# MaartenGr/PolyFuzz

Hardware: AMD Instinct MI355X
Metric: string-pairs/sec, TF-IDF cosine top-n 100k x 100k (config.timed_step says what a step is: by default the user-level .match() call of SURVEY section 8d's metric, `device_step` = the list resident in HBM; latency.top1_single_query_ms = top-1 match latency) (higher is better)
Workload: dtype f32

## Files before the change

### include/polyfuzz_hip.h

```cpp
#ifndef POLYFUZZ_HIP_H
#define POLYFUZZ_HIP_H

#include <stdint.h>

#ifdef __cplusplus
extern "C" {
#endif

#define PFZ_VERSION 100

typedef enum pfz_status {
    PFZ_OK = 0,
    PFZ_ERR_INVALID = -1,
    PFZ_ERR_NO_DEVICE = -2,
    PFZ_ERR_HIP = -3,
    PFZ_ERR_UNSUPPORTED = -4,
    PFZ_ERR_NOMEM = -5,
    PFZ_ERR_RCCL = -6
} pfz_status;

typedef struct pfz_ctx pfz_ctx;
typedef struct pfz_csr pfz_csr;
typedef struct pfz_index pfz_index;
typedef struct pfz_topn pfz_topn;
typedef struct pfz_strings pfz_strings;
typedef struct pfz_tfidf pfz_tfidf;
typedef struct pfz_comm pfz_comm;

int pfz_version(void);
const char *pfz_last_error(void);
int pfz_device_count(void);
int pfz_ctx_create(int device, pfz_ctx **out);
void pfz_ctx_destroy(pfz_ctx *ctx);
int pfz_ctx_sync(pfz_ctx *ctx);
int pfz_ctx_info(pfz_ctx *ctx, char *name256, int32_t *n_cu, int64_t *hbm_bytes);

int pfz_event_record(pfz_ctx *ctx, int32_t slot);
int pfz_event_elapsed_ms(pfz_ctx *ctx, int32_t slot_begin, int32_t slot_end, float *ms);
int pfz_stage_reserve(pfz_ctx *ctx, int64_t bytes, void **host);
int pfz_event_wait(pfz_ctx *ctx, int32_t slot);
int pfz_prof_enable(pfz_ctx *ctx, int32_t on);
int pfz_prof_reset(pfz_ctx *ctx);
int pfz_prof_get(pfz_ctx *ctx, const char *name, double *total_ms, int64_t *launches);

int pfz_csr_upload(pfz_ctx *ctx, int64_t n_rows, int64_t n_cols,
                   const int64_t *indptr, const int32_t *indices, const float *data,
                   pfz_csr **out);
int pfz_csr_shape(const pfz_csr *m, int64_t *n_rows, int64_t *n_cols, int64_t *nnz);
int pfz_csr_download(pfz_ctx *ctx, const pfz_csr *m, int64_t *indptr, int32_t *indices, float *data);
void pfz_csr_free(pfz_csr *m);

int pfz_index_build(pfz_ctx *ctx, const pfz_csr *to_matrix, pfz_index **out);
void pfz_index_free(pfz_index *ix);
int pfz_index_info(const pfz_index *ix, int64_t *n_rows, int64_t *n_cols, int64_t *nnz,
                   int64_t *block_cols, int64_t *n_blocks, int64_t *table_bytes);
int pfz_index_pieces(const pfz_index *ix, int64_t *n_pieces, int64_t *piece_postings);
int pfz_index_symmetric_launches(const pfz_index *ix, int64_t *launches, int64_t *rows);
int pfz_index_symmetric_census(const pfz_index *ix, int64_t *magnet_rows, int64_t *recomputed_rows);

int pfz_topn_alloc(pfz_ctx *ctx, int64_t n_rows, int32_t ntop, pfz_topn **out);
void pfz_topn_free(pfz_topn *t);
int pfz_topn_clear(pfz_ctx *ctx, pfz_topn *t);
int pfz_topn_download(pfz_ctx *ctx, const pfz_topn *t, int32_t *out_idx, float *out_val);
int pfz_topn_download_rows_after(pfz_ctx *ctx, const pfz_topn *t, int64_t row_begin, int64_t row_end,
                                 int32_t event_slot, int32_t *out_idx, float *out_val);
int pfz_topn_rows_begin(pfz_ctx *ctx, const pfz_topn *t, int64_t row_begin, int64_t row_end, int32_t event_slot, int32_t half);
int pfz_topn_rows_finish(pfz_ctx *ctx, int32_t half, const int32_t **idx, const float **val);
int pfz_topn_upload(pfz_ctx *ctx, pfz_topn *t, const int32_t *idx, const float *val);
int pfz_topn_device_ptrs(const pfz_topn *t, void **idx_dev, void **val_dev, int64_t *n_rows, int32_t *ntop);

int pfz_cossim_topn(pfz_ctx *ctx, const pfz_index *to_index, const pfz_csr *from_matrix,
                    int32_t ntop, float lower_bound, int32_t exclude_diag, int64_t diag_offset,
                    pfz_topn *out);

int pfz_cossim_topn_rows(pfz_ctx *ctx, const pfz_index *to_index, const pfz_csr *from_matrix,
                         int64_t row_begin, int64_t row_end, int32_t ntop, float lower_bound,
                         int32_t exclude_diag, int64_t diag_offset, pfz_topn *out);

int pfz_cossim_topn_ranges(pfz_ctx *ctx, const pfz_index *to_index, const pfz_csr *from_matrix, int32_t ntop, float lower_bound,
                           int32_t exclude_diag, int32_t n_ranges, const int64_t *range_ends, int32_t first_event, pfz_topn *out,
                           const int32_t **host_idx, const float **host_val);

int pfz_cossim_topn_host(pfz_ctx *ctx,
                         int64_t n_from, int64_t n_to, int64_t n_cols,
                         const int64_t *from_indptr, const int32_t *from_indices, const float *from_data,
                         const int64_t *to_indptr, const int32_t *to_indices, const float *to_data,
                         int32_t ntop, float lower_bound, int32_t exclude_diag,
                         int32_t *out_idx, float *out_val);

int pfz_strings_upload(pfz_ctx *ctx, const void *chars, const int64_t *offsets, int64_t n_strings,
                       int32_t char_width, pfz_strings **out);
void pfz_strings_free(pfz_strings *s);

typedef struct pfz_tfidf_params {
    int32_t ngram_lo, ngram_hi;
    int32_t clean;
    int32_t remove_space_ngrams;
} pfz_tfidf_params;

int pfz_tfidf_fit(pfz_ctx *ctx, const pfz_tfidf_params *params,
                  const pfz_strings *docs_a, const pfz_strings *docs_b, pfz_tfidf **out);
void pfz_tfidf_free(pfz_tfidf *v);
int pfz_tfidf_info(const pfz_tfidf *v, int64_t *vocab_size, int64_t *n_docs, int32_t *code_bits);
int pfz_tfidf_export(pfz_ctx *ctx, const pfz_tfidf *v, uint32_t *ngrams, double *idf, int64_t *df);
int pfz_tfidf_import(pfz_ctx *ctx, const pfz_tfidf_params *params, int64_t vocab_size, int64_t n_docs,
                     const uint32_t *ngrams, const double *idf, pfz_tfidf **out);
int pfz_tfidf_transform(pfz_ctx *ctx, const pfz_tfidf *v, const pfz_strings *docs, pfz_csr **out);

int pfz_indel_argmax(pfz_ctx *ctx, const pfz_strings *from_strings, const pfz_strings *to_strings,
                     const int32_t *skip_idx, int64_t from_begin, int64_t from_end,
                     int32_t *out_idx, double *out_score);
int pfz_indel_argmax_dev(pfz_ctx *ctx, const pfz_strings *from_strings, const pfz_strings *to_strings,
                         const int32_t *skip_idx, int64_t from_begin, int64_t from_end, pfz_topn *out);
int pfz_indel_matrix_host(pfz_ctx *ctx, const pfz_strings *from_strings, const pfz_strings *to_strings,
                          int64_t from_begin, int64_t from_end, double *out_matrix);
int pfz_indel_plan_info(pfz_ctx *ctx, const pfz_strings *to_strings, int64_t *n_symbols, int64_t *n_groups,
                        int64_t *char_steps);

int pfz_fuzz_extract_one(pfz_ctx *ctx, const pfz_strings *from_strings, const pfz_strings *to_strings, int32_t scorer,
                         const int32_t *skip_idx, int64_t from_begin, int64_t from_end, int32_t *out_idx, double *out_score);
int pfz_fuzz_extract_one_dev(pfz_ctx *ctx, const pfz_strings *from_strings, const pfz_strings *to_strings, int32_t scorer,
                             const int32_t *skip_idx, int64_t from_begin, int64_t from_end, pfz_topn *out,
                             uint64_t *work_counters);
int pfz_fuzz_plan_info(pfz_ctx *ctx, const pfz_strings *to_strings, int64_t *n_symbols, int64_t *n_groups, int64_t *n_tokens,
                       int64_t *n_general_strings);

int pfz_dense_cossim_topn_host(pfz_ctx *ctx, const float *from_vec, int64_t n_from,
                               const float *to_vec, int64_t n_to, int64_t dim,
                               int32_t ntop, float lower_bound, int32_t exclude_diag,
                               int32_t *out_idx, float *out_val);
int pfz_dense_dot_topn_host(pfz_ctx *ctx, const float *from_vec, int64_t n_from,
                            const float *to_vec, int64_t n_to, int64_t dim,
                            int32_t ntop, float lower_bound, int32_t exclude_diag,
                            int32_t *out_idx, float *out_val);

typedef struct pfz_dense pfz_dense;
int pfz_dense_upload(pfz_ctx *ctx, const float *vec, int64_t n, int64_t dim, int32_t normalize, pfz_dense **out);
int pfz_dense_shape(const pfz_dense *m, int64_t *n, int64_t *dim);
void pfz_dense_free(pfz_dense *m);
int pfz_dense_topn(pfz_ctx *ctx, const pfz_dense *from_vectors, const pfz_dense *to_vectors, int32_t ntop,
                   float lower_bound, int32_t exclude_diag, int64_t diag_offset, pfz_topn *out);

int pfz_pr_curve_host(pfz_ctx *ctx, const double *sim, int64_t n, const double *thresholds,
                      int32_t n_thresholds, int64_t *count_ge, double *sum_ge);
int pfz_linkage_top1(pfz_ctx *ctx, const pfz_topn *result, double min_similarity,
                     int32_t *out_cluster, int32_t *out_key, int32_t *out_info3);

int pfz_comm_unique_id(uint8_t id128[128]);
int pfz_comm_init(pfz_ctx *ctx, const uint8_t id128[128], int32_t rank, int32_t world, pfz_comm **out);
int pfz_rccl_versions(int32_t *header, int32_t *runtime);
void pfz_comm_destroy(pfz_comm *c);
typedef struct pfz_comm_group pfz_comm_group;
int pfz_comm_group_create(int32_t world, pfz_comm_group **out);
void pfz_comm_group_destroy(pfz_comm_group *g);
int pfz_comm_init_local(pfz_ctx *ctx, pfz_comm_group *g, int32_t rank, pfz_comm **out);
int pfz_comm_allgather_topn(pfz_comm *c, const pfz_topn *local, pfz_topn *global);
int pfz_comm_merge_to_shards(pfz_comm *c, const pfz_topn *local, int64_t to_offset, pfz_topn *out);
int pfz_comm_barrier(pfz_comm *c);
int pfz_comm_cossim_topn_symmetric(pfz_comm *c, const pfz_index *ix, const pfz_csr *A, int32_t ntop, float lower_bound,
                                   pfz_topn *out);
int pfz_index_symmetric_ok(const pfz_index *ix, const pfz_csr *A, int32_t ntop, int32_t n_parts, int32_t *yes);
int pfz_comm_symmetric_ok(pfz_comm *c, const pfz_index *ix, const pfz_csr *A, int32_t ntop, int32_t *yes);
int pfz_comm_info(const pfz_comm *c, int32_t *rank, int32_t *world);
int pfz_tfidf_fit_sharded(pfz_ctx *ctx, pfz_comm *comm, const pfz_tfidf_params *params,
                          const pfz_strings *replicated, const pfz_strings *local_shard, pfz_tfidf **out);

#ifdef __cplusplus
}
#endif
#endif
```

### polyfuzz_amd/_lib.py

```python
import ctypes
import os
import threading

import numpy as np

from . import _build

c_i32, c_i64, c_f32, c_f64 = ctypes.c_int32, ctypes.c_int64, ctypes.c_float, ctypes.c_double
c_vp = ctypes.c_void_p
P = ctypes.POINTER


class PfzError(RuntimeError):
    def __init__(self, code, msg):
        super().__init__(f"libpolyfuzz_hip error {code}: {msg}")
        self.code = code


class PfzUnsupported(PfzError, NotImplementedError):
    pass


class PfzNoDevice(PfzError):
    pass


class TfidfParams(ctypes.Structure):
    _fields_ = [("ngram_lo", c_i32), ("ngram_hi", c_i32), ("clean", c_i32), ("remove_space_ngrams", c_i32)]


SIGNATURES = {
    "pfz_version": (ctypes.c_int, []),
    "pfz_last_error": (ctypes.c_char_p, []),
    "pfz_device_count": (ctypes.c_int, []),
    "pfz_ctx_create": (ctypes.c_int, [ctypes.c_int, P(c_vp)]),
    "pfz_ctx_destroy": (None, [c_vp]),
    "pfz_ctx_sync": (ctypes.c_int, [c_vp]),
    "pfz_ctx_info": (ctypes.c_int, [c_vp, ctypes.c_char_p, P(c_i32), P(c_i64)]),
    "pfz_event_record": (ctypes.c_int, [c_vp, c_i32]),
    "pfz_event_elapsed_ms": (ctypes.c_int, [c_vp, c_i32, c_i32, P(c_f32)]),
    "pfz_prof_enable": (ctypes.c_int, [c_vp, c_i32]),
    "pfz_prof_reset": (ctypes.c_int, [c_vp]),
    "pfz_prof_get": (ctypes.c_int, [c_vp, ctypes.c_char_p, P(c_f64), P(c_i64)]),
    "pfz_csr_upload": (ctypes.c_int, [c_vp, c_i64, c_i64, c_vp, c_vp, c_vp, P(c_vp)]),
    "pfz_csr_shape": (ctypes.c_int, [c_vp, P(c_i64), P(c_i64), P(c_i64)]),
    "pfz_csr_download": (ctypes.c_int, [c_vp, c_vp, c_vp, c_vp, c_vp]),
    "pfz_csr_free": (None, [c_vp]),
    "pfz_index_build": (ctypes.c_int, [c_vp, c_vp, P(c_vp)]),
    "pfz_index_free": (None, [c_vp]),
    "pfz_index_info": (ctypes.c_int, [c_vp, P(c_i64), P(c_i64), P(c_i64), P(c_i64), P(c_i64), P(c_i64)]),
    "pfz_index_pieces": (ctypes.c_int, [c_vp, P(c_i64), P(c_i64)]),
    "pfz_index_symmetric_launches": (ctypes.c_int, [c_vp, P(c_i64), P(c_i64)]),
    "pfz_index_symmetric_census": (ctypes.c_int, [c_vp, P(c_i64), P(c_i64)]),
    "pfz_index_symmetric_ok": (ctypes.c_int, [c_vp, c_vp, c_i32, c_i32, P(c_i32)]),
    "pfz_comm_cossim_topn_symmetric": (ctypes.c_int, [c_vp, c_vp, c_vp, c_i32, ctypes.c_float, c_vp]),
    "pfz_comm_symmetric_ok": (ctypes.c_int, [c_vp, c_vp, c_vp, c_i32, P(c_i32)]),
    "pfz_rccl_versions": (ctypes.c_int, [P(c_i32), P(c_i32)]),
    "pfz_topn_alloc": (ctypes.c_int, [c_vp, c_i64, c_i32, P(c_vp)]),
    "pfz_topn_free": (None, [c_vp]),
    "pfz_topn_download": (ctypes.c_int, [c_vp, c_vp, c_vp, c_vp]),
    "pfz_topn_clear": (ctypes.c_int, [c_vp, c_vp]),
    "pfz_topn_download_rows_after": (ctypes.c_int, [c_vp, c_vp, c_i64, c_i64, c_i32, c_vp, c_vp]),
    "pfz_topn_rows_begin": (ctypes.c_int, [c_vp, c_vp, c_i64, c_i64, c_i32, c_i32]),
    "pfz_topn_rows_finish": (ctypes.c_int, [c_vp, c_i32, P(c_vp), P(c_vp)]),
    "pfz_cossim_topn_ranges": (ctypes.c_int, [c_vp, c_vp, c_vp, c_i32, ctypes.c_float, c_i32, c_i32, P(c_i64), c_i32, c_vp, P(c_vp), P(c_vp)]),
    "pfz_event_wait": (ctypes.c_int, [c_vp, c_i32]),
    "pfz_stage_reserve": (ctypes.c_int, [c_vp, c_i64, P(c_vp)]),
    "pfz_topn_upload": (ctypes.c_int, [c_vp, c_vp, c_vp, c_vp]),
    "pfz_topn_device_ptrs": (ctypes.c_int, [c_vp, P(c_vp), P(c_vp), P(c_i64), P(c_i32)]),
    "pfz_cossim_topn": (ctypes.c_int, [c_vp, c_vp, c_vp, c_i32, c_f32, c_i32, c_i64, c_vp]),
    "pfz_cossim_topn_rows": (ctypes.c_int, [c_vp, c_vp, c_vp, c_i64, c_i64, c_i32, c_f32, c_i32, c_i64, c_vp]),
    "pfz_cossim_topn_host": (ctypes.c_int, [c_vp, c_i64, c_i64, c_i64, c_vp, c_vp, c_vp, c_vp, c_vp, c_vp,
                                            c_i32, c_f32, c_i32, c_vp, c_vp]),
    "pfz_strings_upload": (ctypes.c_int, [c_vp, c_vp, c_vp, c_i64, c_i32, P(c_vp)]),
    "pfz_strings_free": (None, [c_vp]),
    "pfz_tfidf_fit": (ctypes.c_int, [c_vp, P(TfidfParams), c_vp, c_vp, P(c_vp)]),
    "pfz_tfidf_free": (None, [c_vp]),
    "pfz_tfidf_info": (ctypes.c_int, [c_vp, P(c_i64), P(c_i64), P(c_i32)]),
    "pfz_tfidf_export": (ctypes.c_int, [c_vp, c_vp, c_vp, c_vp, c_vp]),
    "pfz_tfidf_import": (ctypes.c_int, [c_vp, P(TfidfParams), c_i64, c_i64, c_vp, c_vp, P(c_vp)]),
    "pfz_tfidf_transform": (ctypes.c_int, [c_vp, c_vp, c_vp, P(c_vp)]),
    "pfz_indel_argmax": (ctypes.c_int, [c_vp, c_vp, c_vp, c_vp, c_i64, c_i64, c_vp, c_vp]),
    "pfz_indel_matrix_host": (ctypes.c_int, [c_vp, c_vp, c_vp, c_i64, c_i64, c_vp]),
    "pfz_indel_plan_info": (ctypes.c_int, [c_vp, c_vp, P(c_i64), P(c_i64), P(c_i64)]),
    "pfz_indel_argmax_dev": (ctypes.c_int, [c_vp, c_vp, c_vp, c_vp, c_i64, c_i64, c_vp]),
    "pfz_fuzz_extract_one": (ctypes.c_int, [c_vp, c_vp, c_vp, c_i32, c_vp, c_i64, c_i64, c_vp, c_vp]),
    "pfz_fuzz_extract_one_dev": (ctypes.c_int, [c_vp, c_vp, c_vp, c_i32, c_vp, c_i64, c_i64, c_vp, c_vp]),
    "pfz_fuzz_plan_info": (ctypes.c_int, [c_vp, c_vp, P(c_i64), P(c_i64), P(c_i64), P(c_i64)]),
    "pfz_dense_cossim_topn_host": (ctypes.c_int, [c_vp, c_vp, c_i64, c_vp, c_i64, c_i64, c_i32, c_f32, c_i32,
                                                  c_vp, c_vp]),
    "pfz_dense_dot_topn_host": (ctypes.c_int, [c_vp, c_vp, c_i64, c_vp, c_i64, c_i64, c_i32, c_f32, c_i32,
                                               c_vp, c_vp]),
    "pfz_dense_upload": (ctypes.c_int, [c_vp, c_vp, c_i64, c_i64, c_i32, P(c_vp)]),
    "pfz_dense_shape": (ctypes.c_int, [c_vp, P(c_i64), P(c_i64)]),
    "pfz_dense_free": (None, [c_vp]),
    "pfz_dense_topn": (ctypes.c_int, [c_vp, c_vp, c_vp, c_i32, c_f32, c_i32, c_i64, c_vp]),
    "pfz_pr_curve_host": (ctypes.c_int, [c_vp, c_vp, c_i64, c_vp, c_i32, c_vp, c_vp]),
    "pfz_linkage_top1": (ctypes.c_int, [c_vp, c_vp, c_f64, c_vp, c_vp, c_vp]),
    "pfz_comm_unique_id": (ctypes.c_int, [c_vp]),
    "pfz_comm_init": (ctypes.c_int, [c_vp, c_vp, c_i32, c_i32, P(c_vp)]),
    "pfz_comm_destroy": (None, [c_vp]),
    "pfz_comm_group_create": (ctypes.c_int, [c_i32, P(c_vp)]),
    "pfz_comm_group_destroy": (None, [c_vp]),
    "pfz_comm_init_local": (ctypes.c_int, [c_vp, c_vp, c_i32, P(c_vp)]),
    "pfz_comm_allgather_topn": (ctypes.c_int, [c_vp, c_vp, c_vp]),
    "pfz_comm_merge_to_shards": (ctypes.c_int, [c_vp, c_vp, c_i64, c_vp]),
    "pfz_comm_barrier": (ctypes.c_int, [c_vp]),
    "pfz_comm_info": (ctypes.c_int, [c_vp, P(c_i32), P(c_i32)]),
    "pfz_tfidf_fit_sharded": (ctypes.c_int, [c_vp, c_vp, P(TfidfParams), c_vp, c_vp, P(c_vp)]),
}

_lib = None
_lock = threading.Lock()


def lib_path():
    return os.environ.get("POLYFUZZ_HIP_LIB") or _build.LIB_PATH


def load():
    global _lib
    if _lib is not None:
        return _lib
    with _lock:
        if _lib is not None:
            return _lib
        path = lib_path()
        if not os.path.exists(path):
            raise ImportError(
                f"{path} is missing: build it with `python -c 'import __graft_entry__ as g; g.build()'` "
                "(hipcc, gfx950).  polyfuzz_amd has no CPU fallback.")
        lib = ctypes.CDLL(path)
        for name, (res, args) in SIGNATURES.items():
            fn = getattr(lib, name)
            fn.restype = res
            fn.argtypes = args
        _lib = lib
        return lib


def check(rc):
    if rc == 0:
        return
    msg = load().pfz_last_error().decode("utf-8", "replace")
    if rc == -4:
        raise PfzUnsupported(rc, msg)
    if rc == -2:
        raise PfzNoDevice(rc, msg)
    raise PfzError(rc, msg)


def _ptr(a):
    return None if a is None else a.ctypes.data_as(c_vp)


def device_count():
    return int(load().pfz_device_count())


class Context:
    _default = None

    def __init__(self, device=None):
        if device is None:
            device = int(os.environ.get("POLYFUZZ_HIP_DEVICE", os.environ.get("LOCAL_RANK", "0")))
        self.lib = load()
        h = c_vp()
        check(self.lib.pfz_ctx_create(int(device), ctypes.byref(h)))
        self.h = h
        self.device = int(device)

    @classmethod
    def default(cls):
        if cls._default is None:
            cls._default = cls()
        return cls._default

    def close(self):
        if getattr(self, "h", None):
            self.lib.pfz_ctx_destroy(self.h)
            self.h = None

    def __del__(self):
        try:
            self.close()
        except Exception:
            pass

    def sync(self):
        check(self.lib.pfz_ctx_sync(self.h))

    def info(self):
        name = ctypes.create_string_buffer(256)
        ncu, mem = c_i32(), c_i64()
        check(self.lib.pfz_ctx_info(self.h, name, ctypes.byref(ncu), ctypes.byref(mem)))
        return {"name": name.value.decode(), "n_cu": ncu.value, "hbm_bytes": mem.value}

    def event_record(self, slot):
        check(self.lib.pfz_event_record(self.h, slot))

    def event_wait(self, slot):
        check(self.lib.pfz_event_wait(self.h, slot))

    def event_wait_fn(self):
        return ctypes.cast(self.lib.pfz_event_wait, ctypes.c_void_p).value, self.h.value if hasattr(self.h, "value") else int(self.h)

    def event_elapsed_ms(self, a, b):
        ms = c_f32()
        check(self.lib.pfz_event_elapsed_ms(self.h, a, b, ctypes.byref(ms)))
        return float(ms.value)

    def prof_enable(self, on=True):
        check(self.lib.pfz_prof_enable(self.h, int(on)))

    def prof_reset(self):
        check(self.lib.pfz_prof_reset(self.h))

    def prof_get(self, name):
        ms, n = c_f64(), c_i64()
        check(self.lib.pfz_prof_get(self.h, name.encode(), ctypes.byref(ms), ctypes.byref(n)))
        return float(ms.value), int(n.value)


class _Handle:
    _free = None

    def __init__(self, ctx, h):
        self.ctx = ctx
        self.h = h

    def free(self):
        if getattr(self, "h", None) and self.ctx.h:
            getattr(self.ctx.lib, self._free)(self.h)
        self.h = None

    def __del__(self):
        try:
            self.free()
        except Exception:
            pass


class DeviceCSR(_Handle):
    _free = "pfz_csr_free"

    @classmethod
    def upload(cls, ctx, indptr, indices, data, n_cols):
        indptr = np.ascontiguousarray(indptr, np.int64)
        indices = np.ascontiguousarray(indices, np.int32)
        data = np.ascontiguousarray(data, np.float32)
        h = c_vp()
        check(ctx.lib.pfz_csr_upload(ctx.h, len(indptr) - 1, int(n_cols), _ptr(indptr), _ptr(indices), _ptr(data),
                                     ctypes.byref(h)))
        return cls(ctx, h)

    @classmethod
    def from_scipy(cls, ctx, m):
        m = m.tocsr()
        if not m.has_sorted_indices:
            m = m.sorted_indices()
        return cls.upload(ctx, m.indptr, m.indices, m.data, m.shape[1])

    @property
    def shape(self):
        r, c, z = c_i64(), c_i64(), c_i64()
        check(self.ctx.lib.pfz_csr_shape(self.h, ctypes.byref(r), ctypes.byref(c), ctypes.byref(z)))
        return r.value, c.value, z.value

    @property
    def n_rows(self):
        r = c_i64()
        check(self.ctx.lib.pfz_csr_shape(self.h, ctypes.byref(r), None, None))
        return r.value

    def download(self):
        n_rows, n_cols, nnz = self.shape
        indptr = np.empty(n_rows + 1, np.int64)
        indices = np.empty(nnz, np.int32)
        data = np.empty(nnz, np.float32)
        check(self.ctx.lib.pfz_csr_download(self.ctx.h, self.h, _ptr(indptr), _ptr(indices), _ptr(data)))
        return indptr, indices, data, n_cols


class DeviceIndex(_Handle):
    _free = "pfz_index_free"

    @classmethod
    def build(cls, ctx, to_csr):
        h = c_vp()
        check(ctx.lib.pfz_index_build(ctx.h, to_csr.h, ctypes.byref(h)))
        return cls(ctx, h)

    def info(self):
        v = [c_i64() for _ in range(6)]
        check(self.ctx.lib.pfz_index_info(self.h, *[ctypes.byref(x) for x in v]))
        keys = ("n_rows", "n_cols", "nnz", "block_cols", "n_blocks", "table_bytes")
        out = dict(zip(keys, (x.value for x in v)))
        npc, per = c_i64(), c_i64()
        check(self.ctx.lib.pfz_index_pieces(self.h, ctypes.byref(npc), ctypes.byref(per)))
        out.update(n_pieces=npc.value, piece_postings=per.value)
        return out

    def symmetric_launches(self):
        a, b = c_i64(), c_i64()
        check(self.ctx.lib.pfz_index_symmetric_launches(self.h, ctypes.byref(a), ctypes.byref(b)))
        return a.value, b.value

    def symmetric_ok(self, csr, ntop, n_parts=1):
        yes = c_i32()
        check(self.ctx.lib.pfz_index_symmetric_ok(self.h, csr.h, int(ntop), int(n_parts), ctypes.byref(yes)))
        return bool(yes.value)

    def symmetric_census(self):
        a, b = c_i64(), c_i64()
        check(self.ctx.lib.pfz_index_symmetric_census(self.h, ctypes.byref(a), ctypes.byref(b)))
        return a.value, b.value


class DeviceTopN(_Handle):
    _free = "pfz_topn_free"

    @classmethod
    def alloc(cls, ctx, n_rows, ntop):
        h = c_vp()
        check(ctx.lib.pfz_topn_alloc(ctx.h, int(n_rows), int(ntop), ctypes.byref(h)))
        t = cls(ctx, h)
        t.n_rows, t.ntop = int(n_rows), int(ntop)
        return t

    def download(self):
        idx = np.empty((self.n_rows, self.ntop), np.int32)
        val = np.empty((self.n_rows, self.ntop), np.float32)
        check(self.ctx.lib.pfz_topn_download(self.ctx.h, self.h, _ptr(idx), _ptr(val)))
        return idx, val

    def clear(self):
        check(self.ctx.lib.pfz_topn_clear(self.ctx.h, self.h))

    def download_rows_after(self, begin, end, event_slot):
        idx = np.empty((end - begin, self.ntop), np.int32)
        val = np.empty((end - begin, self.ntop), np.float32)
        check(self.ctx.lib.pfz_topn_download_rows_after(self.ctx.h, self.h, int(begin), int(end), int(event_slot), _ptr(idx),
                                                        _ptr(val)))
        return idx, val

    def rows_begin(self, begin, end, event_slot, half):
        check(self.ctx.lib.pfz_topn_rows_begin(self.ctx.h, self.h, int(begin), int(end), int(event_slot), int(half)))

    def rows_finish(self, half):
        a, b = c_vp(), c_vp()
        check(self.ctx.lib.pfz_topn_rows_finish(self.ctx.h, int(half), ctypes.byref(a), ctypes.byref(b)))
        return a.value, b.value

    @classmethod
    def from_host(cls, ctx, idx, val):
        idx = np.ascontiguousarray(idx, np.int32)
        val = np.ascontiguousarray(val, np.float32)
        if idx.ndim == 1:
            idx, val = idx[:, None], val[:, None]
        t = cls.alloc(ctx, idx.shape[0], idx.shape[1])
        check(ctx.lib.pfz_topn_upload(ctx.h, t.h, _ptr(idx), _ptr(val)))
        return t

    def upload(self, idx, val):
        idx = np.ascontiguousarray(idx, np.int32).reshape(self.n_rows, self.ntop)
        val = np.ascontiguousarray(val, np.float32).reshape(self.n_rows, self.ntop)
        check(self.ctx.lib.pfz_topn_upload(self.ctx.h, self.h, _ptr(idx), _ptr(val)))

    def device_ptrs(self):
        pi, pv = c_vp(), c_vp()
        check(self.ctx.lib.pfz_topn_device_ptrs(self.h, ctypes.byref(pi), ctypes.byref(pv), None, None))
        return pi.value, pv.value


def cossim_topn(ctx, index, from_csr, ntop, lower_bound, exclude_diag=False, diag_offset=0, out=None, rows=None):
    if out is None:
        out = DeviceTopN.alloc(ctx, from_csr.n_rows, ntop)
    if rows is None:
        check(ctx.lib.pfz_cossim_topn(ctx.h, index.h, from_csr.h, int(ntop), float(lower_bound),
                                      int(bool(exclude_diag)), int(diag_offset), out.h))
    else:
        check(ctx.lib.pfz_cossim_topn_rows(ctx.h, index.h, from_csr.h, int(rows[0]), int(rows[1]), int(ntop),
                                           float(lower_bound), int(bool(exclude_diag)), int(diag_offset), out.h))
    return out


def cossim_topn_ranges(ctx, index, from_csr, ntop, lower_bound, exclude_diag, range_ends, first_event, out=None, mirror=False):
    if out is None:
        out = DeviceTopN.alloc(ctx, from_csr.n_rows, ntop)
    ends = (c_i64 * len(range_ends))(*[int(e) for e in range_ends])
    hi, hv = c_vp(), c_vp()
    check(ctx.lib.pfz_cossim_topn_ranges(ctx.h, index.h, from_csr.h, int(ntop), float(lower_bound), int(bool(exclude_diag)),
                                         len(range_ends), ends, int(first_event), out.h,
                                         ctypes.byref(hi) if mirror else None, ctypes.byref(hv) if mirror else None))
    return (out, hi.value, hv.value) if mirror else out


def cossim_topn_host(ctx, from_csr3, to_csr3, n_cols, ntop, lower_bound, exclude_diag=False):
    fp, fi, fv = from_csr3
    tp, ti, tv = to_csr3
    fp = np.ascontiguousarray(fp, np.int64)
    fi = np.ascontiguousarray(fi, np.int32)
    fv = np.ascontiguousarray(fv, np.float32)
    tp = np.ascontiguousarray(tp, np.int64)
    ti = np.ascontiguousarray(ti, np.int32)
    tv = np.ascontiguousarray(tv, np.float32)
    n_from, n_to = len(fp) - 1, len(tp) - 1
    idx = np.empty((n_from, ntop), np.int32)
    val = np.empty((n_from, ntop), np.float32)
    check(ctx.lib.pfz_cossim_topn_host(ctx.h, n_from, n_to, int(n_cols), _ptr(fp), _ptr(fi), _ptr(fv),
                                       _ptr(tp), _ptr(ti), _ptr(tv), int(ntop), float(lower_bound),
                                       int(bool(exclude_diag)), _ptr(idx), _ptr(val)))
    return idx, val



try:
    from . import _pack
except ImportError:
    _pack = None


def usable_cpus():
    n = len(os.sched_getaffinity(0)) if hasattr(os, "sched_getaffinity") else (os.cpu_count() or 1)
    try:
        with open("/sys/fs/cgroup/cpu.max") as f:
            quota, period = f.read().split()[:2]
        if quota != "max":
            n = min(n, int(quota) // int(period))
    except (OSError, ValueError):
        pass
    return max(1, n)


def host_threads():
    env = os.environ.get("PFZ_HOST_THREADS")
    return max(1, min(16, int(env))) if env else max(1, min(8, usable_cpus() // 2))


_PACK_THREADS = _PACK_INTO_THREADS = host_threads()


def pack_strings(strings, objects=None):
    if _pack is not None and isinstance(strings, (list, tuple)):
        if objects is not None:
            raw, off, width = _pack.pack(strings, _PACK_THREADS, objects.ctypes.data)
        else:
            raw, off, width = _pack.pack(strings, _PACK_THREADS)
        return np.frombuffer(raw, np.uint8 if width == 1 else np.uint32), np.frombuffer(off, np.int64), width
    if objects is not None:
        objects[:] = strings
    return _pack_strings_py(strings)


def _pack_strings_py(strings):
    n = len(strings)
    lens = np.fromiter(map(len, strings), np.int64, n)
    off = np.zeros(n + 1, np.int64)
    np.cumsum(lens, out=off[1:])
    joined = "".join(strings)
    try:
        raw = joined.encode("latin-1")
        chars = np.frombuffer(raw, np.uint8)
        width = 1
    except UnicodeEncodeError:
        raw = joined.encode("utf-32-le", "surrogatepass")
        chars = np.frombuffer(raw, np.uint32)
        width = 4
    if len(chars) != off[-1]:
        raise ValueError("string packing length mismatch")
    return chars, off, width


class DeviceStrings(_Handle):
    _free = "pfz_strings_free"

    @classmethod
    def upload(cls, ctx, strings):
        if len(strings) >= 1024:
            direct = cls.upload_direct(ctx, strings)
            if direct is not None:
                return direct
        return cls.upload_packed(ctx, *pack_strings(strings))

    @classmethod
    def upload_direct(cls, ctx, strings, objects=None):
        if _pack is None or not hasattr(_pack, "pack_into") or not isinstance(strings, (list, tuple)):
            return None
        n = len(strings)
        off_bytes = (8 * (n + 1) + 255) & ~255
        cap = off_bytes + 48 * n + 65536
        host = c_vp()
        check(ctx.lib.pfz_stage_reserve(ctx.h, cap, ctypes.byref(host)))
        if not host.value:
            return None
        n_chars = _pack.pack_into(strings, objects.ctypes.data if objects is not None else 0, host.value, off_bytes, cap, _PACK_INTO_THREADS)
        if n_chars is None:
            return None
        h = c_vp()
        check(ctx.lib.pfz_strings_upload(ctx.h, c_vp(host.value + off_bytes), c_vp(host.value), n, 1, ctypes.byref(h)))
        s = cls(ctx, h)
        s.n = n
        s.char_width = 1
        return s

    @classmethod
    def upload_packed(cls, ctx, chars, off, width):
        n = len(off) - 1
        h = c_vp()
        check(ctx.lib.pfz_strings_upload(ctx.h, _ptr(chars) if len(chars) else None, _ptr(off), n, width,
                                         ctypes.byref(h)))
        s = cls(ctx, h)
        s.n = n
        s.char_width = width
        return s


class DeviceTfidf(_Handle):
    _free = "pfz_tfidf_free"

    @classmethod
    def fit(cls, ctx, params, docs_a, docs_b=None):
        h = c_vp()
        rc = ctx.lib.pfz_tfidf_fit(ctx.h, ctypes.byref(params), docs_a.h if docs_a is not None else None,
                                   docs_b.h if docs_b is not None else None, ctypes.byref(h))
        if rc == -1 and b"empty vocabulary" in ctx.lib.pfz_last_error():
            raise ValueError("empty vocabulary; perhaps the documents only contain stop words")
        check(rc)
        v = cls(ctx, h)
        v.params = params
        return v

    @classmethod
    def from_state(cls, ctx, params, ngrams, idf, n_docs):
        ngrams = np.ascontiguousarray(ngrams, np.uint32)
        idf = np.ascontiguousarray(idf, np.float64)
        h = c_vp()
        check(ctx.lib.pfz_tfidf_import(ctx.h, ctypes.byref(params), len(idf), int(n_docs), _ptr(ngrams), _ptr(idf),
                                       ctypes.byref(h)))
        v = cls(ctx, h)
        v.params = params
        return v

    def info(self):
        vs, nd, cb = c_i64(), c_i64(), c_i32()
        check(self.ctx.lib.pfz_tfidf_info(self.h, ctypes.byref(vs), ctypes.byref(nd), ctypes.byref(cb)))
        return {"vocab": vs.value, "n_docs": nd.value, "code_bits": cb.value}

# ... 265 lines not shown
```

### polyfuzz_amd/csrc/k3_core.h

```cpp
#pragma once
#include "pfz_internal.h"

#include <math.h>
#include <utility>

#ifndef PFZ_K3_EXP
#define PFZ_K3_EXP 0
#endif

namespace pfz {

constexpr int kSelectMinTop = 16;
constexpr int kWarmMaxTop = 8;
constexpr int kPiece = 16;
constexpr long long kPieceBoundMax = 1 << 20;

#ifndef PFZ_K3_SHFL_MAX
#define PFZ_K3_SHFL_MAX 0
#endif
__device__ inline uint64_t wave_max_u64(uint64_t v)
{
#if PFZ_K3_SHFL_MAX
#pragma unroll
    for (int d = 32; d >= 1; d >>= 1) {
// ... 184 lines not shown
    }
    return best - 1;
}

template <int N4, int kCap, bool kBounded = false>
__device__ inline void sweep_block(int4 *acc4, uint64_t *cand, TopState &st, int col0, int self_col, int ntop, int lane,
                                   int zero, uint64_t ub = ~0ull)
{
    static_assert(N4 % 128 == 0, "a wave sweeps whole 128-slot steps");
#pragma unroll 2
    for (int t = 0; t < N4 / 128; ++t) {
        const int i0 = t * 128 + lane, i1 = i0 + 64;
        const int4 v0 = acc4[i0], v1 = acc4[i1];
        acc4[i0] = make_int4(zero, zero, zero, zero);
        acc4[i1] = make_int4(zero, zero, zero, zero);
        const int mx = max3i(max3i(v0.x, v0.y, v0.z), max3i(v0.w, v1.x, v1.y), max3i(v1.z, v1.w, v1.w));
        if (__ballot(mx > st.thr)) {
            push4<kCap, kBounded>(cand, st, v0, col0 + i0 * 4, self_col, ntop, lane, ub);
            push4<kCap, kBounded>(cand, st, v1, col0 + i1 * 4, self_col, ntop, lane, ub);
        }
    }
}

template <int S> __device__ inline int row_bcast_i(int v)
{
    return __builtin_amdgcn_update_dpp(0, v, 0x150 + S, 0xf, 0xf, false);
}

template <int S>
__device__ inline int2 load_piece_entry(const char *__restrict__ post_bytes, int addr_t, int sub8)
{
    const uint32_t a = (uint32_t)(row_bcast_i<S>(addr_t) + sub8);
#if PFZ_K3_EXP == 2
    return make_int2((int)((a * 2654435761u) >> 19) & 8188, 0x3c000000);
#else
    return *(const int2 *)(post_bytes + a);
#endif
}

template <int S> __device__ inline void apply_entry(int *acc, const int2 &pe, float as_t)
{
    const int v = (int)(__int_as_float(row_bcast_i<S>(__float_as_int(as_t))) * __int_as_float(pe.y));
#if PFZ_K3_EXP == 1
    if (v == 0x7fffffff) atomicAdd((int *)((char *)acc + pe.x), v);
#elif PFZ_K3_EXP == 3
    atomicAdd((int *)((char *)acc + ((pe.x & 0x1f00) | (threadIdx.x * 4))), v);
#else
    atomicAdd((int *)((char *)acc + pe.x), v);
#endif
}

template <int... S>
__device__ inline void run_steps_seq(int *acc, const char *__restrict__ post_bytes, int addr_t, float as_t, int sub8,
                                     std::integer_sequence<int, S...>)
{
    const int2 pe[sizeof...(S)] = {load_piece_entry<S>(post_bytes, addr_t, sub8)...};
    (apply_entry<S>(acc, pe[S], as_t), ...);
}

template <int NS>
__device__ inline void run_steps(int *acc, const char *__restrict__ post_bytes, int addr_t, float as_t, int sub8)
{
    run_steps_seq(acc, post_bytes, addr_t, as_t, sub8, std::make_integer_sequence<int, NS>{});
}

__device__ inline int dpp_add_scan(int v)
{
    asm("s_nop 1\n\tv_add_u32_dpp %0, %0, %0 row_shr:1 row_mask:0xf bank_mask:0xf bound_ctrl:1" : "+v"(v));
    asm("s_nop 1\n\tv_add_u32_dpp %0, %0, %0 row_shr:2 row_mask:0xf bank_mask:0xf bound_ctrl:1" : "+v"(v));
    asm("s_nop 1\n\tv_add_u32_dpp %0, %0, %0 row_shr:4 row_mask:0xf bank_mask:0xf bound_ctrl:1" : "+v"(v));
    asm("s_nop 1\n\tv_add_u32_dpp %0, %0, %0 row_shr:8 row_mask:0xf bank_mask:0xf bound_ctrl:1" : "+v"(v));
    asm("s_nop 1\n\tv_add_u32_dpp %0, %0, %0 row_bcast:15 row_mask:0xa bank_mask:0xf" : "+v"(v));
    asm("s_nop 1\n\tv_add_u32_dpp %0, %0, %0 row_bcast:31 row_mask:0xc bank_mask:0xf" : "+v"(v));
    return v;
}

__device__ inline void scatter_pieces(int *acc, const char *__restrict__ post_bytes, int *mark, int np, int st, float as,
                                      int lane, int src4, int sub8, int dummy_addr)
{
    const int pin = dpp_add_scan(np);
    const int total = __builtin_amdgcn_readlane(pin, 63);
    const int excl = pin - np;
    const int base = st - excl;
    const int pt = 4 * (lane & 15) + (lane >> 4);
    for (int r0 = 0; r0 < total; r0 += 64) {
#if PFZ_K3_EXP == 4
        const int addr_t = np > 0 ? (int)((uint32_t)(st + ((r0 + pt) % np)) << 7) : dummy_addr;
        const float as_t = as;
#else
        const int rel = excl - r0;
        mark[lane] = 0;
        if (np > 0 && rel < 64 && rel + np > 0) mark[rel > 0 ? rel : 0] = lane + 1;
        wave_sync();
        const int owner1 = dpp_max_scan(mark[lane]);
        const int o4 = __builtin_amdgcn_ds_bpermute(src4, owner1) * 4 - 4;
        const int b_o = __builtin_amdgcn_ds_bpermute(o4, base);
        const float as_t = __int_as_float(__builtin_amdgcn_ds_bpermute(o4, __float_as_int(as)));
        const int P = r0 + pt;
        const int addr_t = P < total ? (int)((uint32_t)(b_o + P) << 7) : dummy_addr;
        wave_sync();
#endif
        const int left = total - r0;
        const int ng = left >= 64 ? 8 : (left + 7) >> 3;
#if PFZ_K3_EXP == 6
        if (ng <= 4) {
            if (ng <= 2) run_steps<4>(acc, post_bytes, addr_t, as_t, sub8);
            else run_steps<8>(acc, post_bytes, addr_t, as_t, sub8);
        } else {
            if (ng <= 6) run_steps<12>(acc, post_bytes, addr_t, as_t, sub8);
            else run_steps<16>(acc, post_bytes, addr_t, as_t, sub8);
        }
#else
        if (ng <= 4) {
            if (ng <= 2) {
                if (ng == 1) run_steps<2>(acc, post_bytes, addr_t, as_t, sub8);
                else run_steps<4>(acc, post_bytes, addr_t, as_t, sub8);
            } else {
                if (ng == 3) run_steps<6>(acc, post_bytes, addr_t, as_t, sub8);
                else run_steps<8>(acc, post_bytes, addr_t, as_t, sub8);
            }
        } else {
            if (ng <= 6) {
                if (ng == 5) run_steps<10>(acc, post_bytes, addr_t, as_t, sub8);
                else run_steps<12>(acc, post_bytes, addr_t, as_t, sub8);
            } else {
                if (ng == 7) run_steps<14>(acc, post_bytes, addr_t, as_t, sub8);
                else run_steps<16>(acc, post_bytes, addr_t, as_t, sub8);
            }
        }
#endif
    }
}

inline void k3_fixed_point(const pfz_csr *A, const pfz_index *ix, float lower_bound, float *scale, float *inv_scale, int32_t *thr0)
{
    if (lower_bound < 0.f) lower_bound = 0.f;
    const double bound = (double)A->max_norm * (double)ix->max_norm * 1.0001 + 1e-30;
    int k = 30;
    while (k > -60 && ldexp(bound, k) >= 2147483000.0) --k;
    while (k < 60 && ldexp(bound, k + 1) < 1073741824.0) ++k;
    *scale = (float)ldexp(1.0, k);
    *inv_scale = (float)ldexp(1.0, -k);
    const double thr_d = floor((double)lower_bound * (double)*scale);
    *thr0 = thr_d >= 2147483000.0 ? 2147483000 : (int32_t)thr_d;
}

bool k3_lockstep_wanted(const pfz_ctx *ctx, const pfz_index *ix, int64_t n_rows, int32_t ntop);
int k3_lockstep_launch(pfz_ctx *ctx, const pfz_index *ix, const pfz_csr *A, int64_t row_begin, int64_t n_rows, int32_t ntop,
                       int32_t thr0, float scale, float inv_scale, int32_t exclude_diag, int64_t diag_offset, pfz_topn *out);


int k3_sym_wanted(const pfz_ctx *ctx, const pfz_index *ix, const pfz_csr *A, int64_t row_begin, int64_t row_end, int32_t ntop,
                  int32_t thr0, float scale, int32_t exclude_diag, int64_t diag_offset, const pfz_topn *out);
int k3_sym_launch(pfz_ctx *ctx, const pfz_index *ix, const pfz_csr *A, int64_t row_begin, int64_t row_end, int32_t ntop,
                  int32_t thr0, float scale, float inv_scale, pfz_topn *out, bool start, bool *declined);
int k3_sym_launch_streamed(pfz_ctx *ctx, const pfz_index *ix, const pfz_csr *A, int32_t ntop, int32_t thr0, float scale, float inv_scale,
                           pfz_topn *out, int32_t n_ranges, const int64_t *ends, int32_t first_event, int32_t *host_idx, float *host_val,
                           bool *declined);
void k3_sym_free(pfz_index *ix);

}
```

### polyfuzz_amd/csrc/k3_cossim_topn.hip

```cpp
#include "k3_core.h"

#include <algorithm>
#include <math.h>
#include <stdlib.h>

namespace pfz {

constexpr int kMergeCap = 256;
constexpr int kMaxTop = 1024;

__global__ __launch_bounds__(256) void k_index_count(const int32_t *__restrict__ indptr,
                                                      const int32_t *__restrict__ indices, int32_t n_rows,
                                                      int32_t nb, int32_t block, int32_t *__restrict__ cnt)
{
    const int gid = (blockIdx.x * 256 + threadIdx.x) >> 4;
    const int sub = threadIdx.x & 15;
    if (gid >= n_rows) return;
    const int p0 = indptr[gid], p1 = indptr[gid + 1];
    const int b = gid / block;
    for (int p = p0 + sub; p < p1; p += 16) atomicAdd(&cnt[(int64_t)indices[p] * nb + b], 1);
}

__global__ __launch_bounds__(256) void k_index_fill(const int32_t *__restrict__ indptr,
                                                     const int32_t *__restrict__ indices,
// ... 245 lines not shown
                nxt0 = trow[b_next + 1];
            }
            for (int c0 = p0 + 64; c0 < p1; c0 += 64) {
                int s2 = 0, e2 = 0;
                float as2 = 0.f;
                if (c0 + lane < p1) {
                    const int k = a_idx[c0 + lane];
                    as2 = a_val[c0 + lane] * scale;
                    s2 = tab[(int64_t)k * nb + b];
                    e2 = tab[(int64_t)k * nb + b + 1];
                }
                if (__ballot(e2 > s2)) {
                    touched = true;
                    scatter_pieces(acc, post_bytes, mark, e2 - s2, s2, as2, lane, src4, sub8, dummy_addr);
                }
            }
            if (touched && ablate != 2) {
                wave_sync();
                if (!warmed) {
                    warmed = true;
                    if (ntop <= kWarmMaxTop) {
                        const int t = warm_threshold<N4>(acc4, 0, ntop + (self_col >= 0 ? 1 : 0), lane);
                        st.thr = t > st.thr ? t : st.thr;
                    }
                }
                sweep_block<N4, kCap, kBounded>(acc4, cand, st, b * C, self_col, ntop, lane, zero, ub_row);
                wave_sync();
            }
            b = b_next;
        }

        compact<kCap>(cand, st, ntop, lane);
        if (kBounded && lane == 0) ub[row] = st.cnt == ntop ? cand[ntop - 1] : 0ull;
        for (int r = lane; r < ntop; r += 64) {
            const uint64_t key = r < st.cnt ? cand[r] : 0ull;
            if (n_slices > 1) {
                part_keys[((int64_t)row * n_slices + slice) * ntop + r] = key;
            } else {
                out_idx[(int64_t)row * ntop + r] = key ? (int32_t)(~(uint32_t)key) : -1;
                out_val[(int64_t)row * ntop + r] = key ? (float)(int32_t)(uint32_t)(key >> 32) * inv_scale : 0.f;
            }
        }
        wave_sync();
    }
}

constexpr int kBankMin = 64, kBankCap = 1024;
__global__ __launch_bounds__(256) void k_index_bank_order(const int32_t *__restrict__ cnt, const int32_t *__restrict__ tab,
                                                           const int32_t *__restrict__ heavy, int32_t heavy_cap,
                                                           int2 *__restrict__ post)
{
    __shared__ int2 s_buf[4][kBankCap];
    __shared__ int s_cnt[4][32];
    const int lane = threadIdx.x & 63, wave = threadIdx.x >> 6;
    int2 *buf = s_buf[wave];
    int *bc = s_cnt[wave];
    const int n_heavy = min(heavy[0], heavy_cap);
    const int n_waves = (int)gridDim.x * 4;
    for (int h = (int)blockIdx.x * 4 + wave; h < n_heavy; h += n_waves) {
        {
            const int64_t slot = heavy[1 + h];
            const int c = min(cnt[slot], kBankCap);
            const int64_t base = (int64_t)tab[slot] * kPiece;
            if (lane < 32) bc[lane] = 0;
            __builtin_amdgcn_fence(__ATOMIC_ACQ_REL, "wavefront");
            __builtin_amdgcn_wave_barrier();
            for (int i = lane; i < c; i += 64) {
                int2 pe = post[base + i];
                const int b = (pe.x >> 2) & 31;
                const int j = atomicAdd(&bc[b], 1);
                buf[i] = make_int2(pe.x, pe.y);
                buf[i].x = pe.x | (j << 16);
            }
            __builtin_amdgcn_fence(__ATOMIC_ACQ_REL, "wavefront");
            __builtin_amdgcn_wave_barrier();
            const int my_cnt = lane < 32 ? bc[lane] : 0;
            for (int i = lane; i < c + 63 - (c + 63) % 64; i += 64) {
                const bool on = i < c;
                int2 pe = on ? buf[i] : make_int2(0, 0);
                const int j = (int)((uint32_t)pe.x >> 16), b = (pe.x >> 2) & 31;
                int pos = 0;
#pragma unroll
                for (int q = 0; q < 32; ++q) {
                    const int cq = __shfl(my_cnt, q, 64);
                    pos += min(cq, j) + ((q < b && cq > j) ? 1 : 0);
                }
                if (on) post[base + pos] = make_int2(pe.x & 0xffff, pe.y);
            }
            __builtin_amdgcn_fence(__ATOMIC_ACQ_REL, "wavefront");
            __builtin_amdgcn_wave_barrier();
        }
    }
}

__global__ __launch_bounds__(256) void k3_merge_slices(const uint64_t *__restrict__ part_keys, int32_t n_a,
                                                       int32_t n_slices, int32_t ntop, float inv_scale,
                                                       int32_t *__restrict__ out_idx, float *__restrict__ out_val)
{
    constexpr int kCap = kMergeCap;
    __shared__ __attribute__((aligned(16))) uint64_t cand_all[4][kCap];
    const int lane = threadIdx.x & 63, wave = threadIdx.x >> 6;
    const int row = blockIdx.x * 4 + wave;
    if (row >= n_a) return;
    uint64_t *cand = cand_all[wave];
    TopState st;
    st.cnt = 0;
    st.thr = 0;
    const uint64_t *src = part_keys + (int64_t)row * n_slices * ntop;
    const int total = n_slices * ntop;
    for (int e0 = 0; e0 < total; e0 += 64) {
        const uint64_t key = e0 + lane < total ? src[e0 + lane] : 0ull;
        const uint64_t mk = __ballot(key != 0ull);
        if (key) cand[st.cnt + __popcll(mk & ((1ull << lane) - 1ull))] = key;
        st.cnt += __popcll(mk);
        if (st.cnt > kCap - 64) compact<kCap>(cand, st, ntop, lane, false);
    }
    compact<kCap>(cand, st, ntop, lane);
    for (int r = lane; r < ntop; r += 64) {
        const uint64_t key = r < st.cnt ? cand[r] : 0ull;
        out_idx[(int64_t)row * ntop + r] = key ? (int32_t)(~(uint32_t)key) : -1;
        out_val[(int64_t)row * ntop + r] = key ? (float)(int32_t)(uint32_t)(key >> 32) * inv_scale : 0.f;
    }
}

__global__ __launch_bounds__(256) void k_topn_place(const int32_t *__restrict__ t_idx, const float *__restrict__ t_val, int64_t n_rows,
                                                    int32_t w, int32_t ntop, int32_t col0, int32_t *__restrict__ out_idx,
                                                    float *__restrict__ out_val)
{
    const int64_t i = (int64_t)blockIdx.x * 256 + threadIdx.x;
    if (i >= n_rows * w) return;
    const int64_t r = i / w;
    const int c = (int)(i - r * w);
    out_idx[r * ntop + col0 + c] = t_idx[i];
    out_val[r * ntop + col0 + c] = t_val[i];
}

static int env_int(const char *name, int dflt)
{
    const char *v = getenv(name);
    return v && *v ? atoi(v) : dflt;
}

int index_ready(const pfz_index *ix)
{
    int32_t v = 0;
    if (ix->pieces_lazy.pending) {
        PFZ_TRY(lazy_get(ix->ctx, &ix->pieces_lazy, &v));
        ix->n_pieces = v - 1;
    }
    if (ix->nnz_lazy.pending) {
        PFZ_TRY(lazy_get(ix->ctx, &ix->nnz_lazy, &v));
        ix->nnz = v;
    }
    return PFZ_OK;
}

}

using namespace pfz;

extern "C" {

int pfz_index_build(pfz_ctx *ctx, const pfz_csr *B, pfz_index **out)
{
    PFZ_REQUIRE(ctx && B && out, "pfz_index_build: NULL argument");
    PFZ_HIP(hipSetDevice(ctx->device));
    int block = env_int("PFZ_K3_BLOCK", 2048);
    if (block != 1024 && block != 1536 && block != 2048 && block != 4096) block = 2048;
    const int64_t nb = (B->n_rows + block - 1) / block;
    const int64_t slots = B->n_cols * nb;
    if (slots >= ((int64_t)1 << 31) - 2) {
        set_error("pfz_index_build: vocabulary %lld x %lld to-blocks exceeds the int32 offset table",
                  (long long)B->n_cols, (long long)nb);
        return PFZ_ERR_UNSUPPORTED;
    }
    Owner<pfz_index, pfz_index_free> ix(new pfz_index());
    ix->ctx = ctx;
    ix->n_rows = B->n_rows;
    ix->n_cols = B->n_cols;
    ix->block_cols = block;
    ix->n_blocks = (int32_t)nb;
    ix->max_norm = B->max_norm;
    ix->src_serial = B->serial;
    struct Tmp {
        int32_t *p = nullptr;
        ~Tmp() { if (p) pool_free(p); }
    } cnt, sub;
    const bool any = B->n_rows > 0;
    const bool lds_hist = B->n_cols <= 2 * (int64_t)kHistWords && !getenv("PFZ_NO_LDS_HIST");
    PFZ_TRY(pool_alloc(ctx, &ix->tab_base, (size_t)(slots + 3) * sizeof(int32_t)));
    ix->tab = ix->tab_base + 1;
    PFZ_TRY(pool_alloc(ctx, &cnt.p, (size_t)(slots + 2) * sizeof(int32_t)));
    if (lds_hist && any) {
        PFZ_TRY(pool_alloc(ctx, &sub.p, (size_t)(slots + 1) * kSub * sizeof(int32_t)));
        PFZ_HIP(hipMemsetAsync(sub.p, 0, (size_t)slots * kSub * sizeof(int32_t), ctx->stream));
    } else {
        PFZ_HIP(hipMemsetAsync(cnt.p, 0, (size_t)(slots + 2) * sizeof(int32_t), ctx->stream));
    }
    const char *bo_env = getenv("PFZ_K3_BANK_ORDER");
    const bool bank_order = any && lds_hist && !getenv("PFZ_K3_NO_BANK_ORDER") &&
                            ((bo_env && atoi(bo_env) > 0) || (!bo_env && B->n_rows >= 32768));
    const int32_t bank_min = kBankMin;
    const int32_t heavy_cap = (int32_t)std::min<int64_t>(slots, (int64_t)1 << 22);
    Tmp heavy;
    if (bank_order) {
        PFZ_TRY(pool_alloc(ctx, &heavy.p, (size_t)(heavy_cap + 1) * sizeof(int32_t)));
        PFZ_HIP(hipMemsetAsync(heavy.p, 0, sizeof(int32_t), ctx->stream));
    }
    const int32_t words = (int32_t)((B->n_cols + 1) / 2);
    const unsigned row_grid = (unsigned)((B->n_rows * 16 + 255) / 256);
    const unsigned slot_grid = (unsigned)((slots + kPiece + 255) / 256);
    {
        ProfScope ps(ctx, "k_index_count");
        if (any && lds_hist)
            hipLaunchKernelGGL(k_index_count_lds, dim3((unsigned)nb * kSub), dim3(1024), 0, ctx->stream, B->indptr, B->indices,
                               (int32_t)B->n_rows, (int32_t)nb, block, words, sub.p);
        else if (any)
            hipLaunchKernelGGL(k_index_count, dim3(row_grid), dim3(256), 0, ctx->stream, B->indptr, B->indices,
                               (int32_t)B->n_rows, (int32_t)nb, block, cnt.p);
        hipLaunchKernelGGL(k_index_pieces, dim3(slot_grid), dim3(256), 0, ctx->stream, cnt.p, lds_hist && any ? sub.p : nullptr, slots,
                           ix->tab, heavy.p, heavy_cap, bank_min);
    }
    PFZ_TRY(exclusive_scan_i32(ctx, ix->tab_base, slots + 1, &ix->pieces_lazy));
    const int64_t nnz_bound = B->nnz_lazy.pending ? B->nnz_cap : B->nnz;
    int64_t piece_cap = nnz_bound / kPiece + std::min<int64_t>(slots, nnz_bound) + 1;
    if (piece_cap > kPieceBoundMax) {
        int32_t total = 0;
        PFZ_TRY(lazy_get(ctx, &ix->pieces_lazy, &total));
        ix->n_pieces = total - 1;
        if (total - 1 >= (1 << 25) - 1) {
            set_error("pfz_index_build: %d index pieces (%lld postings padded to 16 per list and block) exceed the 4 GiB "
                      "the kernel addresses with 32-bit byte offsets", total - 1, (long long)csr_nnz(B));
            return PFZ_ERR_UNSUPPORTED;
        }
        piece_cap = total;
    }
    ix->piece_cap = piece_cap;
    PFZ_TRY(lazy_acquire(ctx, &ix->nnz_lazy));
    PFZ_TRY(pool_alloc(ctx, &ix->post, (size_t)piece_cap * kPiece * sizeof(int2)));
    if (block == 2048 && nb >= 2 && nb < 65536)
        PFZ_TRY(pool_alloc(ctx, &ix->pblk, (size_t)piece_cap * sizeof(uint16_t)));
    {
        ProfScope ps(ctx, "k_index_fill");
        hipLaunchKernelGGL(k_index_pad, dim3(slot_grid), dim3(256), 0, ctx->stream, cnt.p, ix->tab, slots, ix->post, ix->pblk, (int32_t)nb,
                           B->indptr + B->n_rows, ix->nnz_lazy.slot);
        PFZ_TRY(lazy_mark(ctx, &ix->nnz_lazy));
        if (any && lds_hist)
            hipLaunchKernelGGL(k_index_fill_lds, dim3((unsigned)nb * kSub), dim3(1024), 0, ctx->stream, B->indptr, B->indices,
                               B->data, (int32_t)B->n_rows, (int32_t)nb, block, words, ix->tab, sub.p, ix->post);
        else if (any)
            hipLaunchKernelGGL(k_index_fill, dim3(row_grid), dim3(256), 0, ctx->stream, B->indptr, B->indices, B->data,
                               (int32_t)B->n_rows, (int32_t)nb, block, cnt.p, ix->tab, ix->post);
    }
    if (bank_order) {
        ProfScope ps(ctx, "k_index_bank_order");
        hipLaunchKernelGGL(k_index_bank_order, dim3((unsigned)ctx->prop.multiProcessorCount * 4), dim3(256), 0, ctx->stream, cnt.p,
                           ix->tab, heavy.p, heavy_cap, ix->post);
    }
    PFZ_HIP(hipGetLastError());
    *out = ix.release();
    return PFZ_OK;
}

void pfz_index_free(pfz_index *ix)
{
    if (!ix) return;
    if (ix->ctx) (void)hipSetDevice(ix->ctx->device);
    k3_sym_free(ix);
    for (LazyI32 *z : {&ix->pieces_lazy, &ix->nnz_lazy})
        if (z->pending || z->slot) {
            if (z->ev) (void)hipEventSynchronize(z->ev);
            lazy_release(ix->ctx, z);
        }
    if (ix->tab_base) pool_free(ix->tab_base);
    if (ix->post) pool_free(ix->post);
    if (ix->pblk) pool_free(ix->pblk);
    delete ix;
}

int pfz_index_info(const pfz_index *ix, int64_t *n_rows, int64_t *n_cols, int64_t *nnz, int64_t *block_cols,
                   int64_t *n_blocks, int64_t *table_bytes)
{
    PFZ_REQUIRE(ix, "pfz_index_info: NULL index");
    PFZ_TRY(index_ready(ix));
    if (n_rows) *n_rows = ix->n_rows;
    if (n_cols) *n_cols = ix->n_cols;
    if (nnz) *nnz = ix->nnz;
    if (block_cols) *block_cols = ix->block_cols;
    if (n_blocks) *n_blocks = ix->n_blocks;
    if (table_bytes) *table_bytes = (ix->n_cols * ix->n_blocks + 2) * (int64_t)sizeof(int32_t);
    return PFZ_OK;
}

int pfz_index_pieces(const pfz_index *ix, int64_t *n_pieces, int64_t *piece_postings)
{
    PFZ_REQUIRE(ix, "pfz_index_pieces: NULL index");
    PFZ_TRY(index_ready(ix));
    if (n_pieces) *n_pieces = ix->n_pieces;
    if (piece_postings) *piece_postings = kPiece;
    return PFZ_OK;
}

int pfz_cossim_topn(pfz_ctx *ctx, const pfz_index *ix, const pfz_csr *A, int32_t ntop, float lower_bound,
                    int32_t exclude_diag, int64_t diag_offset, pfz_topn *out)
{
    PFZ_REQUIRE(A, "pfz_cossim_topn: NULL argument");
// ... 6 lines not shown
    PFZ_REQUIRE(ctx && ix && A && out, "pfz_cossim_topn: NULL argument");
    PFZ_REQUIRE(row_begin >= 0 && row_begin <= row_end && row_end <= A->n_rows,
                "pfz_cossim_topn_rows: rows [%lld, %lld) outside [0, %lld)", (long long)row_begin, (long long)row_end,
                (long long)A->n_rows);
    PFZ_REQUIRE(ntop >= 1, "pfz_cossim_topn: ntop must be >= 1 (got %d)", ntop);
    PFZ_REQUIRE(A->n_cols == ix->n_cols, "pfz_cossim_topn: from-matrix has %lld columns, index has %lld",
                (long long)A->n_cols, (long long)ix->n_cols);
    PFZ_REQUIRE(out->n_rows >= A->n_rows && out->ntop == ntop, "pfz_cossim_topn: result buffer is %lldx%d, need %lldx%d",
                (long long)out->n_rows, out->ntop, (long long)A->n_rows, ntop);
    PFZ_REQUIRE(lower_bound == lower_bound, "pfz_cossim_topn: lower_bound is NaN");
    const int64_t n_rows = row_end - row_begin;
    if (n_rows == 0) return PFZ_OK;
    PFZ_HIP(hipSetDevice(ctx->device));
    float scale, inv_scale;
    int32_t thr0;
    k3_fixed_point(A, ix, lower_bound, &scale, &inv_scale, &thr0);
    if (ntop > kMaxTop) {
        struct Tmp {
            void *p = nullptr;
            ~Tmp() { if (p) pool_free(p); }
        } t_idx, t_val, ub;
        PFZ_TRY(pool_alloc(ctx, &t_idx.p, (size_t)n_rows * kMaxTop * sizeof(int32_t)));
        PFZ_TRY(pool_alloc(ctx, &t_val.p, (size_t)n_rows * kMaxTop * sizeof(float)));
        PFZ_TRY(pool_alloc(ctx, &ub.p, (size_t)n_rows * sizeof(uint64_t)));
        PFZ_HIP(hipMemsetAsync(ub.p, 0xff, (size_t)n_rows * sizeof(uint64_t), ctx->stream));
        const int64_t max_grid = (int64_t)ctx->prop.multiProcessorCount * 16 * 64 * 8;
        const unsigned grid = (unsigned)(n_rows < max_grid ? n_rows : max_grid);
        ProfScope ps(ctx, "k3_cossim_topn");
        for (int32_t col0 = 0; col0 < ntop; col0 += kMaxTop) {
            const int32_t w = ntop - col0 < kMaxTop ? ntop - col0 : kMaxTop;
#define PFZ_K3_DEEP(CC)                                                                                                   \
    hipLaunchKernelGGL((k3_cossim_topn_kernel<CC, 1152, true>), dim3(grid), dim3(64), 0, ctx->stream, A->indptr + row_begin,     \
                       A->indices, A->data, (int32_t)n_rows, ix->tab, ix->post, ix->n_blocks, 0, w, thr0, scale,      \
                       inv_scale, exclude_diag, diag_offset + row_begin, (int32_t *)t_idx.p, (float *)t_val.p, 0, 1,              \
                       (uint64_t *)nullptr, (uint64_t *)ub.p)
            switch (ix->block_cols) {
            case 1024: PFZ_K3_DEEP(1024); break;
            case 1536: PFZ_K3_DEEP(1536); break;
            case 2048: PFZ_K3_DEEP(2048); break;
            case 4096: PFZ_K3_DEEP(4096); break;
            default:
                set_error("pfz_cossim_topn: no kernel for block size %d", ix->block_cols);
                return PFZ_ERR_INVALID;
            }
#undef PFZ_K3_DEEP
            hipLaunchKernelGGL(k_topn_place, dim3((unsigned)((n_rows * w + 255) / 256)), dim3(256), 0, ctx->stream,
                               (const int32_t *)t_idx.p, (const float *)t_val.p, n_rows, w, ntop, col0, out->idx + row_begin * ntop,
                               out->val + row_begin * ntop);
        }
        PFZ_HIP(hipGetLastError());
        return PFZ_OK;
    }
    if (const int sym = k3_sym_wanted(ctx, ix, A, row_begin, row_end, ntop, thr0, scale, exclude_diag, diag_offset, out)) {
        ProfScope ps(ctx, "k3_cossim_topn");
        bool declined = false;
        const int rc = k3_sym_launch(ctx, ix, A, row_begin, row_end, ntop, thr0, scale, inv_scale, out, sym == 1, &declined);
        if (!declined) return rc;
    }
    if (k3_lockstep_wanted(ctx, ix, n_rows, ntop)) {
        ProfScope ps(ctx, "k3_cossim_topn");
        return k3_lockstep_launch(ctx, ix, A, row_begin, n_rows, ntop, thr0, scale, inv_scale, exclude_diag, diag_offset, out);
    }
    int n_slices = env_int("PFZ_K3_SLICES", 0);
    if (n_slices <= 0) {
        const int64_t want = (int64_t)ctx->prop.multiProcessorCount * 24;
        n_slices = n_rows >= want ? 1 : (int)((want + n_rows - 1) / n_rows);
    }
    if (ntop > 128) n_slices = 1;
    n_slices = n_slices < 1 ? 1 : (n_slices > ix->n_blocks ? (ix->n_blocks > 0 ? ix->n_blocks : 1) : n_slices);
    if (ix->n_blocks > 0) {
        const int per_slice = (ix->n_blocks + n_slices - 1) / n_slices;
        n_slices = (ix->n_blocks + per_slice - 1) / per_slice;
    }
    uint64_t *part = nullptr;
    if (n_slices > 1) {
        PFZ_TRY(ensure_scratch(ctx, (size_t)n_rows * (size_t)n_slices * (size_t)ntop * sizeof(uint64_t)));
        part = (uint64_t *)ctx->scratch;
    }
    const int64_t items = n_rows * n_slices;
    const int64_t max_grid = (int64_t)ctx->prop.multiProcessorCount * 16 * 64 * 8;
    const unsigned grid = (unsigned)(items < max_grid ? items : max_grid / n_slices * n_slices);
    const int cap = ntop <= 32 ? 96 : (ntop <= 64 ? 128 : (ntop <= 128 ? 256 : 1152));
#ifdef PFZ_EXPERIMENTS
    const int ablate = env_int("PFZ_K3_ABLATE", 0);
#else
    const int ablate = 0;
#endif
    {
        ProfScope ps(ctx, "k3_cossim_topn");
#define PFZ_K3_LAUNCH(CC, CAP)                                                                                  \
    hipLaunchKernelGGL((k3_cossim_topn_kernel<CC, CAP>), dim3(grid), dim3(64), 0, ctx->stream,                  \
                       A->indptr + row_begin, A->indices, A->data, (int32_t)n_rows, ix->tab, ix->post,          \
                       ix->n_blocks, 0, ntop, thr0, scale, inv_scale, exclude_diag,                  \
                       diag_offset + row_begin, out->idx + row_begin * ntop, out->val + row_begin * ntop,       \
                       ablate, n_slices, part)
#define PFZ_K3_CASE(CC)                              \
    case CC:                                         \
        if (cap == 96) PFZ_K3_LAUNCH(CC, 96);        \
        else if (cap == 128) PFZ_K3_LAUNCH(CC, 128); \
        else if (cap == 256) PFZ_K3_LAUNCH(CC, 256); \
        else PFZ_K3_LAUNCH(CC, 1152);                \
        break;
        switch (ix->block_cols) {
            PFZ_K3_CASE(1024)
            PFZ_K3_CASE(1536)
            PFZ_K3_CASE(2048)
            PFZ_K3_CASE(4096)
        default:
            set_error("pfz_cossim_topn: no kernel for block size %d", ix->block_cols);
            return PFZ_ERR_INVALID;
        }
#undef PFZ_K3_CASE
#undef PFZ_K3_LAUNCH
    }
    if (n_slices > 1) {
        ProfScope ps(ctx, "k3_merge_slices");
        hipLaunchKernelGGL(k3_merge_slices, dim3((unsigned)((n_rows + 3) / 4)), dim3(256), 0, ctx->stream, part,
                           (int32_t)n_rows, n_slices, ntop, inv_scale, out->idx + row_begin * ntop, out->val + row_begin * ntop);
    }
    PFZ_HIP(hipGetLastError());
    return PFZ_OK;
}

int pfz_cossim_topn_ranges(pfz_ctx *ctx, const pfz_index *ix, const pfz_csr *A, int32_t ntop, float lower_bound, int32_t exclude_diag,
                           int32_t n_ranges, const int64_t *range_ends, int32_t first_event, pfz_topn *out, const int32_t **host_idx,
                           const float **host_val)
{
    if (host_idx) *host_idx = nullptr;
    if (host_val) *host_val = nullptr;
    PFZ_REQUIRE(ctx && ix && A && out && range_ends, "pfz_cossim_topn_ranges: NULL argument");
    PFZ_REQUIRE(n_ranges >= 1 && first_event >= 0 && first_event + n_ranges <= kEventSlots,
                "pfz_cossim_topn_ranges: %d ranges from event slot %d do not fit the %d slots", n_ranges, first_event, kEventSlots);
    int64_t prev = 0;
    bool on_blocks = true;
    for (int32_t i = 0; i < n_ranges; ++i) {
        PFZ_REQUIRE(range_ends[i] > prev && range_ends[i] <= A->n_rows, "pfz_cossim_topn_ranges: range ends must ascend inside (0, %lld]",
                    (long long)A->n_rows);
        on_blocks = on_blocks && (i == n_ranges - 1 || range_ends[i] % 2048 == 0);
        prev = range_ends[i];
    }
    PFZ_REQUIRE(prev == A->n_rows, "pfz_cossim_topn_ranges: the last range must end at the matrix' last row");
    PFZ_REQUIRE(ntop >= 1 && lower_bound == lower_bound && A->n_cols == ix->n_cols && out->n_rows >= A->n_rows && out->ntop == ntop,
                "pfz_cossim_topn_ranges: arguments as for pfz_cossim_topn");
    PFZ_HIP(hipSetDevice(ctx->device));
    if (on_blocks && ntop <= kMaxTop && !getenv("PFZ_K3_NO_STREAMED")) {
        float scale, inv_scale;
        int32_t thr0;
        k3_fixed_point(A, ix, lower_bound, &scale, &inv_scale, &thr0);
        if (k3_sym_wanted(ctx, ix, A, 0, A->n_rows, ntop, thr0, scale, exclude_diag, 0, out) == 1) {
            int32_t *h_idx = nullptr;
            float *h_val = nullptr;
            if (host_idx && host_val) {
                const size_t cells = (size_t)A->n_rows * (size_t)ntop;
                const size_t bytes = cells * (sizeof(int32_t) + sizeof(float));
                if (bytes > ctx->mirror_bytes) {
                    PFZ_HIP(hipStreamSynchronize(ctx->stream));
                    if (ctx->stream3) PFZ_HIP(hipStreamSynchronize(ctx->stream3));
                    for (int q = 0; q < 3; ++q)
                        if (ctx->stream3x[q]) PFZ_HIP(hipStreamSynchronize(ctx->stream3x[q]));
                    if (ctx->mirror) PFZ_HIP(hipHostFree(ctx->mirror));
                    ctx->mirror = nullptr;
                    ctx->mirror_bytes = 0;
                    PFZ_HIP(hipHostMalloc((void **)&ctx->mirror, bytes + bytes / 8, hipHostMallocDefault));
                    ctx->mirror_bytes = bytes + bytes / 8;
                }
                h_idx = (int32_t *)ctx->mirror;
                h_val = (float *)(ctx->mirror + cells * sizeof(int32_t));
            }
            ProfScope ps(ctx, "k3_cossim_topn");
            bool declined = false;
            const int rc = k3_sym_launch_streamed(ctx, ix, A, ntop, thr0, scale, inv_scale, out, n_ranges, range_ends, first_event, h_idx, h_val,
                                                  &declined);
            if (!declined) {
                if (rc == PFZ_OK && h_idx) {
                    *host_idx = h_idx;
                    *host_val = h_val;
                }
                return rc;
            }
        }
    }
    prev = 0;
    for (int32_t i = 0; i < n_ranges; ++i) {
        PFZ_TRY(pfz_cossim_topn_rows(ctx, ix, A, prev, range_ends[i], ntop, lower_bound, exclude_diag, 0, out));
        PFZ_HIP(hipEventRecord(ctx->events[first_event + i], ctx->stream));
        ctx->evt_want[first_event + i] = 0;
        prev = range_ends[i];
    }
    return PFZ_OK;
}

int pfz_cossim_topn_host(pfz_ctx *ctx, int64_t n_from, int64_t n_to, int64_t n_cols, const int64_t *from_indptr,
                         const int32_t *from_indices, const float *from_data, const int64_t *to_indptr,
                         const int32_t *to_indices, const float *to_data, int32_t ntop, float lower_bound,
                         int32_t exclude_diag, int32_t *out_idx, float *out_val)
{
    PFZ_REQUIRE(ctx && out_idx && out_val, "pfz_cossim_topn_host: NULL argument");
    pfz_csr *A = nullptr, *B = nullptr;
    pfz_index *ix = nullptr;
    pfz_topn *res = nullptr;
    int rc = pfz_csr_upload(ctx, n_from, n_cols, from_indptr, from_indices, from_data, &A);
    if (rc == PFZ_OK) rc = pfz_csr_upload(ctx, n_to, n_cols, to_indptr, to_indices, to_data, &B);
    if (rc == PFZ_OK) rc = pfz_index_build(ctx, B, &ix);
    if (rc == PFZ_OK) rc = pfz_topn_alloc(ctx, n_from, ntop, &res);
    if (rc == PFZ_OK) rc = pfz_cossim_topn(ctx, ix, A, ntop, lower_bound, exclude_diag, 0, res);
    if (rc == PFZ_OK) rc = pfz_topn_download(ctx, res, out_idx, out_val);
    pfz_topn_free(res);
    pfz_index_free(ix);
    pfz_csr_free(B);
    pfz_csr_free(A);
    return rc;
}

}
```

### polyfuzz_amd/csrc/k3_symmetric.hip

```cpp
#include "k3_core.h"

#include <stdio.h>
#include <stdlib.h>

namespace pfz {

constexpr int kSymC = 2048;
constexpr int kSymCap = 96;
constexpr int kSymKeep = 32;
#ifndef PFZ_K3_SYM_F
#define PFZ_K3_SYM_F 128
#endif
#ifndef PFZ_K3_SYM_PUSH
#define PFZ_K3_SYM_PUSH 512
#endif
constexpr int kSymF = PFZ_K3_SYM_F;
constexpr int kSymPush = PFZ_K3_SYM_PUSH;
constexpr int kSymMergeCap = kSymPush + 64;
#ifndef PFZ_K3_SYM_SIDE_STREAMS
#define PFZ_K3_SYM_SIDE_STREAMS 2
#endif
constexpr int kSymSides = PFZ_K3_SYM_SIDE_STREAMS;
static_assert(kSymSides >= 1 && kSymSides <= 4, "one to four side streams");
constexpr int kSymSlices = 8;
constexpr int kSymSlicedRows = 4096;
#ifndef PFZ_K3_SYM_EXP
#define PFZ_K3_SYM_EXP 0
#endif
constexpr int kSymMag = 1;
constexpr int kSymMagBlocks = 8;
constexpr int kSymP0PerCu = 128;
constexpr int kSymDoneStride = 32;
constexpr int kNoThr = 0x7fffffff;

struct K3SymArgs {
    const int32_t *a_indptr;
    const int32_t *a_idx;
    const float *a_val;
    int32_t n;
    const int32_t *tab;
    const int2 *post;
    const int2 *post_sym;
    const uint16_t *pblk;
    const int32_t *n_pieces1;
    int32_t nb, ntop, thr0;
    float scale, inv_scale;
    int32_t row_begin, row_end;
    int32_t n_parts, my_part, per;
    int32_t thr_by_part;
    uint64_t *keys_out;
    int32_t *thrv;
    uint16_t *slot4;
    uint32_t *gmin;
    int32_t *thr_slot;
    uint16_t *row_slot;
    int32_t *mag;
    int32_t n_mag_items, mag_b0, mag_row_end;
    uint64_t *keys;
    int32_t *push_cnt;
    uint64_t *push_buf;
    int32_t *ovf;
    uint64_t *part;
    int32_t ovf_base, ovf_max, n_sl;
    int32_t *out_idx;
    float *out_val;
    int32_t *host_idx;
    float *host_val;
    uint32_t *done;
    int32_t blk_lo, blk_hi;
};

__device__ inline int thr_pos(const K3SymArgs &a, int row)
{
    return a.thr_by_part ? (row % a.n_parts) * a.per + row / a.n_parts : row;
}
__device__ inline bool row_is_mine(const K3SymArgs &a, int row) { return a.n_parts == 1 || row % a.n_parts == a.my_part; }


__host__ __device__ inline int sym_slot(int rho, int i, int *t, int *l, int *e)
{
    const int p = i >> 1, half = i & 1, c = rho & 3;
    *t = p >> 3;
    *l = (rho >> 2) + 8 * (p & 7);
    *e = half * 4 + c;
    return 512 * *t + 256 * half + 4 * *l + c;
}

__global__ __launch_bounds__(1024) void k3_sym_order(const K3SymArgs a)
{
    __shared__ int s_gmin[256];
    const int b = blockIdx.x, lane = threadIdx.x & 63, wave = threadIdx.x >> 6;
    if (threadIdx.x < 256) s_gmin[threadIdx.x] = kNoThr;
    if (threadIdx.x == 0 && a.done) a.done[b * kSymDoneStride] = 0u;
    __syncthreads();
    for (int rho = wave * 2; rho < wave * 2 + 2; ++rho) {
        const int r = rho + 32 * lane;
        const int row = b * kSymC + r;
        if (row < a.n) a.push_cnt[row] = 0;
        const int thr = row < a.n ? a.thrv[thr_pos(a, row)] : kNoThr;
        const uint64_t key = ((uint64_t)(uint32_t)thr << 6) | (uint32_t)lane;
        int rank = 0;
#pragma unroll 16
        for (int m = 0; m < 64; ++m) {
            const uint32_t lo = (uint32_t)__builtin_amdgcn_readlane((int)(uint32_t)key, m);
            const uint32_t hi = (uint32_t)__builtin_amdgcn_readlane((int)(uint32_t)(key >> 32), m);
            rank += ((((uint64_t)hi << 32) | lo) < key) ? 1 : 0;
        }
        int t, l, e;
        const int slot = sym_slot(rho, rank, &t, &l, &e);
        const bool magnet = rank < kSymMag && row < a.n && b > 0;
        if (rank < kSymMag) a.mag[(int64_t)b * (32 * kSymMag) + rho * kSymMag + rank] = magnet ? row : -1;
        a.slot4[(int64_t)b * kSymC + r] = (uint16_t)(slot * 4);
        a.thr_slot[(int64_t)b * kSymC + slot] = magnet ? kNoThr : thr;
        a.row_slot[(int64_t)b * kSymC + slot] = (uint16_t)r;
        if (!magnet) atomicMin(&s_gmin[t * 64 + l], thr);
    }
    __syncthreads();
    if (threadIdx.x < 64) {
        uint32_t w = 0;
        for (int t = 0; t < 4; ++t) {
            const int g = s_gmin[t * 64 + threadIdx.x];
            w |= (g == kNoThr ? 0xffu : (uint32_t)g >> 24) << (8 * t);
        }
        a.gmin[(int64_t)b * 64 + threadIdx.x] = w;
    }
}

__global__ __launch_bounds__(256) void k3_sym_repost(const K3SymArgs a)
{
    const int64_t i = (int64_t)blockIdx.x * 256 + threadIdx.x;
    if (i >= (int64_t)*a.n_pieces1 * (kPiece / 2)) return;
    const int piece = (int)(i >> 3);
    const int b = a.pblk[piece];
    int4 e = ((const int4 *)a.post)[i];
    const uint16_t *s4 = a.slot4 + (int64_t)b * kSymC;
    if (piece > 0) {
        e.x = s4[e.x >> 2];
        e.z = s4[e.z >> 2];
    }
    ((int4 *)a.post_sym)[i] = e;
}


constexpr uint32_t kStageOwn = 1u << 30;
constexpr uint32_t kStageFgn = 1u << 31;

#ifndef PFZ_K3_SYM_PLAIN_STORES
#define PFZ_K3_SYM_PLAIN_STORES 0
#endif
__device__ inline void store_coherent(uint64_t *p, uint64_t v)
{
#if PFZ_K3_SYM_PLAIN_STORES
    *p = v;
#else
    __hip_atomic_store(p, v, __ATOMIC_RELAXED, __HIP_MEMORY_SCOPE_AGENT);
#endif
}

__device__ inline void sym_item_done(const K3SymArgs &a, int blk, int lane)
{
    if (!a.done) return;
    asm volatile("s_waitcnt vmcnt(0)" ::: "memory");
    if (lane == 0) __hip_atomic_fetch_add(&a.done[blk * kSymDoneStride], 1u, __ATOMIC_RELAXED, __HIP_MEMORY_SCOPE_AGENT);
}

__device__ inline uint32_t sym_items_of_block(const K3SymArgs &a, int b)
{
    const int rows = b < a.nb - 1 ? (a.n - b * kSymC < kSymC ? a.n - b * kSymC : kSymC) : 0;
    return (uint32_t)(rows + 32 * kSymMag * ((a.nb - 1 + kSymMagBlocks - 1) / kSymMagBlocks));
}

__global__ __launch_bounds__(64) void k3_sym_wait(const K3SymArgs a, int32_t *flag, int32_t flag_value)
{
    const int lane = threadIdx.x;
    if (lane == 0) {
        if (flag) __hip_atomic_store(flag, flag_value, __ATOMIC_RELAXED, __HIP_MEMORY_SCOPE_SYSTEM);
        if (a.blk_lo < a.blk_hi) a.ovf[0] = 0;
    }
    const uint64_t t0 = wall_clock64();
    for (int b0 = a.blk_lo; b0 < a.blk_hi; b0 += 64) {
        const int b = b0 + lane;
        const bool on = b < a.blk_hi;
        const uint32_t want = on ? sym_items_of_block(a, b) : 0u;
        for (;;) {
            const uint32_t got = on ? __hip_atomic_load(&a.done[b * kSymDoneStride], __ATOMIC_RELAXED, __HIP_MEMORY_SCOPE_AGENT) : 0u;
            if (!__ballot(got < want)) break;
            if (wall_clock64() - t0 > 1000000000ull) __builtin_trap();
            __builtin_amdgcn_s_sleep(32);
        }
    }
}

template <int kCap>
__device__ inline void drain_stage(uint64_t *cand, TopState &st, uint64_t *fbuf, int &fcnt, int ntop, int lane,
                                   const K3SymArgs &a, uint32_t inv_row)
{
    wave_sync();
    for (int e0 = 0; e0 < fcnt; e0 += 64) {
        const bool on = e0 + lane < fcnt;
        const uint64_t en = on ? fbuf[e0 + lane] : 0ull;
        const uint32_t lo = (uint32_t)en;
        const int cell = (int)(lo & 0x3fffffffu);
        const int x = (int)(uint32_t)(en >> 32);
        int rowl = 0, thr = kNoThr;
        if (on) {
            rowl = a.row_slot[cell];
            thr = a.thr_slot[cell];
        }
        const int row = (cell & ~(kSymC - 1)) + rowl;
#if PFZ_K3_SYM_EXP == 5
        if (false) {
#else
        if ((lo & kStageFgn) && x > thr) {
#endif
            const int pos = atomicAdd(&a.push_cnt[row], 1);
            if (pos < kSymPush) store_coherent(&a.push_buf[(int64_t)row * kSymPush + pos], (en & 0xffffffff00000000ull) | inv_row);
        }
        const bool own = (lo & kStageOwn) && x > st.thr;
        const uint64_t mo = __ballot(own);
        if (mo) {
            const int pos = st.cnt + __popcll(mo & ((1ull << lane) - 1ull));
            if (own) cand[pos] = (en & 0xffffffff00000000ull) | (uint32_t)(~row);
            st.cnt += __popcll(mo);
            st.pushed = 1;
            if (st.cnt > kCap - 64) compact<kCap>(cand, st, ntop, lane, false);
        }
    }
    wave_sync();
    fcnt = 0;
}

template <int kCap>
__device__ inline void stage1(uint64_t *cand, TopState &st, uint64_t *fbuf, int &fcnt, int x, uint32_t tgu, int cell, int ntop,
                              int lane, const K3SymArgs &a, uint32_t inv_row)
{
    const bool own = x > st.thr, fgn = (uint32_t)x >= tgu;
    const uint64_t mk = __ballot(own || fgn);
    if (mk) {
        const int pos = fcnt + __popcll(mk & ((1ull << lane) - 1ull));
        if (own || fgn)
            fbuf[pos] = ((uint64_t)(uint32_t)x << 32) | (own ? kStageOwn : 0u) | (fgn ? kStageFgn : 0u) | (uint32_t)cell;
        fcnt += __popcll(mk);
        if (fcnt > kSymF - 64) drain_stage<kCap>(cand, st, fbuf, fcnt, ntop, lane, a, inv_row);
    }
}

template <int kCap>
__device__ inline void stage8(uint64_t *cand, TopState &st, uint64_t *fbuf, int &fcnt, const int4 &v0, const int4 &v1, int pa,
                              int pb, int pc, uint32_t tgu, int cell0, int cell1, int ntop, int lane, const K3SymArgs &a,
                              uint32_t inv_row)
{
    if (__ballot(pa > st.thr || (uint32_t)pa >= tgu)) {
        stage1<kCap>(cand, st, fbuf, fcnt, v0.x, tgu, cell0, ntop, lane, a, inv_row);
        stage1<kCap>(cand, st, fbuf, fcnt, v0.y, tgu, cell0 + 1, ntop, lane, a, inv_row);
        stage1<kCap>(cand, st, fbuf, fcnt, v0.z, tgu, cell0 + 2, ntop, lane, a, inv_row);
    }
    if (__ballot(pb > st.thr || (uint32_t)pb >= tgu)) {
        stage1<kCap>(cand, st, fbuf, fcnt, v0.w, tgu, cell0 + 3, ntop, lane, a, inv_row);
        stage1<kCap>(cand, st, fbuf, fcnt, v1.x, tgu, cell1, ntop, lane, a, inv_row);
        stage1<kCap>(cand, st, fbuf, fcnt, v1.y, tgu, cell1 + 1, ntop, lane, a, inv_row);
    }
    if (__ballot(pc > st.thr || (uint32_t)pc >= tgu)) {
        stage1<kCap>(cand, st, fbuf, fcnt, v1.z, tgu, cell1 + 2, ntop, lane, a, inv_row);
        stage1<kCap>(cand, st, fbuf, fcnt, v1.w, tgu, cell1 + 3, ntop, lane, a, inv_row);
    }
}

template <int B> __device__ inline uint64_t top_byte_reaches(int mx, uint32_t q)
{
    uint64_t m;
    if (B == 0) asm("v_cmp_ge_u32_sdwa %0, %1, %2 src0_sel:BYTE_3 src1_sel:BYTE_0" : "=s"(m) : "v"(mx), "v"(q));
    else asm("v_cmp_ge_u32_sdwa %0, %1, %2 src0_sel:BYTE_3 src1_sel:BYTE_1" : "=s"(m) : "v"(mx), "v"(q));
    return m;
}

template <int N4, int kCap>
__device__ inline void sweep_block_handover(int4 *acc4, uint64_t *cand, TopState &st, int b, int ntop, int lane, int zero,
                                            uint32_t tq, uint64_t *fbuf, int &fcnt, const K3SymArgs &a, uint32_t inv_row)
{
    static_assert(N4 / 128 == 4, "four sweep steps per block");
#pragma unroll 1
    for (int h = 0; h < 2; ++h) {
#pragma unroll
        for (int u = 0; u < 2; ++u) {
            const int t = 2 * h + u;
            const int i0 = t * 128 + lane, i1 = i0 + 64;
            const int4 v0 = acc4[i0], v1 = acc4[i1];
            acc4[i0] = make_int4(zero, zero, zero, zero);
            acc4[i1] = make_int4(zero, zero, zero, zero);
            const int pa = max3i(v0.x, v0.y, v0.z), pb = max3i(v0.w, v1.x, v1.y), pc = max(v1.z, v1.w);
            const int mx = max3i(pa, pb, pc);
            const uint64_t hit = __ballot(mx > st.thr) | (u == 0 ? top_byte_reaches<0>(mx, tq) : top_byte_reaches<1>(mx, tq));
            if (hit)
                stage8<kCap>(cand, st, fbuf, fcnt, v0, v1, pa, pb, pc, (u == 0 ? tq << 24 : tq << 16) & 0xff000000u, b * kSymC + i0 * 4,
                             b * kSymC + i1 * 4, ntop, lane, a, inv_row);
        }
        tq >>= 16;
    }
}

__device__ inline void store_result(const K3SymArgs &a, int row, int r, uint64_t key)
{
    if (a.keys_out) {
        a.keys_out[(int64_t)row * a.ntop + r] = key;
    } else {
        const int32_t j = key ? (int32_t)(~(uint32_t)key) : -1;
        const float v = key ? (float)(int32_t)(uint32_t)(key >> 32) * a.inv_scale : 0.f;
        a.out_idx[(int64_t)row * a.ntop + r] = j;
        a.out_val[(int64_t)row * a.ntop + r] = v;
        if (a.host_idx) {
            a.host_idx[(int64_t)row * a.ntop + r] = j;
            a.host_val[(int64_t)row * a.ntop + r] = v;
        }
    }
}

template <int C, int MODE>
__global__ __launch_bounds__(64) void k3_sym_kernel(const K3SymArgs a)
{
    static_assert(C == kSymC, "sym_slot() is written for 2048-row blocks");
    __shared__ __attribute__((aligned(16))) struct {
        int acc[C];
        uint64_t cand[kSymCap];
        uint64_t fbuf[MODE == 1 ? kSymF : 1];
    } sm;
    int *const acc = sm.acc;
    uint64_t *const cand = sm.cand;
    uint64_t *const fbuf = sm.fbuf;
    int *const mark = (int *)(sm.cand + kSymCap) - 64;
// ... 333 lines not shown
    delete s;
    ix->sym = nullptr;
}

static int sym_env_int(const char *name, int dflt)
{
    const char *v = getenv(name);
    return v && *v ? atoi(v) : dflt;
}

int k3_sym_wanted(const pfz_ctx *ctx, const pfz_index *ix, const pfz_csr *A, int64_t row_begin, int64_t row_end, int32_t ntop,
                  int32_t thr0, float scale, int32_t exclude_diag, int64_t diag_offset, const pfz_topn *out)
{
    (void)ctx;
    const int force = sym_env_int("PFZ_K3_SYM", -1);
    if (force == 0) return 0;
    if (!exclude_diag || diag_offset != 0 || A->serial != ix->src_serial || A->n_rows != ix->n_rows) return 0;
    if (ix->block_cols != kSymC || !ix->pblk || ntop > kSymKeep || ix->n_blocks < 2 || ix->n_rows >= ((int64_t)1 << 30)) return 0;
    const K3SymState *s = ix->sym;
    if (s && s->n < 0) return 0;
    if (row_begin > 0) {
        const bool cont = s && s->next_row == row_begin && s->a_serial == A->serial && s->out == out && s->ntop == ntop &&
                          s->thr0 == thr0 && s->scale == scale;
        return cont ? 2 : 0;
    }
    if (force == 1) return 1;
    if (ix->n_rows < sym_env_int("PFZ_K3_SYM_MIN", 20480) || ix->n_rows > 250000) return 0;
    return (row_end - row_begin) * 5 >= ix->n_rows ? 1 : 0;
}

static int sym_state_alloc(pfz_ctx *ctx, const pfz_index *ix, K3SymState *s)
{
    const int64_t n = ix->n_rows;
    const size_t cells = (size_t)ix->n_blocks * kSymC;
    PFZ_TRY(pool_alloc(ctx, &s->thrv, (size_t)(n + 64) * sizeof(int32_t)));
    PFZ_TRY(pool_alloc(ctx, &s->slot4, cells * sizeof(uint16_t)));
    PFZ_TRY(pool_alloc(ctx, &s->gmin, cells / 32 * sizeof(uint32_t)));
    PFZ_TRY(pool_alloc(ctx, &s->thr_slot, cells * sizeof(int32_t)));
    PFZ_TRY(pool_alloc(ctx, &s->row_slot, cells * sizeof(uint16_t)));
    PFZ_TRY(pool_alloc(ctx, &s->mag, (size_t)ix->n_blocks * 32 * kSymMag * sizeof(int32_t)));
    PFZ_TRY(pool_alloc(ctx, &s->post_sym, (size_t)ix->piece_cap * kPiece * sizeof(int2)));
    PFZ_TRY(pool_alloc(ctx, &s->keys, (size_t)n * kSymKeep * sizeof(uint64_t)));
    PFZ_TRY(pool_alloc(ctx, &s->push_cnt, (size_t)n * sizeof(int32_t)));
    PFZ_TRY(pool_alloc(ctx, &s->push_buf, (size_t)n * kSymPush * sizeof(uint64_t)));
    PFZ_TRY(pool_alloc(ctx, &s->ovf, (size_t)(n + 1) * sizeof(int32_t)));
    PFZ_TRY(pool_alloc(ctx, &s->part, (size_t)kSymSlicedRows * kSymSlices * kSymKeep * sizeof(uint64_t)));
    for (int q = 0; q + 1 < kSymSides; ++q) {
        PFZ_TRY(pool_alloc(ctx, &s->ovfx[q], (size_t)(n + 1) * sizeof(int32_t)));
        PFZ_TRY(pool_alloc(ctx, &s->partx[q], (size_t)kSymSlicedRows * kSymSlices * kSymKeep * sizeof(uint64_t)));
    }
    PFZ_TRY(pool_alloc(ctx, &s->done, (size_t)(ix->n_blocks + 64) * kSymDoneStride * sizeof(uint32_t)));
    return PFZ_OK;
}

static K3SymState *sym_state_of(pfz_ctx *ctx, const pfz_index *ix)
{
    K3SymState *s = ix->sym;
    if (s) return s->n < 0 ? nullptr : s;
    s = new K3SymState();
    s->ctx = ctx;
    s->n = ix->n_rows;
    ix->sym = s;
    if (getenv("PFZ_K3_SYM_FAIL_ALLOC") || sym_state_alloc(ctx, ix, s) != PFZ_OK) {
        void *const bufs[] = {s->thrv, s->slot4, s->gmin, s->thr_slot, s->row_slot, s->mag, s->post_sym, s->keys, s->push_cnt, s->push_buf, s->ovf, s->part, s->ovfx[0], s->partx[0], s->ovfx[1], s->partx[1], s->ovfx[2], s->partx[2], s->done};
        for (void *p : bufs)
            if (p) pool_free(p);
        *s = K3SymState();
        s->ctx = ctx;
        s->n = -1;
        (void)hipGetLastError();
        return nullptr;
    }
    return s;
}

static int64_t sym_repost_pairs(const pfz_index *ix)
{
    if (ix->pieces_lazy.pending && hipEventQuery(ix->pieces_lazy.ev) == hipSuccess) (void)index_ready(ix);
    (void)hipGetLastError();
    return (ix->pieces_lazy.pending ? ix->piece_cap : (int64_t)ix->n_pieces + 1) * (kPiece / 2);
}

static void sym_fill_args(K3SymArgs &a, const pfz_index *ix, const pfz_csr *A, K3SymState *s, int32_t ntop, int32_t thr0, float scale,
                          float inv_scale)
{
    a.a_indptr = A->indptr;
    a.a_idx = A->indices;
    a.a_val = A->data;
    a.n = (int32_t)ix->n_rows;
    a.tab = ix->tab;
    a.post = ix->post;
    a.post_sym = s->post_sym;
    a.pblk = ix->pblk;
    a.nb = ix->n_blocks;
    a.n_pieces1 = ix->tab + ix->n_cols * ix->n_blocks;
    a.ntop = ntop;
    a.thr0 = thr0;
    a.scale = scale;
    a.inv_scale = inv_scale;
    a.row_begin = 0;
    a.row_end = (int32_t)ix->n_rows;
    a.n_parts = 1;
    a.my_part = 0;
    a.per = (int32_t)ix->n_rows;
    a.thr_by_part = 0;
    a.keys_out = nullptr;
    a.thrv = s->thrv;
    a.slot4 = s->slot4;
    a.gmin = s->gmin;
    a.thr_slot = s->thr_slot;
    a.row_slot = s->row_slot;
    a.mag = s->mag;
    a.n_mag_items = 0;
    a.mag_b0 = 0;
    a.mag_row_end = 0;
    a.keys = s->keys;
    a.push_cnt = s->push_cnt;
    a.push_buf = s->push_buf;
    a.ovf = s->ovf;
    a.part = s->part;
    a.ovf_base = 0;
    a.ovf_max = 0;
    a.n_sl = 1;
    a.out_idx = nullptr;
    a.out_val = nullptr;
    a.done = nullptr;
    a.blk_lo = a.blk_hi = 0;
    a.host_idx = nullptr;
    a.host_val = nullptr;
}

static void sym_launch_pass2(pfz_ctx *ctx, K3SymArgs a, hipStream_t stream = nullptr, int per_cu = 16)
{
    if (!stream) stream = ctx->stream;
    const int nb = a.nb;
    const unsigned grid2 = (unsigned)ctx->prop.multiProcessorCount * (unsigned)per_cu;
    const int per = (nb + kSymSlices - 1) / kSymSlices;
    a.n_mag_items = 0;
    a.n_parts = 1;
    a.n_sl = (nb + per - 1) / per;
    a.ovf_base = 0;
    a.ovf_max = kSymSlicedRows;
    if (a.n_sl > 1) {
        hipLaunchKernelGGL((k3_sym_kernel<kSymC, 2>), dim3(grid2), dim3(64), 0, stream, a);
        hipLaunchKernelGGL(k3_sym_merge_slices, dim3(256), dim3(256), 0, stream, a);
        a.ovf_base = kSymSlicedRows;
    }
    a.n_sl = 1;
    a.ovf_max = a.n;
    hipLaunchKernelGGL((k3_sym_kernel<kSymC, 2>), dim3(grid2), dim3(64), 0, stream, a);
}

int k3_sym_launch(pfz_ctx *ctx, const pfz_index *ix, const pfz_csr *A, int64_t row_begin, int64_t row_end, int32_t ntop,
                  int32_t thr0, float scale, float inv_scale, pfz_topn *out, bool start, bool *declined)
{
    const int64_t n = ix->n_rows;
    const int nb = ix->n_blocks;
    *declined = false;
    K3SymState *s = sym_state_of(ctx, ix);
    if (!s) {
        *declined = true;
        return PFZ_OK;
    }
    s->next_row = -1;
    K3SymArgs a;
    sym_fill_args(a, ix, A, s, ntop, thr0, scale, inv_scale);
    a.out_idx = out->idx;
    a.out_val = out->val;
    if (start) {
        a.row_begin = 0;
        a.row_end = (int32_t)n;
        const unsigned grid0 = (unsigned)std::min<int64_t>(n, (int64_t)ctx->prop.multiProcessorCount * kSymP0PerCu);
        hipLaunchKernelGGL((k3_sym_kernel<kSymC, 0>), dim3(grid0), dim3(64), 0, ctx->stream, a);
        hipLaunchKernelGGL(k3_sym_order, dim3((unsigned)nb), dim3(1024), 0, ctx->stream, a);
        const int64_t pairs = sym_repost_pairs(ix);
        hipLaunchKernelGGL(k3_sym_repost, dim3((unsigned)((pairs + 255) / 256)), dim3(256), 0, ctx->stream, a);
    }
    PFZ_HIP(hipMemsetAsync(s->ovf, 0, sizeof(int32_t), ctx->stream));
    const int64_t last_block_row = (int64_t)(nb - 1) * kSymC;
    a.row_begin = (int32_t)row_begin;
    a.row_end = (int32_t)(row_end < last_block_row ? row_end : last_block_row);
    if (a.row_end < a.row_begin) a.row_end = a.row_begin;
    a.mag_b0 = (int32_t)(row_begin / kSymC);
    a.mag_row_end = (int32_t)row_end;
    a.n_mag_items = (int32_t)(((row_end - 1) / kSymC - a.mag_b0 + 1) * 32 * kSymMag * ((nb - 1 + kSymMagBlocks - 1) / kSymMagBlocks));
#ifdef PFZ_EXPERIMENTS
    if (const char *solo = getenv("PFZ_K3_SYM_SOLO")) {
        int p = 0, np_ = 1;
        if (sscanf(solo, "%d/%d", &p, &np_) == 2 && np_ > 1 && p >= 0 && p < np_ && row_begin == 0) {
            a.n_parts = np_;
            a.my_part = p;
            a.row_begin = p;
        }
    }
    const int rows1 = a.row_end > a.row_begin ? (a.row_end - a.row_begin + a.n_parts - 1) / a.n_parts : 0;
    if (rows1 + a.n_mag_items > 0)
        hipLaunchKernelGGL((k3_sym_kernel<kSymC, 1>), dim3((unsigned)(rows1 + a.n_mag_items)), dim3(64), 0, ctx->stream, a);
    a.n_parts = 1;
    a.my_part = 0;
    if (false)
#endif
    if (a.row_end - a.row_begin + a.n_mag_items > 0)
        hipLaunchKernelGGL((k3_sym_kernel<kSymC, 1>), dim3((unsigned)(a.row_end - a.row_begin + a.n_mag_items)), dim3(64), 0, ctx->stream, a);
    a.n_mag_items = 0;
    a.row_begin = (int32_t)row_begin;
    a.row_end = (int32_t)row_end;
    hipLaunchKernelGGL(k3_sym_merge<4>, dim3((unsigned)((row_end - row_begin + 3) / 4)), dim3(256), 0, ctx->stream, a);
    sym_launch_pass2(ctx, a);
    PFZ_HIP(hipGetLastError());
    s->next_row = row_end;
    s->launches += 1;
    s->rows += row_end - row_begin;
    s->a_serial = A->serial;
    s->out = out;
    s->ntop = ntop;
    s->thr0 = thr0;
    s->scale = scale;
    return PFZ_OK;
}

int k3_sym_launch_streamed(pfz_ctx *ctx, const pfz_index *ix, const pfz_csr *A, int32_t ntop, int32_t thr0, float scale, float inv_scale,
                           pfz_topn *out, int32_t n_ranges, const int64_t *ends, int32_t first_event, int32_t *host_idx, float *host_val,
                           bool *declined)
{
    const int64_t n = ix->n_rows;
    const int nb = ix->n_blocks;
    *declined = false;
    K3SymState *s = sym_state_of(ctx, ix);
    if (!s) {
        *declined = true;
        return PFZ_OK;
    }
    if (!ctx->stream3) {
        int pr_lo = 0, pr_hi = 0;
        PFZ_HIP(hipDeviceGetStreamPriorityRange(&pr_lo, &pr_hi));
        PFZ_HIP(hipStreamCreateWithPriority(&ctx->stream3, hipStreamNonBlocking, pr_hi));
        PFZ_HIP(hipEventCreateWithFlags(&ctx->ev3, hipEventDisableTiming));
        for (int q = 0; q + 1 < kSymSides; ++q) {
            PFZ_HIP(hipStreamCreateWithPriority(&ctx->stream3x[q], hipStreamNonBlocking, pr_hi));
            PFZ_HIP(hipEventCreateWithFlags(&ctx->ev3x[q], hipEventDisableTiming));
        }
    }
    s->next_row = -1;
    K3SymArgs a;
    sym_fill_args(a, ix, A, s, ntop, thr0, scale, inv_scale);
    a.out_idx = out->idx;
    a.out_val = out->val;
    a.host_idx = host_idx;
    a.host_val = host_val;
    a.done = s->done;
    const unsigned grid0 = (unsigned)std::min<int64_t>(n, (int64_t)ctx->prop.multiProcessorCount * kSymP0PerCu);
    hipLaunchKernelGGL((k3_sym_kernel<kSymC, 0>), dim3(grid0), dim3(64), 0, ctx->stream, a);
    hipLaunchKernelGGL(k3_sym_order, dim3((unsigned)nb), dim3(1024), 0, ctx->stream, a);
    const int64_t pairs = sym_repost_pairs(ix);
    hipLaunchKernelGGL(k3_sym_repost, dim3((unsigned)((pairs + 255) / 256)), dim3(256), 0, ctx->stream, a);
    PFZ_HIP(hipEventRecord(ctx->ev3, ctx->stream));
    const int64_t last_block_row = (int64_t)(nb - 1) * kSymC;
    a.row_begin = 0;
    a.row_end = (int32_t)last_block_row;
    a.mag_b0 = 0;
    a.mag_row_end = (int32_t)n;
    a.n_mag_items = (int32_t)((int64_t)nb * 32 * kSymMag * ((nb - 1 + kSymMagBlocks - 1) / kSymMagBlocks));
    a.done = s->done;
    hipLaunchKernelGGL((k3_sym_kernel<kSymC, 1>), dim3((unsigned)(a.row_end + a.n_mag_items)), dim3(64), 0, ctx->stream, a);
    PFZ_HIP(hipGetLastError());
    a.n_mag_items = 0;
    hipStream_t sides[4] = {ctx->stream3, ctx->stream3x[0], ctx->stream3x[1], ctx->stream3x[2]};
    hipEvent_t side_ev[4] = {ctx->ev3, ctx->ev3x[0], ctx->ev3x[1], ctx->ev3x[2]};
    const int n_sides = n_ranges < kSymSides ? n_ranges : kSymSides;
    for (int q = 0; q < n_sides; ++q) PFZ_HIP(hipStreamWaitEvent(sides[q], ctx->ev3, 0));
    int64_t row0 = 0;
    int64_t covered[4] = {0, 0, 0, 0};
    int32_t *flag[4] = {nullptr, nullptr, nullptr, nullptr};
    int32_t flag_value[4] = {0, 0, 0, 0};
    for (int32_t i = 0; i < n_ranges; ++i) {
        const int q = i % n_sides;
        hipStream_t side = sides[q];
        const int64_t row1 = ends[i];
        a.ovf = q ? s->ovfx[q - 1] : s->ovf;
        a.part = q ? s->partx[q - 1] : s->part;
        a.blk_lo = (int32_t)(covered[q] / kSymC);
        a.blk_hi = (int32_t)((row1 + kSymC - 1) / kSymC);
        covered[q] = row1;
        hipLaunchKernelGGL(k3_sym_wait, dim3(1), dim3(64), 0, side, a, flag[q], flag_value[q]);
        a.row_begin = (int32_t)row0;
        a.row_end = (int32_t)row1;
        hipLaunchKernelGGL(k3_sym_merge<PFZ_K3_SYM_MERGE_W>, dim3((unsigned)((row1 - row0 + PFZ_K3_SYM_MERGE_W - 1) / PFZ_K3_SYM_MERGE_W)),
                           dim3(64 * PFZ_K3_SYM_MERGE_W), 0, side, a);
        sym_launch_pass2(ctx, a, side, 2);
        PFZ_HIP(hipGetLastError());
        PFZ_HIP(hipEventRecord(ctx->events[first_event + i], side));
        PFZ_TRY(event_flag_next(ctx, first_event + i, &flag[q], &flag_value[q]));
        row0 = row1;
    }
    a.blk_lo = a.blk_hi = 0;
    a.ovf = s->ovf;
    a.part = s->part;
    for (int q = 0; q < n_sides; ++q) {
        hipLaunchKernelGGL(k3_sym_wait, dim3(1), dim3(64), 0, sides[q], a, flag[q], flag_value[q]);
        PFZ_HIP(hipGetLastError());
        PFZ_HIP(hipEventRecord(side_ev[q], sides[q]));
    }
    for (int q = 0; q < n_sides; ++q) PFZ_HIP(hipStreamWaitEvent(ctx->stream, side_ev[q], 0));
    s->next_row = n;
    s->launches += 1;
    s->rows += n;
    s->a_serial = A->serial;
    s->out = out;
    s->ntop = ntop;
    s->thr0 = thr0;
    s->scale = scale;
    return PFZ_OK;
}

__global__ __launch_bounds__(256) void k3_sym_merge_parts(const uint64_t *__restrict__ keys_all, int32_t n_parts, int32_t n,
                                                           int32_t ntop, float inv_scale, int32_t *__restrict__ out_idx,
                                                           float *__restrict__ out_val)
{
    __shared__ __attribute__((aligned(16))) uint64_t cand_all[4][256];
    const int lane = threadIdx.x & 63, wave = threadIdx.x >> 6;
    const int row = blockIdx.x * 4 + wave;
    if (row >= n) return;
    uint64_t *cand = cand_all[wave];
    TopState st;
    st.cnt = 0;
    st.thr = 0;
    st.pushed = 0;
    const int total = n_parts * ntop;
    for (int e0 = 0; e0 < total; e0 += 64) {
        const int e = e0 + lane;
        const uint64_t k = e < total ? keys_all[((int64_t)(e / ntop) * n + row) * ntop + e % ntop] : 0ull;
        const uint64_t mk = __ballot(k != 0ull);
        if (k) cand[st.cnt + __popcll(mk & ((1ull << lane) - 1ull))] = k;
        st.cnt += __popcll(mk);
    }
    compact<256>(cand, st, ntop, lane);
    for (int q = lane; q < ntop; q += 64) {
        const uint64_t key = q < st.cnt ? cand[q] : 0ull;
        out_idx[(int64_t)row * ntop + q] = key ? (int32_t)(~(uint32_t)key) : -1;
        out_val[(int64_t)row * ntop + q] = key ? (float)(int32_t)(uint32_t)(key >> 32) * inv_scale : 0.f;
    }
}

bool k3_sym_sharded_ok(const pfz_index *ix, const pfz_csr *A, int32_t ntop, int32_t n_parts)
{
    if (A->serial != ix->src_serial || A->n_rows != ix->n_rows) return false;
    if (ix->block_cols != kSymC || !ix->pblk || ntop > kSymKeep || ix->n_blocks < 2 || ix->n_rows >= ((int64_t)1 << 30)) return false;
    if (n_parts < 1 || (int64_t)n_parts * ntop > 256 || n_parts > 64) return false;
    if (ix->sym && ix->sym->n < 0) return false;
    const int force = sym_env_int("PFZ_K3_SYM", -1);
    if (force >= 0) return force != 0;
    return ix->n_rows >= sym_env_int("PFZ_K3_SYM_MIN", 20480) && ix->n_rows <= 250000;
}

static int k3_sym_sharded_body(pfz_ctx *ctx, pfz_comm *comm, const pfz_index *ix, const pfz_csr *A, int32_t ntop, float lower_bound,
                               pfz_topn *out);

int k3_sym_sharded(pfz_ctx *ctx, pfz_comm *comm, const pfz_index *ix, const pfz_csr *A, int32_t ntop, float lower_bound, pfz_topn *out)
{
    const int rc = k3_sym_sharded_body(ctx, comm, ix, A, ntop, lower_bound, out);
    if (rc != PFZ_OK && comm_world(comm) > 1) comm_abort(comm);
    return rc;
}

static int k3_sym_sharded_body(pfz_ctx *ctx, pfz_comm *comm, const pfz_index *ix, const pfz_csr *A, int32_t ntop, float lower_bound,
                               pfz_topn *out)
{
    const int64_t n = ix->n_rows;
    const int nb = ix->n_blocks;
    const int n_parts = comm_world(comm), part = comm_rank(comm);
    K3SymState *s = sym_state_of(ctx, ix);
    if (!s) {
        set_error("pfz_comm_cossim_topn_symmetric: the session buffers of this index could not be allocated");
        return PFZ_ERR_NOMEM;
    }
    float scale, inv_scale;
    int32_t thr0;
    k3_fixed_point(A, ix, lower_bound, &scale, &inv_scale, &thr0);
    s->next_row = -1;
    struct Tmp {
        uint64_t *p = nullptr;
        ~Tmp() { if (p) pool_free(p); }
    } mine, all;
    const size_t list_bytes = (size_t)n * ntop * sizeof(uint64_t);
    PFZ_TRY(pool_alloc(ctx, &mine.p, list_bytes));
    PFZ_TRY(pool_alloc(ctx, &all.p, list_bytes * n_parts));
    K3SymArgs a;
    sym_fill_args(a, ix, A, s, ntop, thr0, scale, inv_scale);
    a.n_parts = n_parts;
    a.my_part = part;
    a.per = (int32_t)((n + n_parts - 1) / n_parts);
    a.thr_by_part = 1;
    a.keys_out = mine.p;
    PFZ_HIP(hipMemsetAsync(s->ovf, 0, sizeof(int32_t), ctx->stream));
    a.row_begin = part;
    a.row_end = (int32_t)n;
    const unsigned mine0 = (unsigned)((n - part + n_parts - 1) / n_parts);
    const unsigned grid0 = std::min<unsigned>(mine0, (unsigned)ctx->prop.multiProcessorCount * (unsigned)kSymP0PerCu);
    if (mine0) hipLaunchKernelGGL((k3_sym_kernel<kSymC, 0>), dim3(grid0), dim3(64), 0, ctx->stream, a);
    PFZ_HIP(hipGetLastError());
    if (n_parts > 1) PFZ_TRY(comm_allgather_bytes(comm, s->thrv + (size_t)part * a.per, s->thrv, (size_t)a.per * sizeof(int32_t)));
    hipLaunchKernelGGL(k3_sym_order, dim3((unsigned)nb), dim3(1024), 0, ctx->stream, a);
    const int64_t pairs = sym_repost_pairs(ix);
    hipLaunchKernelGGL(k3_sym_repost, dim3((unsigned)((pairs + 255) / 256)), dim3(256), 0, ctx->stream, a);
    const int64_t last_block_row = (int64_t)(nb - 1) * kSymC;
    a.row_end = (int32_t)(n < last_block_row ? n : last_block_row);
    const int rows1 = a.row_end > part ? (a.row_end - part + n_parts - 1) / n_parts : 0;
    if (a.row_end < a.row_begin) a.row_end = a.row_begin;
    a.mag_b0 = 0;
    a.mag_row_end = (int32_t)n;
    a.n_mag_items = (int32_t)(nb * 32 * kSymMag * ((nb - 1 + kSymMagBlocks - 1) / kSymMagBlocks));
    hipLaunchKernelGGL((k3_sym_kernel<kSymC, 1>), dim3((unsigned)(rows1 + a.n_mag_items)), dim3(64), 0, ctx->stream, a);
    a.n_mag_items = 0;
    a.row_begin = 0;
    a.row_end = (int32_t)n;
    hipLaunchKernelGGL(k3_sym_merge<4>, dim3((unsigned)((n + 3) / 4)), dim3(256), 0, ctx->stream, a);
    sym_launch_pass2(ctx, a);
    PFZ_HIP(hipGetLastError());
    const uint64_t *lists = mine.p;
    if (n_parts > 1) {
        PFZ_TRY(comm_allgather_bytes(comm, mine.p, all.p, list_bytes));
        lists = all.p;
    }
    hipLaunchKernelGGL(k3_sym_merge_parts, dim3((unsigned)((n + 3) / 4)), dim3(256), 0, ctx->stream, lists, n_parts, (int32_t)n, ntop,
                       inv_scale, out->idx, out->val);
    PFZ_HIP(hipGetLastError());
    s->launches += 1;
    s->rows += n;
    return PFZ_OK;
}

}

extern "C" int pfz_index_symmetric_launches(const pfz_index *ix, int64_t *launches, int64_t *rows)
{
    PFZ_REQUIRE(ix, "pfz_index_symmetric_launches: NULL index");
    if (launches) *launches = ix->sym ? ix->sym->launches : 0;
    if (rows) *rows = ix->sym ? ix->sym->rows : 0;
    return PFZ_OK;
}

extern "C" int pfz_index_symmetric_census(const pfz_index *ix, int64_t *magnet_rows, int64_t *recomputed_rows)
{
    PFZ_REQUIRE(ix, "pfz_index_symmetric_census: NULL index");
    int64_t mags = 0, rec = 0;
    const pfz::K3SymState *s = ix->sym;
    if (s && s->n > 0 && s->launches > 0) {
        PFZ_HIP(hipSetDevice(ix->ctx->device));
        std::vector<int32_t> mag((size_t)ix->n_blocks * 32 * pfz::kSymMag);
        int32_t n_ovf = 0;
        PFZ_TRY(pfz::copy_d2h(ix->ctx, mag.data(), s->mag, mag.size() * sizeof(int32_t)));
        PFZ_TRY(pfz::copy_d2h(ix->ctx, &n_ovf, s->ovf, sizeof(int32_t)));
        for (int32_t r : mag) mags += r >= 0;
        rec = n_ovf;
    }
    if (magnet_rows) *magnet_rows = mags;
    if (recomputed_rows) *recomputed_rows = rec;
    return PFZ_OK;
}
// ... 39 lines not shown
```

### polyfuzz_amd/csrc/pfz_internal.h

```cpp
#pragma once

#include <hip/hip_runtime.h>
#include <stdint.h>
#include <string>
#include <vector>
#include <map>
#include <atomic>

#include "polyfuzz_hip.h"

namespace pfz {

void set_error(const char *fmt, ...) __attribute__((format(printf, 1, 2)));
int hip_fail(hipError_t e, const char *what, const char *file, int line);

#define PFZ_HIP(call)                                                      \
    do {                                                                   \
        hipError_t _e = (call);                                            \
        if (_e != hipSuccess) return pfz::hip_fail(_e, #call, __FILE__, __LINE__); \
    } while (0)

#define PFZ_TRY(call)                 \
    do {                              \
        int _s = (call);              \
        if (_s != PFZ_OK) return _s;  \
    } while (0)

#define PFZ_REQUIRE(cond, ...)                    \
    do {                                          \
        if (!(cond)) {                            \
            pfz::set_error(__VA_ARGS__);          \
            return PFZ_ERR_INVALID;               \
        }                                         \
    } while (0)

constexpr int kWave = 64;
constexpr int kHistWords = 36864;
constexpr int kEventSlots = 64;

inline uint64_t next_serial()
{
    static std::atomic<uint64_t> s{1};
    return s.fetch_add(1);
}
struct K3SymState;

struct LazyI32 {
    hipEvent_t ev = nullptr;
    int32_t *slot = nullptr;
    bool pending = false;
    int32_t value = 0;
};

struct ProfEntry {
    std::vector<hipEvent_t> begin, end;
    double total_ms = 0.0;
    int64_t launches = 0;
};

}

struct pfz_ctx {
    int device = -1;
    hipStream_t stream = nullptr;
    hipStream_t stream2 = nullptr;
    hipEvent_t side_events[4] = {};
    hipStream_t stream3 = nullptr;
    hipEvent_t ev3 = nullptr;
    hipStream_t stream3x[3] = {nullptr, nullptr, nullptr};
    hipEvent_t ev3x[3] = {nullptr, nullptr, nullptr};
    hipDeviceProp_t prop;
    hipEvent_t events[pfz::kEventSlots] = {};
    bool prof = false;
    int prof_level = 0;
    std::map<std::string, pfz::ProfEntry> prof_entries;
    std::vector<hipEvent_t> event_pool;
    void *scratch = nullptr;
    size_t scratch_bytes = 0;
    char *stage = nullptr;
    size_t stage_bytes = 0, stage_off = 0;
    char *stage2 = nullptr;
    size_t stage2_bytes = 0;
    int32_t *evt_flag = nullptr;
    int32_t evt_want[pfz::kEventSlots] = {};
    int32_t evt_serial = 0;
    struct RowsJob { const pfz_topn *t = nullptr; int64_t row_begin = 0, row_end = 0; int32_t slot = -1; bool issued = false; } rows_job[2];
    char *mirror = nullptr;
    size_t mirror_bytes = 0;
    char *rows_stage[2] = {};
    size_t rows_bytes[2] = {}, rows_n[2] = {};
    hipEvent_t rows_ev[2] = {};
    uint64_t *scan_state = nullptr;
    size_t scan_tiles = 0;
    uint32_t scan_epoch = 0;
    std::vector<int32_t *> lazy_slots;
    std::vector<hipEvent_t> lazy_events;
    std::vector<int32_t *> lazy_chunks;
    std::map<size_t, std::vector<void *>> pool_free_lists;
    size_t pool_cached_bytes = 0, pool_live_bytes = 0;
};

struct pfz_csr {
    pfz_ctx *ctx = nullptr;
    int64_t n_rows = 0, n_cols = 0;
    mutable int64_t nnz = 0;
    mutable pfz::LazyI32 nnz_lazy;
    int64_t nnz_cap = 0;
    int32_t *indptr = nullptr;
    int32_t *indices = nullptr;
    float *data = nullptr;
    float max_norm = 1.f;
    uint64_t serial = pfz::next_serial();
};

struct pfz_index {
    pfz_ctx *ctx = nullptr;
    int64_t n_rows = 0, n_cols = 0;
    int32_t block_cols = 0, n_blocks = 0;
    mutable int32_t n_pieces = 0;
    mutable int64_t nnz = 0;
    mutable pfz::LazyI32 pieces_lazy, nnz_lazy;
    int64_t piece_cap = 0;
    int32_t *tab_base = nullptr;
    int32_t *tab = nullptr;
    int2 *post = nullptr;
    uint16_t *pblk = nullptr;
    float max_norm = 1.f;
    uint64_t src_serial = 0;
    mutable pfz::K3SymState *sym = nullptr;
};

struct pfz_topn {
    pfz_ctx *ctx = nullptr;
    int64_t n_rows = 0;
    int32_t ntop = 0;
    int32_t *idx = nullptr;
    float *val = nullptr;
};

struct pfz_strings {
    pfz_ctx *ctx = nullptr;
    int64_t n = 0, n_units = 0;
    int32_t char_width = 1;
    void *chars = nullptr;
    bool chars_in_offsets = false;
    int64_t *offsets = nullptr;
    int64_t max_len = 0;
    std::vector<int64_t> h_off;
    struct pfz_indel_plan *indel_plan = nullptr;
    struct pfz_fuzz_forms *fuzz_forms = nullptr;
    struct pfz_fuzz_plan *fuzz_plan = nullptr;
    uint64_t cache_gen = 0;
    uint64_t *slots = nullptr;
    size_t slots_cap = 0;
    int32_t *row_cnt = nullptr;
};

void pfz_indel_plan_free(struct pfz_indel_plan *p);
void pfz_fuzz_forms_free(struct pfz_fuzz_forms *f);
void pfz_fuzz_plan_free(struct pfz_fuzz_plan *p);

struct pfz_tfidf {
    pfz_ctx *ctx = nullptr;
    pfz_tfidf_params params;
    uint64_t gen = 0;
    int32_t bits_per_char = 0;
    int32_t code_bits = 0;
    uint32_t *alpha_map = nullptr;
    int64_t alpha_map_len = 0;
    std::vector<uint32_t> alphabet;
    uint32_t *bitmap = nullptr;
    int32_t *prefix = nullptr;
    int64_t n_groups = 0;
    int64_t vocab = 0, n_docs = 0;
    uint64_t *vcodes = nullptr;
    int32_t *df = nullptr;
    double *idf = nullptr;
};

namespace pfz {

inline int decode_skip_codes(std::vector<int32_t> &v)
{
    bool eq = false, le = false;
    for (int32_t x : v) {
        eq |= x >= 0;
        le |= x <= -2;
    }
    if (eq && le) return -1;
    if (!le) return 0;
    for (int32_t &x : v) x = x <= -2 ? -2 - x : -1;
    return 1;
}
__host__ __device__ inline bool choice_left_out(int orig, int s, int up_to) { return up_to ? orig <= s : orig == s; }

template <typename T, void (*Free)(T *)> struct Owner {
    T *p;
    explicit Owner(T *q) : p(q) {}
    ~Owner() { if (p) Free(p); }
    Owner(const Owner &) = delete;
    Owner &operator=(const Owner &) = delete;
    T *operator->() const { return p; }
    T *release() { T *q = p; p = nullptr; return q; }
};

int ensure_scratch(pfz_ctx *ctx, size_t bytes);
int lazy_begin(pfz_ctx *ctx, LazyI32 *z, const int32_t *dev);
int lazy_acquire(pfz_ctx *ctx, LazyI32 *z);
int lazy_mark(pfz_ctx *ctx, LazyI32 *z);
int lazy_get(pfz_ctx *ctx, LazyI32 *z, int32_t *out);
void lazy_release(pfz_ctx *ctx, LazyI32 *z);
int64_t csr_nnz(const pfz_csr *m);
int index_ready(const pfz_index *ix);
int ensure_side_stream(pfz_ctx *ctx);
int event_flag_next(pfz_ctx *ctx, int32_t slot, int32_t **flag, int32_t *value);
int copy_h2d(pfz_ctx *ctx, void *dst_dev, const void *src_host, size_t bytes);
int copy_d2h(pfz_ctx *ctx, void *dst_host, const void *src_dev, size_t bytes);
struct ProfScope {
    pfz_ctx *ctx;
    const char *name;
    hipStream_t st;
    hipEvent_t b = nullptr, e = nullptr;
    ProfScope(pfz_ctx *c, const char *n, hipStream_t on = nullptr);
    ~ProfScope();
};
void prof_count(pfz_ctx *ctx, const char *name);

int pool_alloc_raw(pfz_ctx *ctx, void **p, size_t bytes);
template <typename T> inline int pool_alloc(pfz_ctx *ctx, T **p, size_t bytes)
{
    return pool_alloc_raw(ctx, (void **)p, bytes);
}
void pool_free(void *p);
int pool_release(pfz_ctx *ctx);

int comm_rank(const pfz_comm *c);
int comm_world(const pfz_comm *c);
int comm_allgather_bytes(pfz_comm *c, const void *send, void *recv, size_t bytes_per_rank);
int comm_allreduce_sum_i32(pfz_comm *c, int32_t *buf, size_t n);
int comm_allreduce_sum_i64(pfz_comm *c, int64_t *buf, size_t n);
int comm_agree(pfz_comm *c, bool mine, bool *all);
void comm_abort(pfz_comm *c);

int exclusive_scan_i32(pfz_ctx *ctx, int32_t *data, int64_t n, LazyI32 *total = nullptr);

int best_to_topn(pfz_ctx *ctx, const int32_t *d_idx, const double *d_score, int64_t n, pfz_topn *out);

int64_t sort_codes_capacity(int64_t n);
int sort_codes_u64(pfz_ctx *ctx, const uint64_t *in, uint64_t *out, int64_t n);

}
```

### polyfuzz_amd/models/_tfidf.py

```python
import os
import re
import time
from typing import List, Tuple

import numpy as np
import pandas as pd
from scipy.sparse import csr_matrix

from .. import _lib
from ._base import BaseMatcher
from ._utils import topn_to_frame, object_column, clip_top_n, FrameBuilder, _METHODS

_SPLIT_MIN_ROWS = 20000
_SPLIT_EVENT = 48
_SPLIT_BLOCK = 2048
_SYMMETRIC_ROWS = (20480, 250000)


def _split_ends(n, self_match=False):
    env = os.environ.get("PFZ_MATCH_SHARES")
    shares = None
    if env:
        sh = tuple(float(x) for x in env.split(","))
        if 1 <= len(sh) <= 16 and all(x > 0 for x in sh):
            shares = tuple(x / sum(sh) for x in sh)
    if shares is None:
        if self_match and _SYMMETRIC_ROWS[0] <= n <= _SYMMETRIC_ROWS[1] and n >= 2 * _SPLIT_MIN_ROWS and os.environ.get("PFZ_K3_SYM") != "0":
            shares = (1.0 / 12,) * 12
        else:
            shares = (0.4, 0.3, 0.2, 0.1) if n >= 2 * _SPLIT_MIN_ROWS else (0.6, 0.4)
    ends, acc = [], 0.0
    for f in shares[:-1]:
        acc += f
        e = int(n * acc) // _SPLIT_BLOCK * _SPLIT_BLOCK
        if e > (ends[-1] if ends else 0) and e < n:
            ends.append(e)
    ends.append(n)
    return ends


def _clean_string(string: str) -> str:
    string = re.sub(r'[^A-Za-z0-9 ]+', '', string.lower())
    string = re.sub(r'\s+', ' ', string).strip()
    return string


_TRACE = bool(os.environ.get("PFZ_MATCH_TRACE"))
_DIRECT_PACK = os.environ.get("PFZ_DIRECT_PACK", "1") != "0"
_RANGE_FILL = os.environ.get("PFZ_RANGE_FILL", "1") != "0"
_FROM_IN_PACK = os.environ.get("PFZ_FROM_IN_PACK", "1") != "0"


class HipTfidfVectorizer:

    def __init__(self, owner, dev):
        self._owner = owner
        self._dev = dev
        self._state = None

    def _export(self):
        if self._state is None:
            ngrams, idf, df = self._dev.export()
            names = ["".join(chr(c) for c in row if c) for row in ngrams.tolist()]
            self._state = (ngrams, idf, df, names)
        return self._state

    @property
    def idf_(self):
        return self._export()[1]

    @property
    def vocabulary_(self):
        return {g: i for i, g in enumerate(self._export()[3])}

    def get_feature_names_out(self):
        return np.array(self._export()[3], dtype=object)

    def transform(self, raw_documents) -> csr_matrix:
        docs = self._owner._upload(list(raw_documents))
        return _download_csr(self._dev.transform(docs))


def _download_csr(dev_csr) -> csr_matrix:
    indptr, indices, data, n_cols = dev_csr.download()
    return csr_matrix((data.astype(np.float64), indices, indptr), shape=(len(indptr) - 1, n_cols))


class TFIDF(BaseMatcher):
    def __init__(self,
                 n_gram_range: Tuple[int, int] = (3, 3),
                 clean_string: bool = True,
                 min_similarity: float = 0.75,
                 top_n: int = 1,
                 cosine_method: str = "sparse",
                 model_id: str = None,
                 remove_space_ngrams=True):
        super().__init__(model_id)
        self.type = "TF-IDF"
        self.n_gram_range = n_gram_range
        self.clean_string = clean_string
        self.min_similarity = min_similarity
        self.cosine_method = cosine_method
        self.top_n = top_n
        self.remove_space_ngrams = remove_space_ngrams
        self._dev_vec = None
        self._dev_to = None
        self._dev_index = None
        self._vectorizer = None
        self._host_state = None
        self.last_timings = None

    @property
    def vectorizer(self):
        self._restore()
        return self._vectorizer

    @property
    def tf_idf_to(self):
        self._restore()
        return None if self._dev_to is None else _download_csr(self._dev_to)

    def match(self,
              from_list: List[str],
              to_list: List[str] = None,
              re_train: bool = True) -> pd.DataFrame:
        if self.cosine_method not in _METHODS:
            raise ValueError(f"cosine_method must be one of {_METHODS}")
        ctx = _lib.Context.default()
        t0 = time.perf_counter()
        ranged = _RANGE_FILL and _lib._PACK_INTO_THREADS > 1 and to_list is None and isinstance(from_list, list) and len(from_list) >= _SPLIT_MIN_ROWS and \
            _lib._pack is not None and hasattr(_lib._pack, "fill_ranges")
        col = [np.empty(len(from_list), dtype=object)] if isinstance(from_list, list) and len(from_list) >= 1024 and _FROM_IN_PACK and not ranged else None
        from_dev, to_dev = self._extract_tf_idf(from_list, to_list, re_train, col)
        top_n = clip_top_n(self.top_n, to_list)
        self_match = to_list is None
        lower = float(self.min_similarity) if self.cosine_method in ("sparse", "hip") else 0.0
        n = len(from_list)
        names = from_list if self_match else to_list
        split = n >= _SPLIT_MIN_ROWS and top_n >= 1 and _lib._pack is not None and isinstance(names, (list, tuple))
        if split:
            ends = _split_ends(n, self_match)
            res, h_idx, h_val = _lib.cossim_topn_ranges(ctx, self._dev_index, from_dev, top_n, lower, self_match, ends, _SPLIT_EVENT,
                                                        mirror=True)
            if not h_idx:
                res.rows_begin(0, ends[0], _SPLIT_EVENT, 0)
        else:
            res = _lib.cossim_topn(ctx, self._dev_index, from_dev, max(top_n, 1), lower, exclude_diag=self_match)
        t1 = time.perf_counter()
        pending = ranged and split and bool(h_idx)
        from_col = col[0] if col and col[0] is not None else None if pending else object_column(from_list)
        t2 = time.perf_counter()
        if split:
            fb = FrameBuilder(from_list, names, top_n, from_col, from_pending=pending)
            waited = framed = 0.0
            tp = t2
            row0 = 0
            trace = [("enqueued", t1 - t0), ("frame wrapped", time.perf_counter() - t0)] if _TRACE else None
            if h_idx and _RANGE_FILL and hasattr(_lib._pack, "fill_ranges"):
                wait_addr, ctx_addr = ctx.event_wait_fn()
                stamps = np.zeros(2 * len(ends)) if _TRACE else None
                fb.fill_ranges(h_idx, h_val, ends, wait_addr, ctx_addr, _SPLIT_EVENT, stamps)
                tb = time.perf_counter()
                if trace is not None:
                    off = time.perf_counter() - time.monotonic()
                    for i in range(len(ends)):
                        trace += [(f"range {i} [{ends[i - 1] if i else 0}, {ends[i]}) here", stamps[2 * i] + off - t0),
                                  (f"range {i} filled", stamps[2 * i + 1] + off - t0)]
                    trace.append(("fill returned", tb - t0))
                framed, tp = framed + (tb - tp), tb
                ends = ()
            for i, row1 in enumerate(ends):
                if h_idx:
                    ctx.event_wait(_SPLIT_EVENT + i)
                    idx_addr, val_addr = h_idx + 4 * top_n * row0, h_val + 4 * top_n * row0
                else:
                    idx_addr, val_addr = res.rows_finish(i & 1)
                    if i + 1 < len(ends):
                        res.rows_begin(row1, ends[i + 1], _SPLIT_EVENT + i + 1, (i + 1) & 1)
                ta = time.perf_counter()
                fb.fill_raw(idx_addr, val_addr, row1 - row0, row0)
                tb = time.perf_counter()
                if trace is not None:
                    trace += [(f"range {i} [{row0}, {row1}) here", ta - t0), (f"range {i} filled", tb - t0)]
                waited, framed, tp = waited + (ta - tp), framed + (tb - ta), tb
                row0 = row1
            self.last_trace = trace
            frame = fb.frame()
            t4 = time.perf_counter()
            framed += t4 - tp
        else:
            idx, val = res.download()
            t3 = time.perf_counter()
            frame = topn_to_frame(idx, val, from_list, names, top_n, from_col=from_col)
            t4 = time.perf_counter()
            waited, framed = t3 - t2, t4 - t3
        self.last_timings = {"upload_and_enqueue": (t1 - t0) * 1e3, "from_column": (t2 - t1) * 1e3,
                             "wait_and_download": waited * 1e3, "frame": framed * 1e3}
        return frame

    def match_device(self, from_list: List[str], to_list: List[str] = None, re_train: bool = True):
        if self.cosine_method not in _METHODS:
            raise ValueError(f"cosine_method must be one of {_METHODS}")
        ctx = _lib.Context.default()
        from_dev, _ = self._extract_tf_idf(from_list, to_list, re_train)
        top_n = clip_top_n(self.top_n, to_list)
        lower = float(self.min_similarity) if self.cosine_method in ("sparse", "hip") else 0.0
        return _lib.cossim_topn(ctx, self._dev_index, from_dev, max(top_n, 1), lower, exclude_diag=to_list is None)

    def _params(self):
        lo, hi = int(self.n_gram_range[0]), int(self.n_gram_range[1])
        return _lib.TfidfParams(lo, hi, int(bool(self.clean_string)), int(bool(self.remove_space_ngrams)))

    def _upload(self, strings, objects=None):
        ctx = _lib.Context.default()
        direct = _lib.DeviceStrings.upload_direct(ctx, strings, objects) if len(strings) >= 1024 and _DIRECT_PACK else None
        if direct is not None:
            return direct
        packed = _lib.pack_strings(strings, objects)
        if self.clean_string and packed[2] != 1:
            packed = _lib.pack_strings([_clean_string(s) for s in strings])
        return _lib.DeviceStrings.upload_packed(ctx, *packed)

    def _extract_tf_idf(self, from_list, to_list=None, re_train=True, from_objects=None):
        ctx = _lib.Context.default()
        self._restore()
        objs = from_objects[0] if from_objects else None
        if from_objects:
            from_objects[0] = None
        if to_list:
            from_s = self._upload(from_list, objs)
            if from_objects:
                from_objects[0] = objs
            if re_train:
                to_s = self._upload(to_list)
                self._fit(ctx, to_s, from_s)
                self._set_to_side(ctx, self._dev_vec.transform(to_s))
            self._require_fitted()
            return self._dev_vec.transform(from_s), self._dev_to
        if re_train:
            from_s = self._upload(from_list, objs)
            if from_objects:
                from_objects[0] = objs
            self._fit(ctx, from_s, None)
            self._set_to_side(ctx, self._dev_vec.transform(from_s))
        self._require_fitted()
        return self._dev_to, self._dev_to

    def _fit(self, ctx, docs_a, docs_b):
        self._dev_vec = _lib.DeviceTfidf.fit(ctx, self._params(), docs_a, docs_b)
        self._vectorizer = HipTfidfVectorizer(self, self._dev_vec)
        self._host_state = None

    def _set_to_side(self, ctx, dev_csr):
        self._dev_to = dev_csr
        self._dev_index = _lib.DeviceIndex.build(ctx, dev_csr)

    def _require_fitted(self):
        if self._dev_vec is None or self._dev_index is None:
            raise ValueError("This TFIDF instance is not fitted yet: call match(..., re_train=True) first")

    def __getstate__(self):
        state = {k: v for k, v in self.__dict__.items()
                 if k not in ("_dev_vec", "_dev_to", "_dev_index", "_vectorizer", "_host_state")}
        host = self._host_state
        if host is None and self._dev_vec is not None:
            ngrams, idf, _ = self._dev_vec.export()
            host = {"ngrams": ngrams, "idf": idf, "n_docs": self._dev_vec.info()["n_docs"],
                    "params": tuple(getattr(self._dev_vec.params, f) for f, _ in _lib.TfidfParams._fields_),
                    "to_csr": None if self._dev_to is None else self._dev_to.download()}
        state["_host_state"] = host
        return state

    def __setstate__(self, state):
        self.__dict__.update(state)
        self._dev_vec = self._dev_to = self._dev_index = self._vectorizer = None

    def _restore(self):
        if self._dev_vec is not None or self._host_state is None:
            return
        ctx = _lib.Context.default()
        h = self._host_state
        self._dev_vec = _lib.DeviceTfidf.from_state(ctx, _lib.TfidfParams(*h["params"]), h["ngrams"], h["idf"],
                                                    h["n_docs"])
        self._vectorizer = HipTfidfVectorizer(self, self._dev_vec)
        if h["to_csr"] is not None:
            indptr, indices, data, n_cols = h["to_csr"]
            self._set_to_side(ctx, _lib.DeviceCSR.upload(ctx, indptr, indices, data, n_cols))
```

### polyfuzz_amd/pipeline.py

```python
import numpy as np

from . import _lib

PROFILED_KERNELS = ("k1_extract", "k2_rows_short", "k2_rows_long", "k2_df_hist", "k2_finalize", "k_index_count",
                    "k_index_fill", "k_index_bank_order", "k3_cossim_topn")


def shard_bounds(n, world, rank):
    base, rem = divmod(n, world)
    begin = rank * base + min(rank, rem)
    return begin, begin + base + (1 if rank < rem else 0)


def balanced_bounds(strings, world):
    n = len(strings)
    if world <= 1 or n == 0:
        return [(0, n)] + [(n, n)] * (max(world, 1) - 1)
    cost = np.fromiter((len(s) + 1 for s in strings), np.int64, n)
    cs = np.cumsum(cost)
    edges = [0] + [int(np.searchsorted(cs, cs[-1] * r // world, side="left")) for r in range(1, world)] + [n]
    edges = [min(max(e, 0), n) for e in edges]
    for i in range(1, len(edges)):
        edges[i] = max(edges[i], edges[i - 1])
    return list(zip(edges[:-1], edges[1:]))


class HipEngine:

    def __init__(self, ctx):
        self.ctx = ctx

    def upload_strings(self, strings):
        return _lib.DeviceStrings.upload(self.ctx, strings)

    def fit(self, params, docs_a, docs_b):
        return _lib.DeviceTfidf.fit(self.ctx, params, docs_a, docs_b)

    def fit_sharded(self, comm, params, replicated, local_shard):
        return _lib.tfidf_fit_sharded(self.ctx, comm, params, replicated, local_shard)

    def transform(self, vec, docs):
        return vec.transform(docs)

    def build_index(self, to_csr):
        return _lib.DeviceIndex.build(self.ctx, to_csr)

    def alloc_topn(self, n_rows, ntop):
        return _lib.DeviceTopN.alloc(self.ctx, n_rows, ntop)

    def cossim_topn(self, index, from_csr, ntop, lower_bound, exclude_diag, diag_offset, out):
        return _lib.cossim_topn(self.ctx, index, from_csr, ntop, lower_bound, exclude_diag=exclude_diag,
                                diag_offset=diag_offset, out=out)

    def allgather_topn(self, comm, local, out):
        return comm.allgather_topn(local, out)

    def symmetric_ok(self, comm, index, csr, ntop):
        return comm.symmetric_ok(index, csr, ntop)

    def cossim_topn_symmetric(self, comm, index, csr, ntop, lower_bound, out):
        return comm.cossim_topn_symmetric(index, csr, ntop, lower_bound, out)


class TfidfMatchJob:
    def __init__(self, ctx, from_shard, to_list, top_n=1, min_similarity=0.0, n_gram_range=(3, 3),
                 clean_string=True, remove_space_ngrams=True, comm=None, self_match=False, shard_offset=0,
                 rows_per_rank=None, engine=None):
        self.ctx = ctx
        self.eng = engine if engine is not None else HipEngine(ctx)
        self.comm = comm
        self.top_n = int(top_n)
        self.min_similarity = float(min_similarity)
        self.self_match = bool(self_match)
        self.shard_offset = int(shard_offset)
        self.params = _lib.TfidfParams(int(n_gram_range[0]), int(n_gram_range[1]), int(bool(clean_string)),
                                       int(bool(remove_space_ngrams)))
        self.n_from = len(from_shard)
        self.from_dev = self.eng.upload_strings(from_shard)
        if to_list is None:
            if not self.self_match or self.shard_offset != 0:
                raise ValueError("to_list=None means a whole-list self-match (self_match=True, shard_offset=0)")
            self.n_to, self.to_dev = self.n_from, self.from_dev
        elif to_list is from_shard and self.self_match and self.shard_offset == 0:
            self.n_to, self.to_dev = self.n_from, self.from_dev
        else:
            self.n_to = len(to_list)
            self.to_dev = self.eng.upload_strings(to_list)
        self.rows_per_rank = self.n_from if rows_per_rank is None else int(rows_per_rank)
        if self.rows_per_rank < self.n_from:
            raise ValueError("rows_per_rank is smaller than this rank's shard")
        self.local = self.eng.alloc_topn(self.rows_per_rank, self.top_n)
        self.local.clear()
        self.gathered = None
        if comm is not None and comm.world > 1:
            self.gathered = self.eng.alloc_topn(self.rows_per_rank * comm.world, self.top_n)
        self.vec = self.from_csr = self.to_csr = self.index = None
        self.full = None
        self.result_is_full = False
        self._symmetric = None

    def step(self):
        eng = self.eng
        sharded = self.comm is not None and self.comm.world > 1
        if self.self_match:
            self.vec = eng.fit(self.params, self.to_dev, None)
        elif sharded:
            self.vec = eng.fit_sharded(self.comm, self.params, self.to_dev, self.from_dev)
        else:
            self.vec = eng.fit(self.params, self.to_dev, self.from_dev)
        self.to_csr = eng.transform(self.vec, self.to_dev)
        self.index = eng.build_index(self.to_csr)
        if self.self_match and sharded and self.to_dev is not self.from_dev and self._symmetric is None:
            self._symmetric = bool(eng.symmetric_ok(self.comm, self.index, self.to_csr, self.top_n))
        if self._symmetric:
            if self.full is None:
                self.full = eng.alloc_topn(self.n_to, self.top_n)
            self.from_csr = self.to_csr
            eng.cossim_topn_symmetric(self.comm, self.index, self.to_csr, self.top_n, self.min_similarity, self.full)
            self.result_is_full = True
            return self.full
        self.result_is_full = False
        if self.self_match and self.shard_offset == 0 and (self.to_dev is self.from_dev or (not sharded and self.n_from == self.n_to)):
            self.from_csr = self.to_csr
        else:
            self.from_csr = eng.transform(self.vec, self.from_dev)
        eng.cossim_topn(self.index, self.from_csr, self.top_n, self.min_similarity, self.self_match, self.shard_offset,
                        self.local)
        if self.gathered is not None:
            eng.allgather_topn(self.comm, self.local, self.gathered)
        return self.gathered if self.gathered is not None else self.local

    def whole_result(self, idx, val, shard_sizes):
        if self.result_is_full:
            return idx, val
        return self.unpad(idx, val, shard_sizes, self.rows_per_rank)

    @staticmethod
    def unpad(idx, val, shard_sizes, rows_per_rank):
        keep = np.concatenate([np.arange(r * rows_per_rank, r * rows_per_rank + n) for r, n in enumerate(shard_sizes)])
        return idx[keep], val[keep]

    def step_description(self):
        what = ("fit vocabulary+idf on the list (K1/K2), vectorise it, build the inverted index, fused cosine top-n "
                "with the diagonal excluded (K3)" if self.self_match else
                "fit vocabulary+idf on to+from (K1/K2), vectorise both lists, build the to-side inverted index, "
                "fused cosine top-n (K3)")
        if self.result_is_full:
            return what + ("; the self-match cut over the ranks in K3's symmetric form (every unordered pair once over all ranks): all-gather "
                           "of the ranks' pass-0 thresholds and of their per-row candidate lists, merged on every rank")
        return what + ("; all-gather of the per-shard results" if self.gathered else "")

    def host_matrices(self):
        fp, fi, fv, n_cols = self.from_csr.download()
        tp, ti, tv, _ = self.to_csr.download()
        return (fp, fi, fv.astype(np.float64)), (tp, ti, tv.astype(np.float64)), n_cols

    def stats(self):
        (fp, fi, _), (tp, ti, _), n_cols = self.host_matrices()
        df_from = np.bincount(fi, minlength=n_cols).astype(np.float64)
        df_to = np.bincount(ti, minlength=n_cols).astype(np.float64)
        out = {"vocab": int(n_cols), "nnz_from": int(fp[-1]), "nnz_to": int(tp[-1]),
               "madds": float((df_from * df_to).sum())}
        if self.from_csr is self.to_csr and self.index is not None:
            info = self.index.info()
            c, nb = info["block_cols"], info["n_blocks"]
            row_of = np.repeat(np.arange(len(tp) - 1, dtype=np.int64), np.diff(tp))
            per_list = np.bincount(ti.astype(np.int64) * nb + row_of // c, minlength=n_cols * nb).astype(np.float64)
            madds_diag = float((per_list * per_list).sum())
            out["madds_symmetric"] = 0.5 * (out["madds"] + madds_diag)
            out["cells_symmetric"] = float(((nb - np.arange(len(tp) - 1, dtype=np.int64) // c) * c).sum())
        return out


def sharded_self_match(ctx, comm, names, top_n=1, min_similarity=0.0, n_gram_range=(3, 3), clean_string=True,
                       remove_space_ngrams=True, engine=None):
    from .models._utils import topn_to_frame
    names = names if isinstance(names, list) else list(names)
    bounds = balanced_bounds(names, comm.world) if len(names) > 250_000 else [shard_bounds(len(names), comm.world, r) for r in range(comm.world)]
    b, e = bounds[comm.rank]
    sizes = [y - x for x, y in bounds]
    job = TfidfMatchJob(ctx, names[b:e], names, top_n=top_n, min_similarity=min_similarity, n_gram_range=n_gram_range,
                        clean_string=clean_string, remove_space_ngrams=remove_space_ngrams, comm=comm, self_match=True,
                        shard_offset=b, rows_per_rank=max(sizes), engine=engine)
    idx, val = job.step().download()
    idx, val = job.whole_result(idx, val, sizes)
    return topn_to_frame(np.ascontiguousarray(idx, np.int32), np.ascontiguousarray(val, np.float32), names, names, top_n)


class ToShardedMatchJob:

    def __init__(self, ctx, from_list, to_shard, to_offset, comm, top_n=1, min_similarity=0.0, n_gram_range=(3, 3),
                 clean_string=True, remove_space_ngrams=True, self_match=False):
        self.ctx, self.comm = ctx, comm
        self.top_n, self.min_similarity, self.self_match = int(top_n), float(min_similarity), bool(self_match)
        self.to_offset = int(to_offset)
        self.params = _lib.TfidfParams(int(n_gram_range[0]), int(n_gram_range[1]), int(bool(clean_string)),
                                       int(bool(remove_space_ngrams)))
        self.from_dev = _lib.DeviceStrings.upload(ctx, from_list)
        self.to_dev = _lib.DeviceStrings.upload(ctx, to_shard)
        self.n_from = len(from_list)
        self.local = _lib.DeviceTopN.alloc(ctx, self.n_from, self.top_n)
        self.merged = _lib.DeviceTopN.alloc(ctx, self.n_from, self.top_n)

    def step(self):
        ctx = self.ctx
        self.vec = _lib.tfidf_fit_sharded(ctx, self.comm, self.params, None if self.self_match else self.from_dev, self.to_dev)
        self.to_csr = self.vec.transform(self.to_dev)
        self.index = _lib.DeviceIndex.build(ctx, self.to_csr)
        self.from_csr = self.vec.transform(self.from_dev)
        _lib.cossim_topn(ctx, self.index, self.from_csr, self.top_n, self.min_similarity, exclude_diag=self.self_match,
                         diag_offset=-self.to_offset, out=self.local)
        return self.comm.merge_to_shards(self.local, self.to_offset, self.merged)


class DenseMatchJob:

    def __init__(self, ctx, from_shard, to_vectors, top_n=1, min_similarity=0.0, normalize=True, comm=None,
                 self_match=False, shard_offset=0, rows_per_rank=None):
        self.ctx, self.comm = ctx, comm
        self.top_n, self.min_similarity = int(top_n), float(min_similarity)
        self.self_match, self.shard_offset = bool(self_match), int(shard_offset)
        self.from_dev = _lib.DeviceDense.upload(ctx, from_shard, normalize)
        self.to_dev = self.from_dev if to_vectors is None else _lib.DeviceDense.upload(ctx, to_vectors, normalize)
        if to_vectors is None and (not self.self_match or self.shard_offset != 0):
            raise ValueError("to_vectors=None means a whole-matrix self-match (self_match=True, shard_offset=0)")
        self.n_from, self.n_to = self.from_dev.n, self.to_dev.n
        self.rows_per_rank = self.n_from if rows_per_rank is None else int(rows_per_rank)
        if self.rows_per_rank < self.n_from:
            raise ValueError("rows_per_rank is smaller than this rank's shard")
        self.local = _lib.DeviceTopN.alloc(ctx, self.rows_per_rank, self.top_n)
        self.local.clear()
        self.gathered = None
        if comm is not None and comm.world > 1:
            self.gathered = _lib.DeviceTopN.alloc(ctx, self.rows_per_rank * comm.world, self.top_n)

    def step(self):
        _lib.dense_topn(self.ctx, self.from_dev, self.to_dev, self.top_n, self.min_similarity,
                        exclude_diag=self.self_match, diag_offset=self.shard_offset, out=self.local)
        if self.gathered is not None:
            self.comm.allgather_topn(self.local, self.gathered)
        return self.gathered if self.gathered is not None else self.local


class BestChoiceJob:

    def __init__(self, ctx, from_shard, to_list, scorer="ratio", comm=None, skip=None, rows_per_rank=None):
        from .models._rapidfuzz import _DEVICE_SCORERS, _K4_SCORERS, upload_for
        if scorer not in _DEVICE_SCORERS:
            raise NotImplementedError(f"scorer {scorer!r} has no kernel")
        self.ctx, self.comm, self.scorer = ctx, comm, scorer
        self.from_shard, self.to_list, self.skip = list(from_shard), to_list, skip
        self.n_from = len(self.from_shard)
        self.rows_per_rank = self.n_from if rows_per_rank is None else int(rows_per_rank)
        if self.rows_per_rank < self.n_from:
            raise ValueError("rows_per_rank is smaller than this rank's shard")
        self.k4 = scorer in _K4_SCORERS
        self._qfix = None
        self.f_dev = upload_for(ctx, scorer, self.from_shard)
        self.t_dev = upload_for(ctx, scorer, to_list)
        self.local = _lib.DeviceTopN.alloc(ctx, max(self.rows_per_rank, 1), 2)
        self.local.clear()
        self.gathered = None
        if comm is not None and comm.world > 1:
            self.gathered = _lib.DeviceTopN.alloc(ctx, max(self.rows_per_rank, 1) * comm.world, 2)

    def plan_info(self):
        return _lib.indel_plan_info(self.ctx, self.t_dev) if self.k4 else _lib.fuzz_plan_info(self.ctx, self.t_dev)

    def _qratio_rows(self):
        if self._qfix is None:
            self._qfix = []
            if self.scorer == "QRatio":
                for i, s in enumerate(self.from_shard):
                    if len(s) == 0:
                        first = next((j for j in range(len(self.to_list))
                                      if not (self.skip is not None and (j == self.skip[i] or j <= -2 - int(self.skip[i])))), -1)
                        self._qfix.append((i, first))
        return self._qfix

    def step(self):
        if self.n_from and len(self.to_list):
            if self.k4:
                _lib.indel_argmax_dev(self.ctx, self.f_dev, self.t_dev, self.local, self.skip)
            else:
                _lib.fuzz_extract_one_dev(self.ctx, self.f_dev, self.t_dev, self.scorer, self.local, self.skip)
            fix = self._qratio_rows()
            if fix:
                idx, val = self.local.download()
                for i, first in fix:
                    idx[i, 0], val[i, :] = first, 0.0
                self.local.upload(idx, val)
        if self.gathered is not None:
            self.comm.allgather_topn(self.local, self.gathered)
        return self.gathered if self.gathered is not None else self.local

    def result_host(self, result):
        idx, score = _lib.best_from_topn(*result.download())
        if self.gathered is None:
            idx, score = idx[:self.n_from], score[:self.n_from]
        return idx, score

    def roofline(self, step_s, peak_tops):
        if self.k4:
            return None
        w = _lib.fuzz_extract_one_dev(self.ctx, self.f_dev, self.t_dev, self.scorer, self.local, self.skip, counters=True) \
            if self.n_from and len(self.to_list) else None
        w = w or {"pairs_bounded": 0, "pairs_scored": 0, "word_steps_scored": 0}
        pairs = self.n_from * float(len(self.to_list))
        ops = 40.0 * w["pairs_bounded"] + 10.0 * w["word_steps_scored"]
        return {"kernel": "k7_fuzz", "bound": "int32 VALU issue (+ LDS look-ups)", "achieved": ops / step_s / 1e12 if step_s > 0 else None,
                "peak": peak_tops, "unit": "Tera int-op/s", "frac": ops / step_s / 1e12 / peak_tops if step_s > 0 else None, "traffic": None,
                "pairs_per_s_kernel": pairs / step_s if step_s > 0 else None, "pairs_bounded": w["pairs_bounded"],
                "pairs_scored": w["pairs_scored"], "scored_fraction": w["pairs_scored"] / max(pairs, 1.0),
                "word_steps_scored_estimate": w["word_steps_scored"],
                "what": "40 int-ops per bounded pair (two sweeps) + 10 per 64-bit word-step of the scored pairs, over the summed "
                        "k7 kernel time, against 256 CU x 4 SIMD x 32 lanes x 2.4 GHz; extractOne keeps only the maximum, so the "
                        "kernel scores only the pairs whose upper bound reaches the best score found so far"}

    @staticmethod
    def unpad(idx, score, sizes, rows_per_rank):
        keep = np.concatenate([np.arange(r * rows_per_rank, r * rows_per_rank + m) for r, m in enumerate(sizes)])
        return idx[keep], score[keep]
# ... 23 lines not shown
```

Baseline: 3632 billion.

## Deduplicate identical TF-IDF rows before self-match top-n and expand results per group

Adds a GPU pass that hashes each CSR row, groups rows with identical sparse vectors, and builds a compact CSR of distinct rows. The symmetric top-n kernel runs over the distinct rows only, and a new expand kernel maps results back to every original row, adjusting for duplicate groups. It removes redundant similarity work when the input list contains duplicate strings. In exchange it adds hashing, compaction and expansion kernels, so correctness depends on the tie and self-exclusion handling inside each group.

```diff
diff --git a/include/polyfuzz_hip.h b/include/polyfuzz_hip.h
--- a/include/polyfuzz_hip.h
+++ b/include/polyfuzz_hip.h
@@ -80,6 +80,18 @@
 int pfz_cossim_topn_ranges(pfz_ctx *ctx, const pfz_index *to_index, const pfz_csr *from_matrix, int32_t ntop, float lower_bound,
                            int32_t exclude_diag, int32_t n_ranges, const int64_t *range_ends, int32_t first_event, pfz_topn *out,
                            const int32_t **host_idx, const float **host_val);
+
+typedef struct pfz_distinct pfz_distinct;
+int pfz_csr_distinct(pfz_ctx *ctx, const pfz_csr *matrix, pfz_distinct **out);
+void pfz_distinct_free(pfz_distinct *d);
+int pfz_distinct_info(const pfz_distinct *d, int64_t *n_rows, int64_t *n_distinct);
+int pfz_distinct_csr(const pfz_distinct *d, const pfz_csr **csr);
+int pfz_distinct_download(pfz_ctx *ctx, const pfz_distinct *d, int32_t *rep, int32_t *first, int32_t *grp_ptr, int32_t *grp_rows);
+int pfz_cossim_topn_distinct(pfz_ctx *ctx, const pfz_index *distinct_index, pfz_distinct *d, int32_t ntop, float lower_bound,
+                             pfz_topn *out);
+int pfz_cossim_topn_ranges_distinct(pfz_ctx *ctx, const pfz_index *distinct_index, pfz_distinct *d, int32_t ntop, float lower_bound,
+                                    int32_t n_ranges, const int64_t *range_ends, int32_t first_event, pfz_topn *out,
+                                    const int32_t **host_idx, const float **host_val);
 
 int pfz_cossim_topn_host(pfz_ctx *ctx,
                          int64_t n_from, int64_t n_to, int64_t n_cols,
diff --git a/polyfuzz_amd/_lib.py b/polyfuzz_amd/_lib.py
--- a/polyfuzz_amd/_lib.py
+++ b/polyfuzz_amd/_lib.py
@@ -64,6 +64,13 @@
     "pfz_topn_rows_begin": (ctypes.c_int, [c_vp, c_vp, c_i64, c_i64, c_i32, c_i32]),
     "pfz_topn_rows_finish": (ctypes.c_int, [c_vp, c_i32, P(c_vp), P(c_vp)]),
     "pfz_cossim_topn_ranges": (ctypes.c_int, [c_vp, c_vp, c_vp, c_i32, ctypes.c_float, c_i32, c_i32, P(c_i64), c_i32, c_vp, P(c_vp), P(c_vp)]),
+    "pfz_csr_distinct": (ctypes.c_int, [c_vp, c_vp, P(c_vp)]),
+    "pfz_distinct_free": (None, [c_vp]),
+    "pfz_distinct_info": (ctypes.c_int, [c_vp, P(c_i64), P(c_i64)]),
+    "pfz_distinct_csr": (ctypes.c_int, [c_vp, P(c_vp)]),
+    "pfz_distinct_download": (ctypes.c_int, [c_vp, c_vp, c_vp, c_vp, c_vp, c_vp]),
+    "pfz_cossim_topn_distinct": (ctypes.c_int, [c_vp, c_vp, c_vp, c_i32, c_f32, c_vp]),
+    "pfz_cossim_topn_ranges_distinct": (ctypes.c_int, [c_vp, c_vp, c_vp, c_i32, c_f32, c_i32, P(c_i64), c_i32, c_vp, P(c_vp), P(c_vp)]),
     "pfz_event_wait": (ctypes.c_int, [c_vp, c_i32]),
     "pfz_stage_reserve": (ctypes.c_int, [c_vp, c_i64, P(c_vp)]),
     "pfz_topn_upload": (ctypes.c_int, [c_vp, c_vp, c_vp, c_vp]),
@@ -282,6 +289,42 @@
         return indptr, indices, data, n_cols
 
 
+class _BorrowedCSR(DeviceCSR):
+
+    def free(self):
+        self.h = None
+
+
+class DeviceDistinct(_Handle):
+    _free = "pfz_distinct_free"
+
+    @classmethod
+    def build(cls, ctx, csr):
+        h = c_vp()
+        check(ctx.lib.pfz_csr_distinct(ctx.h, csr.h, ctypes.byref(h)))
+        d = cls(ctx, h)
+        a, b = c_i64(), c_i64()
+        check(ctx.lib.pfz_distinct_info(h, ctypes.byref(a), ctypes.byref(b)))
+        d.n_rows, d.n_distinct = a.value, b.value
+        m = c_vp()
+        check(ctx.lib.pfz_distinct_csr(h, ctypes.byref(m)))
+        d.csr = _BorrowedCSR(ctx, m)
+        return d
+
+    def free(self):
+        if getattr(self, "csr", None) is not None:
+            self.csr.h = None
+        super().free()
+
+    def download(self):
+        rep = np.empty(self.n_rows, np.int32)
+        first = np.empty(self.n_distinct, np.int32)
+        grp_ptr = np.empty(self.n_distinct + 1, np.int32)
+        grp_rows = np.empty(self.n_rows, np.int32)
+        check(self.ctx.lib.pfz_distinct_download(self.ctx.h, self.h, _ptr(rep), _ptr(first), _ptr(grp_ptr), _ptr(grp_rows)))
+        return rep, first, grp_ptr, grp_rows
+
+
 class DeviceIndex(_Handle):
     _free = "pfz_index_free"
 
@@ -394,6 +437,23 @@
                                          len(range_ends), ends, int(first_event), out.h,
                                          ctypes.byref(hi) if mirror else None, ctypes.byref(hv) if mirror else None))
     return (out, hi.value, hv.value) if mirror else out
+
+
+def cossim_topn_distinct(ctx, distinct_index, distinct, ntop, lower_bound, out=None):
+    if out is None:
+        out = DeviceTopN.alloc(ctx, distinct.n_rows, ntop)
+    check(ctx.lib.pfz_cossim_topn_distinct(ctx.h, distinct_index.h, distinct.h, int(ntop), float(lower_bound), out.h))
+    return out
+
+
+def cossim_topn_ranges_distinct(ctx, distinct_index, distinct, ntop, lower_bound, range_ends, first_event, out=None):
+    if out is None:
+        out = DeviceTopN.alloc(ctx, distinct.n_rows, ntop)
+    ends = (c_i64 * len(range_ends))(*[int(e) for e in range_ends])
+    hi, hv = c_vp(), c_vp()
+    check(ctx.lib.pfz_cossim_topn_ranges_distinct(ctx.h, distinct_index.h, distinct.h, int(ntop), float(lower_bound), len(range_ends), ends,
+                                                  int(first_event), out.h, ctypes.byref(hi), ctypes.byref(hv)))
+    return out, hi.value, hv.value
 
 
 def cossim_topn_host(ctx, from_csr3, to_csr3, n_cols, ntop, lower_bound, exclude_diag=False):
diff --git a/polyfuzz_amd/csrc/k3_core.h b/polyfuzz_amd/csrc/k3_core.h
--- a/polyfuzz_amd/csrc/k3_core.h
+++ b/polyfuzz_amd/csrc/k3_core.h
@@ -360,11 +360,28 @@
 
 int k3_sym_wanted(const pfz_ctx *ctx, const pfz_index *ix, const pfz_csr *A, int64_t row_begin, int64_t row_end, int32_t ntop,
                   int32_t thr0, float scale, int32_t exclude_diag, int64_t diag_offset, const pfz_topn *out);
+struct K3Expand {
+    int32_t n, ntop;
+    const int32_t *rep;
+    const int32_t *grp_ptr;
+    const int32_t *grp_rows;
+    const int32_t *d_indptr;
+    const float *d_val;
+    uint64_t *keys;
+    float scale, inv_scale;
+    int32_t thr0;
+    int32_t *out_idx;
+    float *out_val;
+    int32_t *host_idx;
+    float *host_val;
+};
+void k3_expand_launch(hipStream_t stream, const K3Expand &x, int64_t row_begin, int64_t row_end);
 int k3_sym_launch(pfz_ctx *ctx, const pfz_index *ix, const pfz_csr *A, int64_t row_begin, int64_t row_end, int32_t ntop,
-                  int32_t thr0, float scale, float inv_scale, pfz_topn *out, bool start, bool *declined);
+                  int32_t thr0, float scale, float inv_scale, pfz_topn *out, bool start, bool *declined, const K3Expand *ex = nullptr);
 int k3_sym_launch_streamed(pfz_ctx *ctx, const pfz_index *ix, const pfz_csr *A, int32_t ntop, int32_t thr0, float scale, float inv_scale,
                            pfz_topn *out, int32_t n_ranges, const int64_t *ends, int32_t first_event, int32_t *host_idx, float *host_val,
-                           bool *declined);
+                           bool *declined, const K3Expand *ex = nullptr, const int64_t *d_ends = nullptr);
 void k3_sym_free(pfz_index *ix);
-
-}
+int ctx_mirror(pfz_ctx *ctx, size_t bytes);
+
+}
diff --git a/polyfuzz_amd/csrc/k3_cossim_topn.hip b/polyfuzz_amd/csrc/k3_cossim_topn.hip
--- a/polyfuzz_amd/csrc/k3_cossim_topn.hip
+++ b/polyfuzz_amd/csrc/k3_cossim_topn.hip
@@ -421,6 +421,21 @@
         PFZ_TRY(lazy_get(ix->ctx, &ix->nnz_lazy, &v));
         ix->nnz = v;
     }
+    return PFZ_OK;
+}
+
+int ctx_mirror(pfz_ctx *ctx, size_t bytes)
+{
+    if (bytes <= ctx->mirror_bytes) return PFZ_OK;
+    PFZ_HIP(hipStreamSynchronize(ctx->stream));
+    if (ctx->stream3) PFZ_HIP(hipStreamSynchronize(ctx->stream3));
+    for (int q = 0; q < 3; ++q)
+        if (ctx->stream3x[q]) PFZ_HIP(hipStreamSynchronize(ctx->stream3x[q]));
+    if (ctx->mirror) PFZ_HIP(hipHostFree(ctx->mirror));
+    ctx->mirror = nullptr;
+    ctx->mirror_bytes = 0;
+    PFZ_HIP(hipHostMalloc((void **)&ctx->mirror, bytes + bytes / 8, hipHostMallocDefault));
+    ctx->mirror_bytes = bytes + bytes / 8;
     return PFZ_OK;
 }
 
@@ -733,18 +748,7 @@
             float *h_val = nullptr;
             if (host_idx && host_val) {
                 const size_t cells = (size_t)A->n_rows * (size_t)ntop;
-                const size_t bytes = cells * (sizeof(int32_t) + sizeof(float));
-                if (bytes > ctx->mirror_bytes) {
-                    PFZ_HIP(hipStreamSynchronize(ctx->stream));
-                    if (ctx->stream3) PFZ_HIP(hipStreamSynchronize(ctx->stream3));
-                    for (int q = 0; q < 3; ++q)
-                        if (ctx->stream3x[q]) PFZ_HIP(hipStreamSynchronize(ctx->stream3x[q]));
-                    if (ctx->mirror) PFZ_HIP(hipHostFree(ctx->mirror));
-                    ctx->mirror = nullptr;
-                    ctx->mirror_bytes = 0;
-                    PFZ_HIP(hipHostMalloc((void **)&ctx->mirror, bytes + bytes / 8, hipHostMallocDefault));
-                    ctx->mirror_bytes = bytes + bytes / 8;
-                }
+                PFZ_TRY(ctx_mirror(ctx, cells * (sizeof(int32_t) + sizeof(float))));
                 h_idx = (int32_t *)ctx->mirror;
                 h_val = (float *)(ctx->mirror + cells * sizeof(int32_t));
             }
diff --git a/polyfuzz_amd/csrc/k3_distinct.hip b/polyfuzz_amd/csrc/k3_distinct.hip
--- /dev/null
+++ b/polyfuzz_amd/csrc/k3_distinct.hip
@@ -0,0 +1,436 @@
+#include "k3_core.h"
+
+namespace pfz {
+
+constexpr int kDistinctSub = 8;
+constexpr int kDistinctRows = 256 / kDistinctSub;
+constexpr int kProbe = 64;
+constexpr uint64_t kSlotEmpty = ~0ull;
+constexpr uint64_t kRowMask = (1ull << 30) - 1ull;
+
+__device__ inline uint64_t mix64(uint64_t x)
+{
+    x ^= x >> 30;
+    x *= 0xbf58476d1ce4e5b9ull;
+    x ^= x >> 27;
+    x *= 0x94d049bb133111ebull;
+    x ^= x >> 31;
+    return x;
+}
+
+__device__ inline uint64_t shfl_xor_u64(uint64_t v, int m)
+{
+    const uint32_t lo = (uint32_t)__shfl_xor((int)(uint32_t)v, m);
+    const uint32_t hi = (uint32_t)__shfl_xor((int)(uint32_t)(v >> 32), m);
+    return ((uint64_t)hi << 32) | lo;
+}
+
+__global__ __launch_bounds__(256) void k_distinct_insert(const int32_t *__restrict__ indptr, const int32_t *__restrict__ idx,
+                                                         const float *__restrict__ val, int32_t n, uint64_t *__restrict__ table,
+                                                         uint32_t mask, int32_t *__restrict__ slot_of)
+{
+    const int row = blockIdx.x * kDistinctRows + threadIdx.x / kDistinctSub, sub = threadIdx.x % kDistinctSub;
+    const int b = row < n ? indptr[row] : 0, e = row < n ? indptr[row + 1] : 0;
+    uint64_t h = 0;
+    for (int p = b + sub; p < e; p += kDistinctSub)
+        h += mix64(((uint64_t)(uint32_t)idx[p] << 32) | (uint32_t)__float_as_int(val[p]));
+    for (int m = 1; m < kDistinctSub; m <<= 1) h += shfl_xor_u64(h, m);
+    if (sub != 0 || row >= n) return;
+    h = mix64(h + (uint64_t)(uint32_t)(e - b) * 0x9e3779b97f4a7c15ull);
+    const uint64_t tag = h & ~kRowMask, entry = tag | (uint32_t)row;
+    uint32_t slot = (uint32_t)h & mask;
+    int found = -1;
+    for (int t = 0; t < kProbe; ++t) {
+        const uint64_t old = atomicCAS((unsigned long long *)&table[slot], (unsigned long long)kSlotEmpty, (unsigned long long)entry);
+        if (old == kSlotEmpty) {
+            found = (int)slot;
+            break;
+        }
+        if ((old & ~kRowMask) == tag) {
+            atomicMin((unsigned long long *)&table[slot], (unsigned long long)entry);
+            found = (int)slot;
+            break;
+        }
+        slot = (slot + 1u) & mask;
+    }
+    slot_of[row] = found;
+}
+
+__global__ __launch_bounds__(256) void k_distinct_resolve(const int32_t *__restrict__ indptr, const int32_t *__restrict__ idx,
+                                                          const float *__restrict__ val, int32_t n, const uint64_t *__restrict__ table,
+                                                          const int32_t *__restrict__ slot_of, int32_t *__restrict__ leader,
+                                                          int32_t *__restrict__ flag, int32_t *__restrict__ len, int32_t *__restrict__ cnt,
+                                                          int32_t *__restrict__ cursor)
+{
+    const int row = blockIdx.x * kDistinctRows + threadIdx.x / kDistinctSub, sub = threadIdx.x % kDistinctSub;
+    int cand = row;
+    if (row < n) {
+        const int s = slot_of[row];
+        if (s >= 0) cand = (int)(table[s] & kRowMask);
+    }
+    int same = 1;
+    if (cand != row) {
+        const int b = indptr[row], e = indptr[row + 1], cb = indptr[cand], ce = indptr[cand + 1];
+        same = (e - b) == (ce - cb);
+        if (same)
+            for (int p = sub; p < e - b; p += kDistinctSub)
+                same &= (idx[b + p] == idx[cb + p]) & (__float_as_int(val[b + p]) == __float_as_int(val[cb + p]));
+    }
+    for (int m = 1; m < kDistinctSub; m <<= 1) same &= __shfl_xor(same, m);
+    if (sub != 0 || row >= n) return;
+    if (!same) cand = row;
+    leader[row] = cand;
+    flag[row] = cand == row;
+    len[row] = 0;
+    cnt[row] = 0;
+    cursor[row] = 0;
+}
+
+__global__ __launch_bounds__(256) void k_distinct_number(const int32_t *__restrict__ indptr, int32_t n, const int32_t *__restrict__ leader,
+                                                         const int32_t *__restrict__ did, int32_t *__restrict__ rep,
+                                                         int32_t *__restrict__ first, int32_t *__restrict__ len, int32_t *__restrict__ cnt,
+                                                         int32_t *__restrict__ below)
+{
+    const int r = blockIdx.x * 256 + threadIdx.x;
+    if (r >= n) return;
+    const int l = leader[r], d = did[l];
+    rep[r] = d;
+    atomicAdd(&cnt[d], 1);
+    if (l == r) {
+        first[d] = r;
+        len[d] = indptr[r + 1] - indptr[r];
+    }
+    if (r % 2048 == 0) below[r / 2048] = did[r];
+}
+
+__global__ __launch_bounds__(256) void k_distinct_fill(const int32_t *__restrict__ indptr, const int32_t *__restrict__ idx,
+                                                       const float *__restrict__ val, int32_t n, const int32_t *__restrict__ leader,
+                                                       const int32_t *__restrict__ rep, const int32_t *__restrict__ d_indptr,
+                                                       int32_t *__restrict__ d_idx, float *__restrict__ d_val,
+                                                       const int32_t *__restrict__ grp_ptr, int32_t *__restrict__ cursor,
+                                                       int32_t *__restrict__ grp_rows, int32_t *__restrict__ unordered)
+{
+    const int row = blockIdx.x * kDistinctRows + threadIdx.x / kDistinctSub, sub = threadIdx.x % kDistinctSub;
+    if (row >= n) return;
+    const int d = rep[row];
+    if (leader[row] == row) {
+        const int b = indptr[row], e = indptr[row + 1], o = d_indptr[d];
+        for (int p = sub; p < e - b; p += kDistinctSub) {
+            d_idx[o + p] = idx[b + p];
+            d_val[o + p] = val[b + p];
+        }
+        if (sub == 0) grp_rows[grp_ptr[d]] = row;
+    } else if (sub == 0) {
+        unordered[grp_ptr[d] + 1 + atomicAdd(&cursor[d], 1)] = row;
+    }
+}
+
+__global__ __launch_bounds__(256) void k_distinct_place(int32_t n, const int32_t *__restrict__ leader, const int32_t *__restrict__ rep,
+                                                        const int32_t *__restrict__ grp_ptr, const int32_t *__restrict__ unordered,
+                                                        int32_t *__restrict__ grp_rows, const int32_t *__restrict__ did,
+                                                        const int32_t *__restrict__ d_indptr, int32_t *__restrict__ below, int32_t n_below)
+{
+    const int r = blockIdx.x * 256 + threadIdx.x;
+    if (r == 0) {
+        below[n_below] = did[n];
+        below[n_below + 1] = d_indptr[n];
+    }
+    if (r >= n || leader[r] == r) return;
+    const int d = rep[r], b = grp_ptr[d] + 1, e = grp_ptr[d + 1];
+    int rank = 0;
+    for (int p = b; p < e; ++p) rank += unordered[p] < r;
+    grp_rows[b + rank] = r;
+}
+
+__global__ __launch_bounds__(64) void k3_expand(const K3Expand x, int32_t row_begin, int32_t row_end)
+{
+    const int lane = threadIdx.x;
+    const int r = row_begin + blockIdx.x;
+    if (r >= row_end) return;
+    const int ntop = x.ntop;
+    const int d = x.rep[r];
+    uint64_t key = lane < ntop ? x.keys[(int64_t)d * ntop + lane] : 0ull;
+    int cur = 0, end = 0;
+    if (key) {
+        const int c = (int)(~(uint32_t)key);
+        cur = x.grp_ptr[c];
+        end = x.grp_ptr[c + 1];
+    }
+    const int sb = x.grp_ptr[d], se = x.grp_ptr[d + 1];
+    uint64_t mine = 0ull;
+    if (se - sb == 1 && !__ballot(end - cur > 1)) {
+        if (key) mine = (key & 0xffffffff00000000ull) | (uint32_t)(~x.grp_rows[cur]);
+    } else {
+        uint32_t sum = (uint32_t)(key >> 32);
+        if (se - sb > 1) {
+            int s = 0;
+            for (int p = x.d_indptr[d] + lane; p < x.d_indptr[d + 1]; p += 64) {
+                const float v = x.d_val[p];
+                const float as = v * x.scale;
+                s += (int)(as * v);
+            }
+            for (int m = 1; m < 64; m <<= 1) s += __shfl_xor(s, m);
+            if (lane == ntop && s > x.thr0) {
+                sum = (uint32_t)s;
+                cur = sb;
+                end = se;
+            }
+        }
+        int col = 0;
+        if (cur < end) {
+            col = x.grp_rows[cur];
+            if (col == r && ++cur < end) col = x.grp_rows[cur];
+        }
+        for (int o = 0; o < ntop; ++o) {
+            const uint64_t k = cur < end ? ((uint64_t)sum << 32) | (uint32_t)(~col) : 0ull;
+            uint64_t best = k;
+            for (int m = 1; m < 64; m <<= 1) {
+                const uint64_t other = shfl_xor_u64(best, m);
+                best = other > best ? other : best;
+            }
+            if (best == 0ull) break;
+            if (lane == o) mine = best;
+            if (k == best && ++cur < end) {
+                col = x.grp_rows[cur];
+                if (col == r && ++cur < end) col = x.grp_rows[cur];
+            }
+        }
+    }
+    if (lane < ntop) {
+        const int32_t j = mine ? (int32_t)(~(uint32_t)mine) : -1;
+        const float v = mine ? (float)(int32_t)(uint32_t)(mine >> 32) * x.inv_scale : 0.f;
+        x.out_idx[(int64_t)r * ntop + lane] = j;
+        x.out_val[(int64_t)r * ntop + lane] = v;
+        if (x.host_idx) {
+            x.host_idx[(int64_t)r * ntop + lane] = j;
+            x.host_val[(int64_t)r * ntop + lane] = v;
+            __threadfence_system();
+        }
+    }
+}
+
+void k3_expand_launch(hipStream_t stream, const K3Expand &x, int64_t row_begin, int64_t row_end)
+{
+    if (row_end <= row_begin) return;
+    hipLaunchKernelGGL(k3_expand, dim3((unsigned)(row_end - row_begin)), dim3(64), 0, stream, x, (int32_t)row_begin, (int32_t)row_end);
+}
+
+static int distinct_keys(pfz_ctx *ctx, pfz_distinct *d, int32_t ntop)
+{
+    const size_t want = (size_t)(d->nd > 0 ? d->nd : 1) * (size_t)ntop;
+    if (want <= d->keys_cap) return PFZ_OK;
+    if (d->keys) pool_free(d->keys);
+    d->keys = nullptr;
+    d->keys_cap = 0;
+    PFZ_TRY(pool_alloc(ctx, &d->keys, want * sizeof(uint64_t)));
+    d->keys_cap = want;
+    return PFZ_OK;
+}
+
+static void fill_expand(K3Expand &x, const pfz_distinct *d, int32_t ntop, float scale, float inv_scale, int32_t thr0, pfz_topn *out)
+{
+    x.n = (int32_t)d->n;
+    x.ntop = ntop;
+    x.rep = d->rep;
+    x.grp_ptr = d->grp_ptr;
+    x.grp_rows = d->grp_rows;
+    x.d_indptr = d->csr->indptr;
+    x.d_val = d->csr->data;
+    x.keys = d->keys;
+    x.scale = scale;
+    x.inv_scale = inv_scale;
+    x.thr0 = thr0;
+    x.out_idx = out->idx;
+    x.out_val = out->val;
+    x.host_idx = nullptr;
+    x.host_val = nullptr;
+}
+
+}
+
+using namespace pfz;
+
+extern "C" {
+
+void pfz_distinct_free(pfz_distinct *d)
+{
+    if (!d) return;
+    if (d->ctx) (void)hipSetDevice(d->ctx->device);
+    void *const bufs[] = {d->rep, d->first, d->grp_ptr, d->grp_rows, d->keys};
+    for (void *p : bufs)
+        if (p) pool_free(p);
+    pfz_csr_free(d->csr);
+    delete d;
+}
+
+int pfz_csr_distinct(pfz_ctx *ctx, const pfz_csr *m, pfz_distinct **out)
+{
+    PFZ_REQUIRE(ctx && m && out, "pfz_csr_distinct: NULL argument");
+    PFZ_REQUIRE(m->n_rows >= 1 && m->n_rows < ((int64_t)1 << 30), "pfz_csr_distinct: 1 to 2^30 - 1 rows (got %lld)", (long long)m->n_rows);
+    PFZ_HIP(hipSetDevice(ctx->device));
+    const int64_t n = m->n_rows;
+    Owner<pfz_distinct, pfz_distinct_free> d(new pfz_distinct());
+    d->ctx = ctx;
+    d->n = n;
+    d->csr = new pfz_csr();
+    d->csr->ctx = ctx;
+    d->csr->n_cols = m->n_cols;
+    d->csr->max_norm = m->max_norm;
+    const int64_t cap = m->nnz_lazy.pending ? m->nnz_cap : m->nnz;
+    d->csr->nnz_cap = cap;
+    PFZ_TRY(pool_alloc(ctx, &d->csr->indptr, (size_t)(n + 1) * sizeof(int32_t)));
+    PFZ_TRY(pool_alloc(ctx, &d->csr->indices, (size_t)(cap > 0 ? cap : 1) * sizeof(int32_t)));
+    PFZ_TRY(pool_alloc(ctx, &d->csr->data, (size_t)(cap > 0 ? cap : 1) * sizeof(float)));
+    PFZ_TRY(pool_alloc(ctx, &d->rep, (size_t)n * sizeof(int32_t)));
+    PFZ_TRY(pool_alloc(ctx, &d->first, (size_t)n * sizeof(int32_t)));
+    PFZ_TRY(pool_alloc(ctx, &d->grp_ptr, (size_t)(n + 1) * sizeof(int32_t)));
+    PFZ_TRY(pool_alloc(ctx, &d->grp_rows, (size_t)n * sizeof(int32_t)));
+    uint32_t slots = 1024;
+    while ((int64_t)slots < 2 * n) slots <<= 1;
+    const int32_t n_below = (int32_t)((n + 2047) / 2048);
+    struct Tmp {
+        void *p = nullptr;
+        ~Tmp() { if (p) pool_free(p); }
+    } table, work;
+    PFZ_TRY(pool_alloc(ctx, &table.p, (size_t)slots * sizeof(uint64_t)));
+    PFZ_TRY(pool_alloc(ctx, &work.p, ((size_t)n * 5 + 1 + (size_t)n_below + 2) * sizeof(int32_t)));
+    int32_t *slot_of = (int32_t *)work.p, *leader = slot_of + n, *did = leader + n, *cursor = did + n + 1, *unordered = cursor + n,
+            *below = unordered + n;
+    int32_t *len = d->csr->indptr, *cnt = d->grp_ptr;
+    const unsigned row_grid = (unsigned)((n + kDistinctRows - 1) / kDistinctRows), flat_grid = (unsigned)((n + 255) / 256);
+    {
+        ProfScope ps(ctx, "k_distinct");
+        PFZ_HIP(hipMemsetAsync(table.p, 0xff, (size_t)slots * sizeof(uint64_t), ctx->stream));
+        hipLaunchKernelGGL(k_distinct_insert, dim3(row_grid), dim3(256), 0, ctx->stream, m->indptr, m->indices, m->data, (int32_t)n,
+                           (uint64_t *)table.p, slots - 1u, slot_of);
+        hipLaunchKernelGGL(k_distinct_resolve, dim3(row_grid), dim3(256), 0, ctx->stream, m->indptr, m->indices, m->data, (int32_t)n,
+                           (const uint64_t *)table.p, slot_of, leader, did, len, cnt, cursor);
+        PFZ_TRY(exclusive_scan_i32(ctx, did, n));
+        hipLaunchKernelGGL(k_distinct_number, dim3(flat_grid), dim3(256), 0, ctx->stream, m->indptr, (int32_t)n, leader, did, d->rep,
+                           d->first, len, cnt, below);
+        PFZ_TRY(exclusive_scan_i32(ctx, len, n));
+        PFZ_TRY(exclusive_scan_i32(ctx, cnt, n));
+        hipLaunchKernelGGL(k_distinct_fill, dim3(row_grid), dim3(256), 0, ctx->stream, m->indptr, m->indices, m->data, (int32_t)n, leader,
+                           d->rep, d->csr->indptr, d->csr->indices, d->csr->data, d->grp_ptr, cursor, d->grp_rows, unordered);
+        hipLaunchKernelGGL(k_distinct_place, dim3(flat_grid), dim3(256), 0, ctx->stream, (int32_t)n, leader, d->rep, d->grp_ptr, unordered,
+                           d->grp_rows, did, d->csr->indptr, below, n_below);
+        PFZ_HIP(hipGetLastError());
+    }
+    std::vector<int32_t> h((size_t)n_below + 2);
+    PFZ_TRY(copy_d2h(ctx, h.data(), below, h.size() * sizeof(int32_t)));
+    d->nd = h[(size_t)n_below];
+    d->csr->n_rows = d->nd;
+    d->csr->nnz = h[(size_t)n_below + 1];
+    d->below.assign(h.begin(), h.begin() + n_below);
+    d->below.push_back((int32_t)d->nd);
+    *out = d.release();
+    return PFZ_OK;
+}
+
+int pfz_distinct_info(const pfz_distinct *d, int64_t *n_rows, int64_t *n_distinct)
+{
+    PFZ_REQUIRE(d, "pfz_distinct_info: NULL argument");
+    if (n_rows) *n_rows = d->n;
+    if (n_distinct) *n_distinct = d->nd;
+    return PFZ_OK;
+}
+
+int pfz_distinct_csr(const pfz_distinct *d, const pfz_csr **csr)
+{
+    PFZ_REQUIRE(d && csr, "pfz_distinct_csr: NULL argument");
+    *csr = d->csr;
+    return PFZ_OK;
+}
+
+int pfz_distinct_download(pfz_ctx *ctx, const pfz_distinct *d, int32_t *rep, int32_t *first, int32_t *grp_ptr, int32_t *grp_rows)
+{
+    PFZ_REQUIRE(ctx && d, "pfz_distinct_download: NULL argument");
+    PFZ_HIP(hipSetDevice(ctx->device));
+    PFZ_HIP(hipStreamSynchronize(ctx->stream));
+    if (rep) PFZ_TRY(copy_d2h(ctx, rep, d->rep, (size_t)d->n * sizeof(int32_t)));
+    if (first && d->nd > 0) PFZ_TRY(copy_d2h(ctx, first, d->first, (size_t)d->nd * sizeof(int32_t)));
+    if (grp_ptr) PFZ_TRY(copy_d2h(ctx, grp_ptr, d->grp_ptr, (size_t)(d->nd + 1) * sizeof(int32_t)));
+    if (grp_rows) PFZ_TRY(copy_d2h(ctx, grp_rows, d->grp_rows, (size_t)d->n * sizeof(int32_t)));
+    return PFZ_OK;
+}
+
+static int distinct_job(pfz_ctx *ctx, const pfz_index *ix, pfz_distinct *d, int32_t ntop, float lower_bound, pfz_topn *out,
+                        float *scale, float *inv_scale, int32_t *thr0, const char *who)
+{
+    PFZ_REQUIRE(ctx && ix && d && out, "%s: NULL argument", who);
+    PFZ_REQUIRE(ntop >= 1 && lower_bound == lower_bound, "%s: ntop >= 1 and a lower bound that is a number", who);
+    PFZ_REQUIRE(ix->src_serial == d->csr->serial, "%s: the index must be built from the distinct rows (pfz_distinct_csr)", who);
+    PFZ_REQUIRE(out->n_rows >= d->n && out->ntop == ntop, "%s: result buffer is %lldx%d, need %lldx%d", who, (long long)out->n_rows,
+                out->ntop, (long long)d->n, ntop);
+    PFZ_HIP(hipSetDevice(ctx->device));
+    k3_fixed_point(d->csr, ix, lower_bound, scale, inv_scale, thr0);
+    if (k3_sym_wanted(ctx, ix, d->csr, 0, d->nd, ntop, *thr0, *scale, 1, 0, out) != 1) {
+        set_error("%s: %lld distinct rows, top %d: not a self-match K3 takes in its symmetric form", who, (long long)d->nd, ntop);
+        return PFZ_ERR_UNSUPPORTED;
+    }
+    return distinct_keys(ctx, d, ntop);
+}
+
+int pfz_cossim_topn_distinct(pfz_ctx *ctx, const pfz_index *ix, pfz_distinct *d, int32_t ntop, float lower_bound, pfz_topn *out)
+{
+    float scale, inv_scale;
+    int32_t thr0;
+    PFZ_TRY(distinct_job(ctx, ix, d, ntop, lower_bound, out, &scale, &inv_scale, &thr0, "pfz_cossim_topn_distinct"));
+    K3Expand x;
+    fill_expand(x, d, ntop, scale, inv_scale, thr0, out);
+    ProfScope ps(ctx, "k3_cossim_topn");
+    bool declined = false;
+    PFZ_TRY(k3_sym_launch(ctx, ix, d->csr, 0, d->nd, ntop, thr0, scale, inv_scale, out, true, &declined, &x));
+    if (declined) {
+        set_error("pfz_cossim_topn_distinct: no memory for the symmetric session");
+        return PFZ_ERR_UNSUPPORTED;
+    }
+    return PFZ_OK;
+}
+
+int pfz_cossim_topn_ranges_distinct(pfz_ctx *ctx, const pfz_index *ix, pfz_distinct *d, int32_t ntop, float lower_bound, int32_t n_ranges,
+                                    const int64_t *range_ends, int32_t first_event, pfz_topn *out, const int32_t **host_idx,
+                                    const float **host_val)
+{
+    if (host_idx) *host_idx = nullptr;
+    if (host_val) *host_val = nullptr;
+    PFZ_REQUIRE(range_ends, "pfz_cossim_topn_ranges_distinct: NULL argument");
+    PFZ_REQUIRE(n_ranges >= 1 && first_event >= 0 && first_event + n_ranges <= kEventSlots,
+                "pfz_cossim_topn_ranges_distinct: %d ranges from event slot %d do not fit the %d slots", n_ranges, first_event, kEventSlots);
+    float scale, inv_scale;
+    int32_t thr0;
+    PFZ_TRY(distinct_job(ctx, ix, d, ntop, lower_bound, out, &scale, &inv_scale, &thr0, "pfz_cossim_topn_ranges_distinct"));
+    std::vector<int64_t> d_ends((size_t)n_ranges);
+    int64_t prev = 0;
+    for (int32_t i = 0; i < n_ranges; ++i) {
+        const int64_t e = range_ends[i];
+        PFZ_REQUIRE(e > prev && e <= d->n && (e % 2048 == 0 || e == d->n) && (i < n_ranges - 1 || e == d->n),
+                    "pfz_cossim_topn_ranges_distinct: range ends ascend in multiples of 2048 to the last row (%lld)", (long long)d->n);
+        const int64_t need = e == d->n ? d->nd : d->below[(size_t)(e / 2048)];
+        d_ends[(size_t)i] = std::min<int64_t>((need + 2047) / 2048 * 2048, d->nd);
+        prev = e;
+    }
+    K3Expand x;
+    fill_expand(x, d, ntop, scale, inv_scale, thr0, out);
+    if (host_idx && host_val) {
+        const size_t cells = (size_t)d->n * (size_t)ntop;
+        PFZ_TRY(ctx_mirror(ctx, cells * (sizeof(int32_t) + sizeof(float))));
+        x.host_idx = (int32_t *)ctx->mirror;
+        x.host_val = (float *)(ctx->mirror + cells * sizeof(int32_t));
+    }
+    ProfScope ps(ctx, "k3_cossim_topn");
+    bool declined = false;
+    PFZ_TRY(k3_sym_launch_streamed(ctx, ix, d->csr, ntop, thr0, scale, inv_scale, out, n_ranges, range_ends, first_event, nullptr, nullptr,
+                                   &declined, &x, d_ends.data()));
+    if (declined) {
+        set_error("pfz_cossim_topn_ranges_distinct: no memory for the symmetric session");
+        return PFZ_ERR_UNSUPPORTED;
+    }
+    if (x.host_idx) {
+        *host_idx = x.host_idx;
+        *host_val = x.host_val;
+    }
+    return PFZ_OK;
+}
+
+}
diff --git a/polyfuzz_amd/csrc/k3_symmetric.hip b/polyfuzz_amd/csrc/k3_symmetric.hip
--- a/polyfuzz_amd/csrc/k3_symmetric.hip
+++ b/polyfuzz_amd/csrc/k3_symmetric.hip
@@ -174,7 +174,7 @@
 {
     const int lane = threadIdx.x;
     if (lane == 0) {
-        if (flag) __hip_atomic_store(flag, flag_value, __ATOMIC_RELAXED, __HIP_MEMORY_SCOPE_SYSTEM);
+        if (flag) __hip_atomic_store(flag, flag_value, __ATOMIC_RELEASE, __HIP_MEMORY_SCOPE_SYSTEM);
         if (a.blk_lo < a.blk_hi) a.ovf[0] = 0;
     }
     const uint64_t t0 = wall_clock64();
@@ -814,7 +814,7 @@
 }
 
 int k3_sym_launch(pfz_ctx *ctx, const pfz_index *ix, const pfz_csr *A, int64_t row_begin, int64_t row_end, int32_t ntop,
-                  int32_t thr0, float scale, float inv_scale, pfz_topn *out, bool start, bool *declined)
+                  int32_t thr0, float scale, float inv_scale, pfz_topn *out, bool start, bool *declined, const K3Expand *ex)
 {
     const int64_t n = ix->n_rows;
     const int nb = ix->n_blocks;
@@ -829,6 +829,7 @@
     sym_fill_args(a, ix, A, s, ntop, thr0, scale, inv_scale);
     a.out_idx = out->idx;
     a.out_val = out->val;
+    if (ex) a.keys_out = ex->keys;
     if (start) {
         a.row_begin = 0;
         a.row_end = (int32_t)n;
@@ -869,10 +870,11 @@
     a.row_end = (int32_t)row_end;
     hipLaunchKernelGGL(k3_sym_merge<4>, dim3((unsigned)((row_end - row_begin + 3) / 4)), dim3(256), 0, ctx->stream, a);
     sym_launch_pass2(ctx, a);
+    if (ex) k3_expand_launch(ctx->stream, *ex, 0, ex->n);
     PFZ_HIP(hipGetLastError());
-    s->next_row = row_end;
+    s->next_row = ex ? -1 : row_end;
     s->launches += 1;
-    s->rows += row_end - row_begin;
+    s->rows += ex ? ex->n : row_end - row_begin;
     s->a_serial = A->serial;
     s->out = out;
     s->ntop = ntop;
@@ -883,7 +885,7 @@
 
 int k3_sym_launch_streamed(pfz_ctx *ctx, const pfz_index *ix, const pfz_csr *A, int32_t ntop, int32_t thr0, float scale, float inv_scale,
                            pfz_topn *out, int32_t n_ranges, const int64_t *ends, int32_t first_event, int32_t *host_idx, float *host_val,
-                           bool *declined)
+                           bool *declined, const K3Expand *ex, const int64_t *d_ends)
 {
     const int64_t n = ix->n_rows;
     const int nb = ix->n_blocks;
@@ -910,6 +912,11 @@
     a.out_val = out->val;
     a.host_idx = host_idx;
     a.host_val = host_val;
+    if (ex) {
+        a.keys_out = ex->keys;
+        a.host_idx = nullptr;
+        a.host_val = nullptr;
+    }
     a.done = s->done;
     const unsigned grid0 = (unsigned)std::min<int64_t>(n, (int64_t)ctx->prop.multiProcessorCount * kSymP0PerCu);
     hipLaunchKernelGGL((k3_sym_kernel<kSymC, 0>), dim3(grid0), dim3(64), 0, ctx->stream, a);
@@ -938,7 +945,8 @@
     for (int32_t i = 0; i < n_ranges; ++i) {
         const int q = i % n_sides;
         hipStream_t side = sides[q];
-        const int64_t row1 = ends[i];
+        const int64_t row1 = ex ? d_ends[i] : ends[i];
+        if (ex) row0 = covered[q];
         a.ovf = q ? s->ovfx[q - 1] : s->ovf;
         a.part = q ? s->partx[q - 1] : s->part;
         a.blk_lo = (int32_t)(covered[q] / kSymC);
@@ -947,9 +955,12 @@
         hipLaunchKernelGGL(k3_sym_wait, dim3(1), dim3(64), 0, side, a, flag[q], flag_value[q]);
         a.row_begin = (int32_t)row0;
         a.row_end = (int32_t)row1;
-        hipLaunchKernelGGL(k3_sym_merge<PFZ_K3_SYM_MERGE_W>, dim3((unsigned)((row1 - row0 + PFZ_K3_SYM_MERGE_W - 1) / PFZ_K3_SYM_MERGE_W)),
-                           dim3(64 * PFZ_K3_SYM_MERGE_W), 0, side, a);
-        sym_launch_pass2(ctx, a, side, 2);
+        if (row1 > row0) {
+            hipLaunchKernelGGL(k3_sym_merge<PFZ_K3_SYM_MERGE_W>, dim3((unsigned)((row1 - row0 + PFZ_K3_SYM_MERGE_W - 1) / PFZ_K3_SYM_MERGE_W)),
+                               dim3(64 * PFZ_K3_SYM_MERGE_W), 0, side, a);
+            sym_launch_pass2(ctx, a, side, 2);
+        }
+        if (ex) k3_expand_launch(side, *ex, i ? ends[i - 1] : 0, ends[i]);
         PFZ_HIP(hipGetLastError());
         PFZ_HIP(hipEventRecord(ctx->events[first_event + i], side));
         PFZ_TRY(event_flag_next(ctx, first_event + i, &flag[q], &flag_value[q]));
@@ -964,9 +975,9 @@
         PFZ_HIP(hipEventRecord(side_ev[q], sides[q]));
     }
     for (int q = 0; q < n_sides; ++q) PFZ_HIP(hipStreamWaitEvent(ctx->stream, side_ev[q], 0));
-    s->next_row = n;
+    s->next_row = ex ? -1 : n;
     s->launches += 1;
-    s->rows += n;
+    s->rows += ex ? ex->n : n;
     s->a_serial = A->serial;
     s->out = out;
     s->ntop = ntop;
diff --git a/polyfuzz_amd/csrc/pfz_internal.h b/polyfuzz_amd/csrc/pfz_internal.h
--- a/polyfuzz_amd/csrc/pfz_internal.h
+++ b/polyfuzz_amd/csrc/pfz_internal.h
@@ -156,6 +156,19 @@
     int32_t *row_cnt = nullptr;
 };
 
+struct pfz_distinct {
+    pfz_ctx *ctx = nullptr;
+    int64_t n = 0, nd = 0;
+    pfz_csr *csr = nullptr;
+    int32_t *rep = nullptr;
+    int32_t *first = nullptr;
+    int32_t *grp_ptr = nullptr;
+    int32_t *grp_rows = nullptr;
+    uint64_t *keys = nullptr;
+    size_t keys_cap = 0;
+    std::vector<int32_t> below;
+};
+
 void pfz_indel_plan_free(struct pfz_indel_plan *p);
 void pfz_fuzz_forms_free(struct pfz_fuzz_forms *f);
 void pfz_fuzz_plan_free(struct pfz_fuzz_plan *p);
diff --git a/polyfuzz_amd/models/_tfidf.py b/polyfuzz_amd/models/_tfidf.py
--- a/polyfuzz_amd/models/_tfidf.py
+++ b/polyfuzz_amd/models/_tfidf.py
@@ -15,6 +15,11 @@
 _SPLIT_EVENT = 48
 _SPLIT_BLOCK = 2048
 _SYMMETRIC_ROWS = (20480, 250000)
+_SYMMETRIC_TOP_N = 32
+
+
+def distinct_rows_wanted(n, top_n):
+    return _SYMMETRIC_ROWS[0] <= n <= _SYMMETRIC_ROWS[1] and 1 <= top_n <= _SYMMETRIC_TOP_N and os.environ.get("PFZ_K3_SYM") != "0"
 
 
 def _split_ends(n, self_match=False):
@@ -106,6 +111,8 @@
         self._dev_vec = None
         self._dev_to = None
         self._dev_index = None
+        self._dev_distinct = None
+        self._dev_index_d = None
         self._vectorizer = None
         self._host_state = None
         self.last_timings = None
@@ -140,12 +147,20 @@
         split = n >= _SPLIT_MIN_ROWS and top_n >= 1 and _lib._pack is not None and isinstance(names, (list, tuple))
         if split:
             ends = _split_ends(n, self_match)
-            res, h_idx, h_val = _lib.cossim_topn_ranges(ctx, self._dev_index, from_dev, top_n, lower, self_match, ends, _SPLIT_EVENT,
-                                                        mirror=True)
+            res = None
+            if self._on_distinct(self_match, top_n):
+                try:
+                    res, h_idx, h_val = _lib.cossim_topn_ranges_distinct(ctx, self._dev_index_d, self._dev_distinct, top_n, lower, ends,
+                                                                         _SPLIT_EVENT)
+                except _lib.PfzUnsupported:
+                    self._dev_distinct = self._dev_index_d = None
+            if res is None:
+                res, h_idx, h_val = _lib.cossim_topn_ranges(ctx, self._index(), from_dev, top_n, lower, self_match, ends, _SPLIT_EVENT,
+                                                            mirror=True)
             if not h_idx:
                 res.rows_begin(0, ends[0], _SPLIT_EVENT, 0)
         else:
-            res = _lib.cossim_topn(ctx, self._dev_index, from_dev, max(top_n, 1), lower, exclude_diag=self_match)
+            res = self._cossim_topn(ctx, from_dev, top_n, lower, self_match)
         t1 = time.perf_counter()
         pending = ranged and split and bool(h_idx)
         from_col = col[0] if col and col[0] is not None else None if pending else object_column(from_list)
@@ -205,7 +220,7 @@
         from_dev, _ = self._extract_tf_idf(from_list, to_list, re_train)
         top_n = clip_top_n(self.top_n, to_list)
         lower = float(self.min_similarity) if self.cosine_method in ("sparse", "hip") else 0.0
-        return _lib.cossim_topn(ctx, self._dev_index, from_dev, max(top_n, 1), lower, exclude_diag=to_list is None)
+        return self._cossim_topn(ctx, from_dev, top_n, lower, to_list is None)
 
     def _params(self):
         lo, hi = int(self.n_gram_range[0]), int(self.n_gram_range[1])
@@ -242,7 +257,7 @@
             if from_objects:
                 from_objects[0] = objs
             self._fit(ctx, from_s, None)
-            self._set_to_side(ctx, self._dev_vec.transform(from_s))
+            self._set_to_side(ctx, self._dev_vec.transform(from_s), self_match=True)
         self._require_fitted()
         return self._dev_to, self._dev_to
 
@@ -251,17 +266,40 @@
         self._vectorizer = HipTfidfVectorizer(self, self._dev_vec)
         self._host_state = None
 
-    def _set_to_side(self, ctx, dev_csr):
+    def _set_to_side(self, ctx, dev_csr, self_match=False):
         self._dev_to = dev_csr
+        self._dev_index = self._dev_distinct = self._dev_index_d = None
+        if self_match and distinct_rows_wanted(dev_csr.n_rows, clip_top_n(self.top_n, None)):
+            distinct = _lib.DeviceDistinct.build(ctx, dev_csr)
+            if _SYMMETRIC_ROWS[0] <= distinct.n_distinct:
+                self._dev_distinct = distinct
+                self._dev_index_d = _lib.DeviceIndex.build(ctx, distinct.csr)
+                return
         self._dev_index = _lib.DeviceIndex.build(ctx, dev_csr)
 
+    def _index(self):
+        if self._dev_index is None and self._dev_to is not None:
+            self._dev_index = _lib.DeviceIndex.build(_lib.Context.default(), self._dev_to)
+        return self._dev_index
+
+    def _on_distinct(self, self_match, top_n):
+        return self_match and self._dev_distinct is not None and 1 <= top_n <= _SYMMETRIC_TOP_N and os.environ.get("PFZ_K3_SYM") != "0"
+
+    def _cossim_topn(self, ctx, from_dev, top_n, lower, self_match):
+        if self._on_distinct(self_match, top_n):
+            try:
+                return _lib.cossim_topn_distinct(ctx, self._dev_index_d, self._dev_distinct, top_n, lower)
+            except _lib.PfzUnsupported:
+                self._dev_distinct = self._dev_index_d = None
+        return _lib.cossim_topn(ctx, self._index(), from_dev, max(top_n, 1), lower, exclude_diag=self_match)
+
     def _require_fitted(self):
-        if self._dev_vec is None or self._dev_index is None:
+        if self._dev_vec is None or self._dev_to is None:
             raise ValueError("This TFIDF instance is not fitted yet: call match(..., re_train=True) first")
 
     def __getstate__(self):
         state = {k: v for k, v in self.__dict__.items()
-                 if k not in ("_dev_vec", "_dev_to", "_dev_index", "_vectorizer", "_host_state")}
+                 if k not in ("_dev_vec", "_dev_to", "_dev_index", "_dev_distinct", "_dev_index_d", "_vectorizer", "_host_state")}
         host = self._host_state
         if host is None and self._dev_vec is not None:
             ngrams, idf, _ = self._dev_vec.export()
@@ -273,7 +311,7 @@
 
     def __setstate__(self, state):
         self.__dict__.update(state)
-        self._dev_vec = self._dev_to = self._dev_index = self._vectorizer = None
+        self._dev_vec = self._dev_to = self._dev_index = self._dev_distinct = self._dev_index_d = self._vectorizer = None
 
     def _restore(self):
         if self._dev_vec is not None or self._host_state is None:
diff --git a/polyfuzz_amd/pipeline.py b/polyfuzz_amd/pipeline.py
--- a/polyfuzz_amd/pipeline.py
+++ b/polyfuzz_amd/pipeline.py
@@ -2,7 +2,7 @@
 
 from . import _lib
 
-PROFILED_KERNELS = ("k1_extract", "k2_rows_short", "k2_rows_long", "k2_df_hist", "k2_finalize", "k_index_count",
+PROFILED_KERNELS = ("k1_extract", "k2_rows_short", "k2_rows_long", "k2_df_hist", "k2_finalize", "k_distinct", "k_index_count",
                     "k_index_fill", "k_index_bank_order", "k3_cossim_topn")
 
 
@@ -51,6 +51,12 @@
     def cossim_topn(self, index, from_csr, ntop, lower_bound, exclude_diag, diag_offset, out):
         return _lib.cossim_topn(self.ctx, index, from_csr, ntop, lower_bound, exclude_diag=exclude_diag,
                                 diag_offset=diag_offset, out=out)
+
+    def distinct(self, csr):
+        return _lib.DeviceDistinct.build(self.ctx, csr)
+
+    def cossim_topn_distinct(self, index, distinct, ntop, lower_bound, out):
+        return _lib.cossim_topn_distinct(self.ctx, index, distinct, ntop, lower_bound, out=out)
 
     def allgather_topn(self, comm, local, out):
         return comm.allgather_topn(local, out)
@@ -94,7 +100,7 @@
         self.gathered = None
         if comm is not None and comm.world > 1:
             self.gathered = self.eng.alloc_topn(self.rows_per_rank * comm.world, self.top_n)
-        self.vec = self.from_csr = self.to_csr = self.index = None
+        self.vec = self.from_csr = self.to_csr = self.index = self.distinct = None
         self.full = None
         self.result_is_full = False
         self._symmetric = None
@@ -109,7 +115,14 @@
         else:
             self.vec = eng.fit(self.params, self.to_dev, self.from_dev)
         self.to_csr = eng.transform(self.vec, self.to_dev)
-        self.index = eng.build_index(self.to_csr)
+        self.distinct = None
+        if self.self_match and not sharded and self.shard_offset == 0 and self.to_dev is self.from_dev and hasattr(eng, "distinct"):
+            from .models._tfidf import distinct_rows_wanted, _SYMMETRIC_ROWS
+            if distinct_rows_wanted(self.n_to, self.top_n):
+                distinct = eng.distinct(self.to_csr)
+                if _SYMMETRIC_ROWS[0] <= distinct.n_distinct:
+                    self.distinct = distinct
+        self.index = eng.build_index(self.distinct.csr if self.distinct is not None else self.to_csr)
         if self.self_match and sharded and self.to_dev is not self.from_dev and self._symmetric is None:
             self._symmetric = bool(eng.symmetric_ok(self.comm, self.index, self.to_csr, self.top_n))
         if self._symmetric:
@@ -120,6 +133,13 @@
             self.result_is_full = True
             return self.full
         self.result_is_full = False
+        if self.distinct is not None:
+            self.from_csr = self.to_csr
+            try:
+                return eng.cossim_topn_distinct(self.index, self.distinct, self.top_n, self.min_similarity, self.local)
+            except _lib.PfzUnsupported:
+                self.distinct = None
+                self.index = eng.build_index(self.to_csr)
         if self.self_match and self.shard_offset == 0 and (self.to_dev is self.from_dev or (not sharded and self.n_from == self.n_to)):
             self.from_csr = self.to_csr
         else:
@@ -164,10 +184,15 @@
         if self.from_csr is self.to_csr and self.index is not None:
             info = self.index.info()
             c, nb = info["block_cols"], info["n_blocks"]
+            if self.distinct is not None:
+                tp, ti, _, _ = self.distinct.csr.download()
+                df_d = np.bincount(ti, minlength=n_cols).astype(np.float64)
+                out["distinct_rows"] = int(len(tp) - 1)
+                out["madds_distinct"] = float((df_d * df_d).sum())
             row_of = np.repeat(np.arange(len(tp) - 1, dtype=np.int64), np.diff(tp))
             per_list = np.bincount(ti.astype(np.int64) * nb + row_of // c, minlength=n_cols * nb).astype(np.float64)
             madds_diag = float((per_list * per_list).sum())
-            out["madds_symmetric"] = 0.5 * (out["madds"] + madds_diag)
+            out["madds_symmetric"] = 0.5 * (out.get("madds_distinct", out["madds"]) + madds_diag)
             out["cells_symmetric"] = float(((nb - np.arange(len(tp) - 1, dtype=np.int64) // c) * c).sum())
         return out
 
```

Result: slower. 1919 billion (-47.2%).
